# omerbt/Splice

Measured on AMD Instinct MI355X. Metric: opt_steps_per_sec, higher is better.
Workload: dtype bf16

## Files before the change

### include/splice_hip.h

```cpp
#ifndef SPLICE_HIP_H
#define SPLICE_HIP_H
#include <stddef.h>
#include <stdint.h>

#ifdef __cplusplus
extern "C" {
#endif

typedef uint16_t splice_bf16;
typedef void* splice_stream_t;

#define SPLICE_OK 0
#define SPLICE_ERR_ARG -1
#define SPLICE_ERR_HIP -2
#define SPLICE_ERR_STATE -3
#define SPLICE_ERR_NOMEM -4

int splice_version(void);
int splice_dev_switches(void);
const char* splice_last_error(void);

typedef struct splice_gemm_epilogue {
    const float* bias;
    const float* resid;
    int ldr, resid_mod;
    float* out_f32;
    int ldo;
    splice_bf16* out_bf;
    int ldbf;
    splice_bf16* out_bf_t;
    int ldt;
    splice_bf16* out_pre;
    int ldp, pre_row_lo;
    const splice_bf16* aux;
    int ldaux;
    float* out_f32_cols;
    int ld_cols, col_lo, col_hi;
    float alpha;
    int ksplit;
    long long slab_stride;
    const splice_bf16* rd_other;
    int ld_rd, rd_rows;
    float* rowdot;
    const float* row_scale;
    const float* col_scale;
    uint8_t* out_f8;
    int ld8;
    uint8_t* out_f8_t;
    int ldt8;
} splice_gemm_epilogue;

enum {
    SPLICE_EPI_BIAS = 1, SPLICE_EPI_RESID = 2, SPLICE_EPI_OUT_F32 = 4, SPLICE_EPI_OUT_BF = 8,
    SPLICE_EPI_OUT_T = 16, SPLICE_EPI_GELU = 32, SPLICE_EPI_GELU_GRAD = 64,
    SPLICE_EPI_COLS_F32 = 128, SPLICE_EPI_ALPHA = 256, SPLICE_EPI_ROWDOT = 512, SPLICE_EPI_SCALE_RC = 1024, SPLICE_EPI_OUT_F8 = 2048,
    SPLICE_EPI_OUT_F8T = 4096
};

int splice_gemm_nt_bf16(unsigned flags, const splice_bf16* A, int lda, const splice_bf16* B, int ldb,
                        int M, int N, int K, const splice_gemm_epilogue* epi, splice_stream_t stream);

int splice_gemm_nt_fp8(unsigned flags, const uint8_t* A, int lda, const uint8_t* B, int ldb, int M, int N, int K,
                       const splice_gemm_epilogue* epi, splice_stream_t stream);
int splice_quantize_rows_fp8(const float* x, int ldx, uint8_t* q, int ldq, float* scale, int rows, int cols, splice_stream_t stream);
int splice_gemm_splitk_slabs(int M, int ksplit);
int splice_gemm_force_tile(int tile);
int splice_attention_variant(int variant);
int splice_attention_qfold(int on);
int splice_attention_bwd_variant(int variant);

int splice_layernorm_fwd(const float* x, const float* gamma, const float* beta, splice_bf16* y,
                         float* mean, float* rstd, int rows, int D, float eps, splice_stream_t stream);
int splice_layernorm_bwd(const float* dy, const float* x, const float* gamma, const float* mean,
                         const float* rstd, const float* g_in, float* g_out, splice_bf16* g_out_bf,
                         int rows, int D, splice_stream_t stream);

int splice_attention_fwd(const splice_bf16* qkv, const splice_bf16* qkvT, int ldt, int B, int T, int Tld,
                         int D, int H, float scale, splice_bf16* out, float* lse, splice_stream_t stream);
int splice_attention_fwd_fp8(const uint8_t* qkv8, const uint8_t* qkvT8, int ldt8, int B, int T, int Tld, int D, int H, float scale,
                             splice_bf16* out, float* lse, splice_stream_t stream);
int splice_attention_bwd(const splice_bf16* qkv, const splice_bf16* qkvT, int ldt, int B, int T, int Tld,
                         int D, int H, float scale, const splice_bf16* out, const float* lse,
                         const splice_bf16* dout, const splice_bf16* doutT, float* delta,
                         splice_bf16* dqkv, splice_stream_t stream);
int splice_attention_probs(const splice_bf16* qkv, int B, int T, int Tld, int D, int H, float scale,
                           const float* lse, float* probs, splice_stream_t stream);

int splice_augment_structure(const float* img, float* out, float* scratch, int H, int W, int flip, int n_ops, const int* order,
                             const float* factors, float blur_sigma, splice_stream_t stream);

size_t splice_keys_selfsim_ws_bytes(int T, int D);
int splice_keys_selfsim_fwd(const float* K, int ldk, int T, int D, float eps, float* S, void* ws,
                            splice_stream_t stream);
int splice_keys_selfsim_bwd(const float* dS, const float* S, int T, int D, float eps, float* dK, int lddk,
                            int accumulate, void* ws, splice_stream_t stream);

int splice_mse(const float* a, int lda, const float* b, int ldb, int rows, int cols, float weight,
               float* loss_accum, float* grad, int ldg, splice_stream_t stream);

int splice_patchify(const float* img, splice_bf16* patches, int B, int H, int W, int p, int Tld,
                    int normalize, splice_stream_t stream);
int splice_unpatchify(const float* dpatches, float* dimg, int B, int H, int W, int p, int Tld,
                      int normalize, splice_stream_t stream);
int splice_cast_f32_bf16(const float* x, splice_bf16* y, size_t n, splice_stream_t stream);
int splice_cast_bf16_f32(const splice_bf16* x, float* y, size_t n, splice_stream_t stream);
int splice_transpose_f32_bf16(const float* x, splice_bf16* y, int rows, int cols, int ldy, splice_stream_t stream);
int splice_resize_bilinear_fwd(const float* in, float* out, int planes, int h, int w, int oh, int ow, splice_stream_t stream);
int splice_resize_bilinear_bwd(const float* dout, float* din, int planes, int h, int w, int oh, int ow, splice_stream_t stream);

int splice_vit_create(int patch, int dim, int depth, int heads, void** out_handle);
void splice_vit_destroy(void* vit);
int splice_vit_set_param(void* vit, const char* name, const float* data, long long numel, splice_stream_t stream);
float splice_vit_qscale(void* vit);
int splice_vit_params_complete(void* vit);
int splice_vit_enable_fp8(void* vit, splice_stream_t stream);
int splice_vit_ctx_create(void* vit, int B, int H, int W, const float* pos_TD, int need_grad,
                          splice_stream_t stream, void** out_ctx);
void splice_vit_ctx_destroy(void* ctx);
int splice_vit_ctx_info(void* ctx, int* T, int* Tld, int* rows);
int splice_vit_ctx_set_top_cls_only(void* ctx, int on);
int splice_vit_ctx_set_fp8(void* ctx, int mode);
int splice_vit_forward(void* ctx, const float* img, int normalize, splice_stream_t stream);
int splice_vit_forward_ex(void* ctx, const float* img, int normalize, int grad_pass_begin, splice_stream_t stream);
int splice_vit_forward_passes(void* ctx, const float* img, int normalize, int grad_pass_begin, int pass_begin, int pass_end,
                              splice_stream_t stream);
int splice_vit_get_tensor(void* ctx, int kind, int layer, void** out_ptr);
int splice_vit_read_tensor(void* ctx, int kind, int layer, void* dst, size_t bytes, splice_stream_t stream);
int splice_vit_backward(void* ctx, int pass_begin, int pass_end, const float* const* d_block,
                        const float* const* d_qkv, const float* const* d_keys, float* d_img,
                        int normalize, splice_stream_t stream);

int splice_gen_create(void** out_handle);
#define SPLICE_GEN_MAX_SCALES 6
typedef struct splice_gen_arch {
    int n_scales, in_channels, out_channels;
    int down[SPLICE_GEN_MAX_SCALES], up[SPLICE_GEN_MAX_SCALES], skip[SPLICE_GEN_MAX_SCALES];
    int filter_down[SPLICE_GEN_MAX_SCALES], filter_up[SPLICE_GEN_MAX_SCALES];
    int filter_skip;
    int reflect;
} splice_gen_arch;
int splice_gen_create_arch(const splice_gen_arch* arch, void** out_handle);
void splice_gen_destroy(void* gen);
long long splice_gen_param_count(void* gen);
int splice_gen_num_tensors(void* gen);
int splice_gen_tensor_info(void* gen, int i, const char** name, long long* offset, long long* numel);
int splice_gen_plan_create(void* gen, int N, int H, int W, int need_grad, void** out_plan);
void splice_gen_plan_destroy(void* plan);
int splice_gen_forward(void* plan, const float* params, const float* x, float* y, splice_stream_t stream);
int splice_gen_forward_borrowed(void* plan, const float* params, const float* x, float* y, splice_stream_t stream);
int splice_gen_backward(void* plan, const float* params, const float* dy, float* grads, int accumulate,
                        splice_stream_t stream);
long long splice_gen_buffer_count(void* gen);
int splice_gen_num_buffers(void* gen);
int splice_gen_buffer_info(void* gen, int i, const char** name, long long* offset, long long* numel);
int splice_gen_running_stats_update(void* const* plans, int n_plans, float* running, long long running_stride, float momentum,
                                    splice_stream_t stream);
int splice_adam_step(float* params, float* grads, float* m, float* v, long long n, float lr, float beta1,
                     float beta2, float eps, int step, int zero_grad, splice_stream_t stream);
int splice_optim_step(int kind, float* params, float* grads, float* m, float* v, long long n, float lr, float hp0, float hp1,
                      float eps, int step, int zero_grad, splice_stream_t stream);
int splice_optim_step_ex(int kind, float* params, float* grads, const float* g2, float* m, float* v, long long n, float lr,
                         const float* lr_dev, float hp0, float hp1, float eps, int step, int zero_grad, splice_stream_t stream);
int splice_optim_step_pairs(int kind, float* params, float* grads, const float* g2, float* m, float* v, int n_pairs, long long stride,
                            long long n, const float* lr_dev, float hp0, float hp1, float eps, int step, int zero_grad,
                            splice_stream_t stream);

int splice_prof_begin(int which);
int splice_prof_end(float* total_ms, int* launches);
int splice_prof_end_ex(float* total_ms, int* calls, int* kernels);
int splice_prof_end_detail(float* total_ms, int* calls, int* kernels, char* detail, int detail_len);
int splice_prof_active(void);
int splice_vit_ctx_dims(void* ctx, int* B, int* H, int* W, int* D, int* depth, int* heads, int* patch);
int splice_gen_plan_dims(void* plan, int* N, int* H, int* W, long long* nparams);
int splice_gen_plan_set_arena_stride(void* plan, long long stride);
int splice_gen_plan_set_batch_stats(void* plan, int on);
int splice_gen_plan_set_groups(void* plan, int images_per_group);
int splice_gen_plan_resize(void* plan, int H, int W);

typedef struct splice_step_config {
    int crop_h, crop_w;
    int vit_h, vit_w;
    int ent_h, ent_w;
    int ent_vit_h, ent_vit_w;
    float lambda_global_cls, lambda_global_ssim, lambda_global_identity, lambda_entire_cls, lambda_entire_ssim;
    int entire_every, cls_warmup;
    float lr, beta1, beta2, eps;
    int pairs;
    long long arena_stride;
    int fp8_selfsim;
    int top_cls_only;
    int n_crops;
    int n_crops_b;
} splice_step_config;
#define SPLICE_STEP_MAX_PAIR_CFGS 32
#define SPLICE_STEP_MAX_GROUP_IMAGES 32
int splice_step_create(const splice_step_config* cfg, void* vit_ctx_global, void* vit_ctx_entire, void* gen_plan_a, void* gen_plan_b,
                       void* gen_plan_entire, void** out_handle);
void splice_step_destroy(void* step);
int splice_step_run(void* step, float* params, float* grads, float* m, float* v, const float* A_crop, const float* B_crop,
                    const float* A_entire, int step_idx, float* losses_out, splice_stream_t stream);
int splice_step_output(void* step, int which, float** out_ptr);
int splice_step_graph_stats(void* step, long long* out);
int splice_step_use_graph(void* step, int on);
int splice_step_use_overlap(void* step, int on);
int splice_step_set_crops(void* step, int a_h, int a_w, int b_h, int b_w);
int splice_step_set_mode(void* step, int skip_adam, int accumulate);
int splice_step_set_optimizer(void* step, int kind, float hp0, float hp1, float eps);
int splice_step_set_lr(void* step, float lr);
int splice_step_set_pair_weights(void* step, const float* lambdas);
int splice_step_set_pair_lr(void* step, const float* lr);
int splice_step_set_phases(void* step, int phases, void* leader);
int splice_step_set_running_stats(void* step, float* running, long long stride);

#ifdef __cplusplus
}
#endif
#endif
```

### splice_amd/_lib.py

```python
import ctypes as C
import os

_HERE = os.path.dirname(os.path.abspath(__file__))
LIB_PATH = os.path.join(_HERE, "libsplice_hip.so")

_lib = None


class GemmEpilogue(C.Structure):
    _fields_ = [
        ("bias", C.c_void_p), ("resid", C.c_void_p), ("ldr", C.c_int), ("resid_mod", C.c_int),
        ("out_f32", C.c_void_p), ("ldo", C.c_int),
        ("out_bf", C.c_void_p), ("ldbf", C.c_int),
        ("out_bf_t", C.c_void_p), ("ldt", C.c_int),
        ("out_pre", C.c_void_p), ("ldp", C.c_int), ("pre_row_lo", C.c_int),
        ("aux", C.c_void_p), ("ldaux", C.c_int),
        ("out_f32_cols", C.c_void_p), ("ld_cols", C.c_int), ("col_lo", C.c_int), ("col_hi", C.c_int),
        ("alpha", C.c_float), ("ksplit", C.c_int), ("slab_stride", C.c_longlong),
        ("rd_other", C.c_void_p), ("ld_rd", C.c_int), ("rd_rows", C.c_int), ("rowdot", C.c_void_p),
        ("row_scale", C.c_void_p), ("col_scale", C.c_void_p),
        ("out_f8", C.c_void_p), ("ld8", C.c_int),
        ("out_f8_t", C.c_void_p), ("ldt8", C.c_int),
    ]


class GenArch(C.Structure):
    _fields_ = [("n_scales", C.c_int), ("in_channels", C.c_int), ("out_channels", C.c_int),
                ("down", C.c_int * 6), ("up", C.c_int * 6), ("skip", C.c_int * 6),
                ("filter_down", C.c_int * 6), ("filter_up", C.c_int * 6), ("filter_skip", C.c_int), ("reflect", C.c_int)]


class StepConfig(C.Structure):
    _fields_ = [
        ("crop_h", C.c_int), ("crop_w", C.c_int), ("vit_h", C.c_int), ("vit_w", C.c_int),
        ("ent_h", C.c_int), ("ent_w", C.c_int), ("ent_vit_h", C.c_int), ("ent_vit_w", C.c_int),
        ("lambda_global_cls", C.c_float), ("lambda_global_ssim", C.c_float), ("lambda_global_identity", C.c_float),
        ("lambda_entire_cls", C.c_float), ("lambda_entire_ssim", C.c_float),
        ("entire_every", C.c_int), ("cls_warmup", C.c_int),
        ("lr", C.c_float), ("beta1", C.c_float), ("beta2", C.c_float), ("eps", C.c_float),
        ("pairs", C.c_int), ("arena_stride", C.c_longlong), ("fp8_selfsim", C.c_int), ("top_cls_only", C.c_int), ("n_crops", C.c_int), ("n_crops_b", C.c_int),
    ]


EPI_BIAS, EPI_RESID, EPI_OUT_F32, EPI_OUT_BF, EPI_OUT_T = 1, 2, 4, 8, 16
EPI_GELU, EPI_GELU_GRAD, EPI_COLS_F32, EPI_ALPHA, EPI_ROWDOT, EPI_SCALE_RC, EPI_OUT_F8, EPI_OUT_F8T = 32, 64, 128, 256, 512, 1024, 2048, 4096

_vp, _i, _f, _sz, _u = C.c_void_p, C.c_int, C.c_float, C.c_size_t, C.c_uint

_SIGNATURES = {
    "splice_version": ([], C.c_int),
    "splice_dev_switches": ([], C.c_int),
    "splice_last_error": ([], C.c_char_p),
    "splice_gemm_nt_bf16": ([_u, _vp, _i, _vp, _i, _i, _i, _i, C.POINTER(GemmEpilogue), _vp], _i),
    "splice_gemm_nt_fp8": ([_u, _vp, _i, _vp, _i, _i, _i, _i, C.POINTER(GemmEpilogue), _vp], _i),
    "splice_quantize_rows_fp8": ([_vp, _i, _vp, _i, _vp, _i, _i, _vp], _i),
    "splice_gemm_splitk_slabs": ([_i, _i], _i),
    "splice_gemm_force_tile": ([_i], _i),
    "splice_attention_variant": ([_i], _i),
    "splice_attention_qfold": ([_i], _i),
    "splice_attention_bwd_variant": ([_i], _i),
    "splice_layernorm_fwd": ([_vp, _vp, _vp, _vp, _vp, _vp, _i, _i, _f, _vp], _i),
    "splice_layernorm_bwd": ([_vp, _vp, _vp, _vp, _vp, _vp, _vp, _vp, _i, _i, _vp], _i),
    "splice_attention_fwd": ([_vp, _vp, _i, _i, _i, _i, _i, _i, _f, _vp, _vp, _vp], _i),
    "splice_attention_fwd_fp8": ([_vp, _vp, _i, _i, _i, _i, _i, _i, _f, _vp, _vp, _vp], _i),
    "splice_attention_bwd": ([_vp, _vp, _i, _i, _i, _i, _i, _i, _f, _vp, _vp, _vp, _vp, _vp, _vp, _vp], _i),
    "splice_attention_probs": ([_vp, _i, _i, _i, _i, _i, _f, _vp, _vp, _vp], _i),
    "splice_augment_structure": ([_vp, _vp, _vp, _i, _i, _i, _i, C.POINTER(C.c_int), C.POINTER(C.c_float), _f, _vp], _i),
    "splice_keys_selfsim_ws_bytes": ([_i, _i], _sz),
    "splice_keys_selfsim_fwd": ([_vp, _i, _i, _i, _f, _vp, _vp, _vp], _i),
    "splice_keys_selfsim_bwd": ([_vp, _vp, _i, _i, _f, _vp, _i, _i, _vp, _vp], _i),
    "splice_mse": ([_vp, _i, _vp, _i, _i, _i, _f, _vp, _vp, _i, _vp], _i),
    "splice_patchify": ([_vp, _vp, _i, _i, _i, _i, _i, _i, _vp], _i),
    "splice_unpatchify": ([_vp, _vp, _i, _i, _i, _i, _i, _i, _vp], _i),
    "splice_cast_f32_bf16": ([_vp, _vp, _sz, _vp], _i),
    "splice_cast_bf16_f32": ([_vp, _vp, _sz, _vp], _i),
    "splice_transpose_f32_bf16": ([_vp, _vp, _i, _i, _i, _vp], _i),
    "splice_resize_bilinear_fwd": ([_vp, _vp, _i, _i, _i, _i, _i, _vp], _i),
    "splice_resize_bilinear_bwd": ([_vp, _vp, _i, _i, _i, _i, _i, _vp], _i),
    "splice_vit_create": ([_i, _i, _i, _i, C.POINTER(_vp)], _i),
    "splice_vit_destroy": ([_vp], None),
    "splice_vit_set_param": ([_vp, C.c_char_p, _vp, C.c_longlong, _vp], _i),
    "splice_vit_params_complete": ([_vp], _i),
    "splice_vit_enable_fp8": ([_vp, _vp], _i),
    "splice_vit_ctx_create": ([_vp, _i, _i, _i, _vp, _i, _vp, C.POINTER(_vp)], _i),
    "splice_vit_ctx_destroy": ([_vp], None),
    "splice_vit_ctx_info": ([_vp, C.POINTER(_i), C.POINTER(_i), C.POINTER(_i)], _i),
    "splice_vit_ctx_set_top_cls_only": ([_vp, _i], _i),
    "splice_vit_ctx_set_fp8": ([_vp, _i], _i),
    "splice_vit_forward": ([_vp, _vp, _i, _vp], _i),
    "splice_vit_forward_ex": ([_vp, _vp, _i, _i, _vp], _i),
    "splice_vit_forward_passes": ([_vp, _vp, _i, _i, _i, _i, _vp], _i),
    "splice_vit_get_tensor": ([_vp, _i, _i, C.POINTER(_vp)], _i),
    "splice_vit_qscale": ([_vp], C.c_float),
    "splice_vit_read_tensor": ([_vp, _i, _i, _vp, _sz, _vp], _i),
    "splice_vit_backward": ([_vp, _i, _i, C.POINTER(_vp), C.POINTER(_vp), C.POINTER(_vp), _vp, _i, _vp], _i),
    "splice_gen_create": ([C.POINTER(_vp)], _i),
    "splice_gen_create_arch": ([C.POINTER(GenArch), C.POINTER(_vp)], _i),
    "splice_gen_destroy": ([_vp], None),
    "splice_gen_param_count": ([_vp], C.c_longlong),
    "splice_gen_num_tensors": ([_vp], _i),
    "splice_gen_tensor_info": ([_vp, _i, C.POINTER(C.c_char_p), C.POINTER(C.c_longlong), C.POINTER(C.c_longlong)], _i),
    "splice_gen_plan_create": ([_vp, _i, _i, _i, _i, C.POINTER(_vp)], _i),
    "splice_gen_plan_destroy": ([_vp], None),
    "splice_gen_forward": ([_vp, _vp, _vp, _vp, _vp], _i),
    "splice_gen_forward_borrowed": ([_vp, _vp, _vp, _vp, _vp], _i),
    "splice_gen_backward": ([_vp, _vp, _vp, _vp, _i, _vp], _i),
    "splice_adam_step": ([_vp, _vp, _vp, _vp, C.c_longlong, _f, _f, _f, _f, _i, _i, _vp], _i),
    "splice_optim_step": ([_i, _vp, _vp, _vp, _vp, C.c_longlong, _f, _f, _f, _f, _i, _i, _vp], _i),
    "splice_optim_step_ex": ([_i, _vp, _vp, _vp, _vp, _vp, C.c_longlong, _f, _vp, _f, _f, _f, _i, _i, _vp], _i),
    "splice_optim_step_pairs": ([_i, _vp, _vp, _vp, _vp, _vp, _i, C.c_longlong, C.c_longlong, _vp, _f, _f, _f, _i, _i, _vp], _i),
    "splice_prof_begin": ([_i], _i),
    "splice_prof_end": ([C.POINTER(_f), C.POINTER(_i)], _i),
    "splice_prof_end_ex": ([C.POINTER(_f), C.POINTER(_i), C.POINTER(_i)], _i),
    "splice_prof_end_detail": ([C.POINTER(_f), C.POINTER(_i), C.POINTER(_i), C.c_char_p, _i], _i),
    "splice_prof_active": ([], _i),
    "splice_step_use_graph": ([_vp, _i], _i),
    "splice_step_graph_stats": ([_vp, C.POINTER(C.c_longlong)], _i),
    "splice_step_use_overlap": ([_vp, _i], _i),
    "splice_vit_ctx_dims": ([_vp] + [C.POINTER(_i)] * 7, _i),
    "splice_gen_plan_dims": ([_vp, C.POINTER(_i), C.POINTER(_i), C.POINTER(_i), C.POINTER(C.c_longlong)], _i),
    "splice_step_create": ([C.POINTER(StepConfig), _vp, _vp, _vp, _vp, _vp, C.POINTER(_vp)], _i),
    "splice_step_destroy": ([_vp], None),
    "splice_step_run": ([_vp, _vp, _vp, _vp, _vp, _vp, _vp, _vp, _i, _vp, _vp], _i),
    "splice_step_output": ([_vp, _i, C.POINTER(_vp)], _i),
    "splice_step_set_crops": ([_vp, _i, _i, _i, _i], _i),
    "splice_step_set_running_stats": ([_vp, _vp, C.c_longlong], _i),
    "splice_step_set_mode": ([_vp, _i, _i], _i),
    "splice_step_set_optimizer": ([_vp, _i, _f, _f, _f], _i),
    "splice_step_set_lr": ([_vp, _f], _i),
    "splice_step_set_pair_weights": ([_vp, _vp], _i),
    "splice_step_set_pair_lr": ([_vp, _vp], _i),
    "splice_step_set_phases": ([_vp, _i, _vp], _i),
    "splice_gen_buffer_count": ([_vp], C.c_longlong),
    "splice_gen_num_buffers": ([_vp], _i),
    "splice_gen_buffer_info": ([_vp, _i, C.POINTER(C.c_char_p), C.POINTER(C.c_longlong), C.POINTER(C.c_longlong)], _i),
    "splice_gen_running_stats_update": ([C.POINTER(_vp), _i, _vp, C.c_longlong, _f, _vp], _i),
    "splice_gen_plan_resize": ([_vp, _i, _i], _i),
    "splice_gen_plan_set_arena_stride": ([_vp, C.c_longlong], _i),
    "splice_gen_plan_set_batch_stats": ([_vp, _i], _i),
    "splice_gen_plan_set_groups": ([_vp, _i], _i),
}


def exported_symbols():
    return sorted(_SIGNATURES)


def register(name, argtypes, restype):
    _SIGNATURES[name] = (argtypes, restype)


def lib():
    global _lib
    if _lib is None:
        if not os.path.exists(LIB_PATH):
            raise RuntimeError(
                f"{LIB_PATH} not found: the HIP extension is not built "
                "(run __graft_entry__.build() or `make -C splice_amd/csrc`). There is no CPU fallback.")
        _lib = C.CDLL(LIB_PATH)
        for name, (argtypes, restype) in _SIGNATURES.items():
            fn = getattr(_lib, name)
            fn.argtypes = argtypes
            fn.restype = restype
    return _lib


def check(rc, what=""):
    if rc != 0:
        msg = lib().splice_last_error().decode(errors="replace")
        raise RuntimeError(f"libsplice_hip {what} failed (rc={rc}): {msg}")


def ptr(t):
    return None if t is None else C.c_void_p(t.data_ptr())


def current_stream():
    import torch
    return C.c_void_p(torch.cuda.current_stream().cuda_stream)
```

### splice_amd/csrc/capi.hip

```cpp
#include <stdarg.h>
#include <stdio.h>

#include "kernels.h"

static thread_local char g_err[512] = "";

void splice_set_error(const char* fmt, ...) {
    va_list ap;
    va_start(ap, fmt);
    vsnprintf(g_err, sizeof(g_err), fmt, ap);
    va_end(ap);
}

static int finish(int rc, const char* what) {
    if (rc != SPLICE_OK) {
        splice_set_error("%s: invalid argument", what);
        return rc;
    }
    const hipError_t e = hipGetLastError();
    if (e != hipSuccess) {
        splice_set_error("%s: HIP error %d (%s)", what, (int)e, hipGetErrorString(e));
        return SPLICE_ERR_HIP;
    }
    return SPLICE_OK;
}

#define ST(s) ((hipStream_t)(s))

extern "C" {

int splice_version(void) { return 100; }
int splice_dev_switches(void) {
#ifdef SPLICE_DEV_SWITCHES
    return 1;
#else
    return 0;
#endif
}
const char* splice_last_error(void) { return g_err; }

int splice_gemm_nt_bf16(unsigned flags, const splice_bf16* A, int lda, const splice_bf16* B, int ldb, int M, int N, int K,
                        const splice_gemm_epilogue* epi, splice_stream_t stream) {
    if (!A || !B || !epi) return finish(SPLICE_ERR_ARG, "splice_gemm_nt_bf16");
    return finish(gemm_nt_launch(flags, A, lda, B, ldb, M, N, K, *epi, ST(stream)), "splice_gemm_nt_bf16");
}

int splice_gemm_nt_fp8(unsigned flags, const uint8_t* A, int lda, const uint8_t* B, int ldb, int M, int N, int K,
                       const splice_gemm_epilogue* epi, splice_stream_t stream) {
    if (!A || !B || !epi) return finish(SPLICE_ERR_ARG, "splice_gemm_nt_fp8");
    return finish(gemm_nt_fp8_launch(flags, A, lda, B, ldb, M, N, K, *epi, ST(stream)), "splice_gemm_nt_fp8");
}
int splice_quantize_rows_fp8(const float* x, int ldx, uint8_t* q, int ldq, float* scale, int rows, int cols, splice_stream_t stream) {
    if (!x || !q || !scale) return finish(SPLICE_ERR_ARG, "splice_quantize_rows_fp8");
    return finish(quantize_rows_fp8_launch(x, ldx, q, ldq, scale, rows, cols, ST(stream)), "splice_quantize_rows_fp8");
}

int splice_gemm_splitk_slabs(int M, int ksplit) { return gemm_splitk_slabs(M, ksplit); }

int splice_gemm_force_tile(int tile) { gemm_force_tile(tile); return SPLICE_OK; }
int splice_attention_variant(int variant) { attn_set_variant(variant); return SPLICE_OK; }
int splice_attention_qfold(int on) { attn_set_qfold(on); return SPLICE_OK; }
int splice_attention_bwd_variant(int variant) { attn_set_bwd_variant(variant); return SPLICE_OK; }

int splice_layernorm_fwd(const float* x, const float* gamma, const float* beta, splice_bf16* y, float* mean, float* rstd,
                         int rows, int D, float eps, splice_stream_t stream) {
    return finish(layernorm_fwd_launch(x, gamma, beta, y, mean, rstd, rows, D, eps, ST(stream)), "splice_layernorm_fwd");
}
int splice_layernorm_bwd(const float* dy, const float* x, const float* gamma, const float* mean, const float* rstd,
                         const float* g_in, float* g_out, splice_bf16* g_out_bf, int rows, int D, splice_stream_t stream) {
    return finish(layernorm_bwd_launch(dy, x, gamma, mean, rstd, g_in, g_out, g_out_bf, rows, D, ST(stream)), "splice_layernorm_bwd");
}

int splice_attention_fwd(const splice_bf16* qkv, const splice_bf16* qkvT, int ldt, int B, int T, int Tld, int D, int H,
                         float scale, splice_bf16* out, float* lse, splice_stream_t stream) {
    AttnArgs a = {};
    a.qkv = qkv; a.qkvT = qkvT; a.ldt = ldt; a.B = B; a.T = T; a.Tld = Tld; a.D = D; a.H = H; a.scale = scale;
    a.out = out; a.lse = lse; a.qfold = attn_qfold_hook();
    return finish(attn_fwd_launch(&a, ST(stream)), "splice_attention_fwd");
}
int splice_attention_fwd_fp8(const uint8_t* qkv8, const uint8_t* qkvT8, int ldt8, int B, int T, int Tld, int D, int H, float scale,
                             splice_bf16* out, float* lse, splice_stream_t stream) {
    if (!qkv8 || !qkvT8 || !out || !lse) return finish(SPLICE_ERR_ARG, "splice_attention_fwd_fp8");
    AttnArgs a = {};
    a.qkv8 = qkv8; a.qkvT8 = qkvT8; a.ldt8 = ldt8; a.ldt = 4; a.B = B; a.T = T; a.Tld = Tld; a.D = D; a.H = H; a.scale = scale;
    a.out = out; a.lse = lse;
    return finish(attn_fwd_launch(&a, ST(stream)), "splice_attention_fwd_fp8");
}
int splice_attention_bwd(const splice_bf16* qkv, const splice_bf16* qkvT, int ldt, int B, int T, int Tld, int D, int H,
                         float scale, const splice_bf16* out, const float* lse, const splice_bf16* dout,
                         const splice_bf16* doutT, float* delta, splice_bf16* dqkv, splice_stream_t stream) {
    AttnArgs a = {};
    a.qkv = qkv; a.qkvT = qkvT; a.ldt = ldt; a.B = B; a.T = T; a.Tld = Tld; a.D = D; a.H = H; a.scale = scale;
    a.out = const_cast<splice_bf16*>(out); a.lse = const_cast<float*>(lse);
    a.dout = dout; a.doutT = doutT; a.delta = delta; a.dqkv = dqkv; a.qfold = attn_qfold_hook();
    return finish(attn_bwd_launch(&a, ST(stream)), "splice_attention_bwd");
}
int splice_attention_probs(const splice_bf16* qkv, int B, int T, int Tld, int D, int H, float scale, const float* lse,
                           float* probs, splice_stream_t stream) {
    AttnArgs a = {};
    a.qkv = qkv; a.B = B; a.T = T; a.Tld = Tld; a.D = D; a.H = H; a.scale = scale; a.lse = const_cast<float*>(lse);
    return finish(attn_probs_launch(&a, probs, ST(stream)), "splice_attention_probs");
}

int splice_augment_structure(const float* img, float* out, float* scratch, int H, int W, int flip, int n_ops, const int* order,
                             const float* factors, float blur_sigma, splice_stream_t stream) {
    return finish(augment_structure_launch(img, out, scratch, H, W, flip, n_ops, order, factors, blur_sigma, ST(stream)), "splice_augment_structure");
}

size_t splice_keys_selfsim_ws_bytes(int T, int D) { return selfsim_ws_bytes(T, D); }
int splice_keys_selfsim_fwd(const float* K, int ldk, int T, int D, float eps, float* S, void* ws, splice_stream_t stream) {
    SelfSimWs w;
    selfsim_ws_carve(ws, T, D, &w);
    return finish(selfsim_fwd_launch(K, ldk, T, D, eps, S, w, ST(stream)), "splice_keys_selfsim_fwd");
}
int splice_keys_selfsim_bwd(const float* dS, const float* S, int T, int D, float eps, float* dK, int lddk, int accumulate,
                            void* ws, splice_stream_t stream) {
    SelfSimWs w;
    selfsim_ws_carve(ws, T, D, &w);
    return finish(selfsim_bwd_launch(dS, S, T, D, eps, dK, lddk, accumulate, w, ST(stream)), "splice_keys_selfsim_bwd");
}
int splice_mse(const float* a, int lda, const float* b, int ldb, int rows, int cols, float weight, float* loss_accum,
               float* grad, int ldg, splice_stream_t stream) {
    return finish(mse_launch(a, lda, b, ldb, rows, cols, weight, loss_accum, grad, ldg, ST(stream)), "splice_mse");
}

int splice_patchify(const float* img, splice_bf16* patches, int B, int H, int W, int p, int Tld, int normalize,
                    splice_stream_t stream) {
    return finish(patchify_launch(img, patches, B, H, W, p, Tld, normalize, ST(stream)), "splice_patchify");
}
int splice_unpatchify(const float* dpatches, float* dimg, int B, int H, int W, int p, int Tld, int normalize,
                      splice_stream_t stream) {
    return finish(unpatchify_launch(dpatches, dimg, B, H, W, p, Tld, normalize, ST(stream)), "splice_unpatchify");
}
int splice_cast_f32_bf16(const float* x, splice_bf16* y, size_t n, splice_stream_t stream) {
    return finish(cast_f32_bf16_launch(x, y, n, ST(stream)), "splice_cast_f32_bf16");
}
int splice_cast_bf16_f32(const splice_bf16* x, float* y, size_t n, splice_stream_t stream) {
    return finish(cast_bf16_f32_launch(x, y, n, ST(stream)), "splice_cast_bf16_f32");
}
int splice_resize_bilinear_fwd(const float* in, float* out, int planes, int h, int w, int oh, int ow, splice_stream_t stream) {
    return finish(resize_bilinear_fwd_launch(in, out, planes, h, w, oh, ow, ST(stream)), "splice_resize_bilinear_fwd");
}
int splice_resize_bilinear_bwd(const float* dout, float* din, int planes, int h, int w, int oh, int ow, splice_stream_t stream) {
    return finish(resize_bilinear_bwd_launch(dout, din, planes, h, w, oh, ow, ST(stream)), "splice_resize_bilinear_bwd");
}
int splice_transpose_f32_bf16(const float* x, splice_bf16* y, int rows, int cols, int ldy, splice_stream_t stream) {
    return finish(transpose_f32_to_bf16_launch(x, y, rows, cols, ldy, ST(stream)), "splice_transpose_f32_bf16");
}
}
```

### splice_amd/csrc/gemm.h

```cpp
#pragma once
#include <atomic>
#include "common.h"

constexpr int GEMM_BK = 64;

typedef int mx8_t __attribute__((ext_vector_type(8)));
__device__ __forceinline__ f32x4 mfma16_fp8_mx(const u32x4& a0, const u32x4& a1, const u32x4& b0, const u32x4& b1, f32x4 c) {
    const mx8_t av = {(int)a0[0], (int)a0[1], (int)a0[2], (int)a0[3], (int)a1[0], (int)a1[1], (int)a1[2], (int)a1[3]};
    const mx8_t bv = {(int)b0[0], (int)b0[1], (int)b0[2], (int)b0[3], (int)b1[0], (int)b1[1], (int)b1[2], (int)b1[3]};
    return __builtin_amdgcn_mfma_scale_f32_16x16x128_f8f6f4(av, bv, c, 0 , 0 , 0, 0x7F7F7F7F, 0, 0x7F7F7F7F);
}

template <int BM, int BN, bool SWAP = false, bool FP8 = false, int WGM = 2>
struct GemmTile {
    static constexpr int NW = 2 * WGM;
    static constexpr int WROWS = BM / WGM;
    static constexpr int FM = WROWS / 16;
    static constexpr int FN = BN / 32;
    static constexpr int A_LOADS = BM * 8 / (64 * NW);
    static constexpr int B_LOADS = BN * 8 / (64 * NW);
    static constexpr int LDS_ELEMS = (BM + BN) * GEMM_BK;
    f32x4 acc[FM][FN];

    __device__ __forceinline__ void slice_mfma(const bf16_t* As, const bf16_t* Bs, int wm, int wn, int frow, int fchunk) {
// ... 125 lines not shown
        auto issue = [&](int sl, int stage) {
            const uint32_t st = lds0 + (uint32_t)stage * (LDS_ELEMS * 2);
            const bf16_t* ab = A + kbeg + sl * GEMM_BK;
            const bf16_t* bb = B + kbeg + sl * GEMM_BK;
#pragma unroll
            for (int i = 0; i < A_LOADS; ++i) dma16(st + i * (8 * NW * GEMM_BK * 2), ao[i], ab);
#pragma unroll
            for (int i = 0; i < B_LOADS; ++i) dma16(st + (BM + 8 * NW * i) * (GEMM_BK * 2), bo[i], bb);
        };
        const int nsl = K / GEMM_BK;
#pragma unroll
        for (int p = 0; p < NS - 1; ++p)
            if (p < nsl) issue(p, p);
        const int frow = lane & 15, fchunk = lane >> 4;
        int stage = 0, nstage = NS - 1;
        for (int t = 0; t < nsl; ++t) {
            if (t + NS - 2 < nsl) wait_dma<(NS - 2) * NL>(); else wait_dma<0>();
            __builtin_amdgcn_s_barrier();
            if (t + NS - 1 < nsl) issue(t + NS - 1, nstage);
            const bf16_t* As = smem + stage * LDS_ELEMS;
            const bf16_t* Bs = As + BM * GEMM_BK;
            slice_mfma(As, Bs, wm, wn, frow, fchunk);
            stage = stage + 1 == NS ? 0 : stage + 1;
            nstage = nstage + 1 == NS ? 0 : nstage + 1;
        }
    }

    static __device__ __forceinline__ float sumsq8(const u32x4& v, float acc) {
#pragma unroll
        for (int q = 0; q < 4; ++q) {
            const float lo = __uint_as_float(v[q] << 16), hi = __uint_as_float(v[q] & 0xFFFF0000u);
            acc = __builtin_fmaf(lo, lo, acc);
            acc = __builtin_fmaf(hi, hi, acc);
        }
        return acc;
    }
    template <int NS>
    __device__ __forceinline__ void run_ring_norms(const bf16_t* __restrict__ A, int lda, const bf16_t* __restrict__ B, int ldb, int M, int N, int K,
                                                   int m0, int n0, bf16_t* smem, float (&ssa)[FM], float (&ssb)[FN]) {
        static_assert(NS >= 3 && !FP8 && !SWAP, "bf16, unswapped, ring form");
        constexpr int NL = A_LOADS + B_LOADS;
        const int tid = threadIdx.x, lane = tid & 63;
        const int wave = __builtin_amdgcn_readfirstlane(tid >> 6);
        const int wm = wave >> 1, wn = wave & 1;
#pragma unroll
        for (int i = 0; i < FM; ++i) {
            ssa[i] = 0.f;
#pragma unroll
            for (int j = 0; j < FN; ++j) acc[i][j] = f32x4{0.f, 0.f, 0.f, 0.f};
        }
#pragma unroll
        for (int j = 0; j < FN; ++j) ssb[j] = 0.f;
        const int lrow = lane >> 3, gchunk = (lane & 7) ^ lrow;
        uint32_t ao[A_LOADS], bo[B_LOADS];
#pragma unroll
        for (int i = 0; i < A_LOADS; ++i) {
            int gr = m0 + wave * 8 + 8 * NW * i + lrow;
            gr = gr < M ? gr : M - 1;
            ao[i] = ((uint32_t)gr * (uint32_t)lda + gchunk * 8) * 2u;
        }
#pragma unroll
        for (int i = 0; i < B_LOADS; ++i) {
            int gr = n0 + wave * 8 + 8 * NW * i + lrow;
            gr = gr < N ? gr : N - 1;
            bo[i] = ((uint32_t)gr * (uint32_t)ldb + gchunk * 8) * 2u;
        }
        const uint32_t lds0 = (uint32_t)(size_t)(__attribute__((address_space(3))) bf16_t*)smem + (uint32_t)wave * (8 * GEMM_BK * 2);
        auto issue = [&](int sl, int stage) {
            const uint32_t st = lds0 + (uint32_t)stage * (LDS_ELEMS * 2);
            const bf16_t* ab = A + sl * GEMM_BK;
            const bf16_t* bb = B + sl * GEMM_BK;
#pragma unroll
            for (int i = 0; i < A_LOADS; ++i) dma16(st + i * (8 * NW * GEMM_BK * 2), ao[i], ab);
#pragma unroll
            for (int i = 0; i < B_LOADS; ++i) dma16(st + (BM + 8 * NW * i) * (GEMM_BK * 2), bo[i], bb);
        };
        const int nsl = K / GEMM_BK;
#pragma unroll
        for (int p = 0; p < NS - 1; ++p)
            if (p < nsl) issue(p, p);
        const int frow = lane & 15, fchunk = lane >> 4;
        int stage = 0, nstage = NS - 1;
        for (int t = 0; t < nsl; ++t) {
            if (t + NS - 2 < nsl) wait_dma<(NS - 2) * NL>(); else wait_dma<0>();
            __builtin_amdgcn_s_barrier();
            if (t + NS - 1 < nsl) issue(t + NS - 1, nstage);
            const bf16_t* As = smem + stage * LDS_ELEMS;
            const bf16_t* Bs = As + BM * GEMM_BK;
#pragma unroll
            for (int kk = 0; kk < 2; ++kk) {
                u32x4 af[FM], bf[FN];
                const int chunk = kk * 4 + fchunk;
#pragma unroll
                for (int i = 0; i < FM; ++i) {
                    const int row = wm * WROWS + i * 16 + frow;
                    af[i] = *reinterpret_cast<const u32x4*>(As + row * GEMM_BK + ((chunk ^ (row & 7)) << 3));
                }
#pragma unroll
                for (int j = 0; j < FN; ++j) {
                    const int row = wn * (BN / 2) + j * 16 + frow;
                    bf[j] = *reinterpret_cast<const u32x4*>(Bs + row * GEMM_BK + ((chunk ^ (row & 7)) << 3));
                }
#pragma unroll
                for (int i = 0; i < FM; ++i)
#pragma unroll
                    for (int j = 0; j < FN; ++j) acc[i][j] = mfma16(af[i], bf[j], acc[i][j]);
#pragma unroll
                for (int i = 0; i < FM; ++i) ssa[i] = sumsq8(af[i], ssa[i]);
#pragma unroll
                for (int j = 0; j < FN; ++j) ssb[j] = sumsq8(bf[j], ssb[j]);
            }
            stage = stage + 1 == NS ? 0 : stage + 1;
            nstage = nstage + 1 == NS ? 0 : nstage + 1;
        }
#pragma unroll
        for (int i = 0; i < FM; ++i) { ssa[i] += __shfl_xor(ssa[i], 16, 64); ssa[i] += __shfl_xor(ssa[i], 32, 64); }
#pragma unroll
        for (int j = 0; j < FN; ++j) { ssb[j] += __shfl_xor(ssb[j], 16, 64); ssb[j] += __shfl_xor(ssb[j], 32, 64); }
    }

    template <class F>
    __device__ __forceinline__ void for_each_cols(int m0, int n0, F&& f) {
        static_assert(SWAP, "for_each_cols needs the swapped fragment layout");
        const int lane = threadIdx.x & 63, wave = threadIdx.x >> 6;
        const int wm = wave >> 1, wn = wave & 1;
#pragma unroll
        for (int i = 0; i < FM; ++i)
#pragma unroll
            for (int j = 0; j < FN; ++j)
                f(m0 + wm * WROWS + i * 16 + (lane & 15), n0 + wn * (BN / 2) + j * 16 + (lane >> 4) * 4, acc[i][j]);
    }

    template <class F>
    __device__ __forceinline__ void for_each(int m0, int n0, F&& f) {
        const int lane = threadIdx.x & 63, wave = threadIdx.x >> 6;
        const int wm = wave >> 1, wn = wave & 1;
#pragma unroll
        for (int i = 0; i < FM; ++i)
#pragma unroll
            for (int j = 0; j < FN; ++j)
                f(m0 + wm * WROWS + i * 16 + (lane >> 4) * 4, n0 + wn * (BN / 2) + j * 16 + (lane & 15), acc[i][j]);
    }
};

constexpr int GEMM_VSPLIT_ROWS = 2401;
static inline int gemm_splitk_slabs(int M, int ks) { return (ks > 1 && M >= GEMM_VSPLIT_ROWS) ? 1 : ks; }

typedef splice_gemm_epilogue GemmEpi;
enum : unsigned {
    EPI_BIAS = SPLICE_EPI_BIAS, EPI_RESID = SPLICE_EPI_RESID, EPI_OUT_F32 = SPLICE_EPI_OUT_F32,
    EPI_OUT_BF = SPLICE_EPI_OUT_BF, EPI_OUT_T = SPLICE_EPI_OUT_T, EPI_GELU = SPLICE_EPI_GELU,
    EPI_GELU_GRAD = SPLICE_EPI_GELU_GRAD, EPI_COLS_F32 = SPLICE_EPI_COLS_F32, EPI_ALPHA = SPLICE_EPI_ALPHA,
    EPI_ROWDOT = SPLICE_EPI_ROWDOT, EPI_SCALE_RC = SPLICE_EPI_SCALE_RC, EPI_OUT_F8 = SPLICE_EPI_OUT_F8,
    EPI_OUT_F8T = SPLICE_EPI_OUT_F8T
};

template <unsigned FLAGS>
__device__ __forceinline__ void gemm_epilogue(const GemmEpi& e, int M, int N, int row0, int col, f32x4 v) {
    if (col >= N || row0 >= M) return;
    float b = 0.f;
    if (FLAGS & EPI_BIAS) b = e.bias[col];
    float x[4];
#pragma unroll
    for (int r = 0; r < 4; ++r) {
        x[r] = v[r];
        if (FLAGS & EPI_ALPHA) x[r] *= e.alpha;
        x[r] += b;
    }
    if (FLAGS & EPI_RESID) {
#pragma unroll
        for (int r = 0; r < 4; ++r)
            if (row0 + r < M) {
                const int rr = e.resid_mod ? (row0 + r) % e.resid_mod : (row0 + r);
                x[r] += e.resid[(size_t)rr * e.ldr + col];
            }
    }
    if (FLAGS & EPI_GELU_GRAD) {
#pragma unroll
        for (int r = 0; r < 4; ++r)
            if (row0 + r < M) x[r] *= gelu_grad_f(bf2f(e.aux[(size_t)(row0 + r) * e.ldaux + col]));
    }
    if (FLAGS & EPI_GELU) {
        if (e.out_pre) {
#pragma unroll
            for (int r = 0; r < 4; ++r)
                if (row0 + r < M) e.out_pre[(size_t)(row0 + r) * e.ldp + col] = f2bf(x[r]);
        }
#pragma unroll
        for (int r = 0; r < 4; ++r) x[r] = gelu_f(x[r]);
    }
    if (FLAGS & EPI_OUT_F32) {
#pragma unroll
        for (int r = 0; r < 4; ++r)
            if (row0 + r < M) e.out_f32[(size_t)(row0 + r) * e.ldo + col] = x[r];
    }
    if (FLAGS & EPI_OUT_BF) {
#pragma unroll
        for (int r = 0; r < 4; ++r)
            if (row0 + r < M) e.out_bf[(size_t)(row0 + r) * e.ldbf + col] = f2bf(x[r]);
    }
    if (FLAGS & EPI_OUT_T) {
        bf16_t* p = e.out_bf_t + (size_t)col * e.ldt + row0;
        if (row0 + 3 < M) {
            uint2 pk = {pack2bf(x[0], x[1]), pack2bf(x[2], x[3])};
            *reinterpret_cast<uint2*>(p) = pk;
        } else {
#pragma unroll
            for (int r = 0; r < 4; ++r)
                if (row0 + r < M) p[r] = f2bf(x[r]);
        }
    }
    if (FLAGS & EPI_COLS_F32) {
        if (col >= e.col_lo && col < e.col_hi) {
#pragma unroll
            for (int r = 0; r < 4; ++r)
                if (row0 + r < M) e.out_f32_cols[(size_t)(row0 + r) * e.ld_cols + (col - e.col_lo)] = x[r];
        }
    }
}

template <unsigned FLAGS, bool PRE = false>
__device__ __forceinline__ void gemm_epilogue_cols(const GemmEpi& e, int M, int N, int row, int col0, f32x4 v, float4 pre_bias = float4{},
                                                   float4 pre_resid = float4{}, uint2 pre_aux = uint2{}) {
    if (row >= M || col0 >= N) return;
    const bool full = PRE || col0 + 3 < N;
    float x[4] = {v[0], v[1], v[2], v[3]};
    if (FLAGS & EPI_ALPHA) {
#pragma unroll
        for (int r = 0; r < 4; ++r) x[r] *= e.alpha;
    }
    if (FLAGS & EPI_SCALE_RC) {
        const float rs = e.row_scale ? e.row_scale[row] : 1.0f;
#pragma unroll
        for (int r = 0; r < 4; ++r) x[r] *= rs * e.col_scale[min(col0 + r, N - 1)];
    }
    if (FLAGS & EPI_BIAS) {
        if (full) {
            const float4 b = PRE ? pre_bias : *reinterpret_cast<const float4*>(e.bias + col0);
            x[0] += b.x; x[1] += b.y; x[2] += b.z; x[3] += b.w;
        } else {
#pragma unroll
            for (int r = 0; r < 4; ++r) if (col0 + r < N) x[r] += e.bias[col0 + r];
        }
    }
    if (FLAGS & EPI_RESID) {
        const int rr = PRE ? 0 : (e.resid_mod ? row % e.resid_mod : row);
        const float* p = e.resid + (size_t)rr * e.ldr + col0;
        if (PRE || (full && !(e.ldr & 3))) {
            const float4 b = PRE ? pre_resid : *reinterpret_cast<const float4*>(p);
            x[0] += b.x; x[1] += b.y; x[2] += b.z; x[3] += b.w;
        } else {
#pragma unroll
            for (int r = 0; r < 4; ++r) if (col0 + r < N) x[r] += p[r];
        }
    }
    if (FLAGS & EPI_GELU_GRAD) {
        const bf16_t* p = e.aux + (size_t)row * e.ldaux + col0;
        if (PRE || (full && !(e.ldaux & 3))) {
            const uint2 u = PRE ? pre_aux : *reinterpret_cast<const uint2*>(p);
            x[0] *= gelu_grad_f(bf2f((bf16_t)(u.x & 0xFFFF))); x[1] *= gelu_grad_f(bf2f((bf16_t)(u.x >> 16)));
            x[2] *= gelu_grad_f(bf2f((bf16_t)(u.y & 0xFFFF))); x[3] *= gelu_grad_f(bf2f((bf16_t)(u.y >> 16)));
        } else {
#pragma unroll
            for (int r = 0; r < 4; ++r) if (col0 + r < N) x[r] *= gelu_grad_f(bf2f(p[r]));
        }
    }
    auto store_bf = [&](bf16_t* base, int ld) {
        bf16_t* p = base + (size_t)row * ld + col0;
        if (full && !(ld & 3)) *reinterpret_cast<uint2*>(p) = uint2{pack2bf(x[0], x[1]), pack2bf(x[2], x[3])};
        else {
#pragma unroll
            for (int r = 0; r < 4; ++r) if (col0 + r < N) p[r] = f2bf(x[r]);
        }
    };
    if (FLAGS & EPI_GELU) {
        if (e.out_pre && row >= e.pre_row_lo) store_bf(e.out_pre, e.ldp);
#pragma unroll
        for (int r = 0; r < 4; ++r) x[r] = gelu_f(x[r]);
    }
    if (FLAGS & EPI_OUT_F32) {
        float* p = e.out_f32 + (size_t)row * e.ldo + col0;
        if (full && !(e.ldo & 3)) *reinterpret_cast<float4*>(p) = float4{x[0], x[1], x[2], x[3]};
        else {
#pragma unroll
            for (int r = 0; r < 4; ++r) if (col0 + r < N) p[r] = x[r];
        }
    }
    if (FLAGS & EPI_OUT_BF) store_bf(e.out_bf, e.ldbf);
    if (FLAGS & EPI_OUT_T) {
#pragma unroll
        for (int r = 0; r < 4; ++r)
            if (col0 + r < N) e.out_bf_t[(size_t)(col0 + r) * e.ldt + row] = f2bf(x[r]);
    }
    if (FLAGS & EPI_COLS_F32) {
#pragma unroll
        for (int r = 0; r < 4; ++r) {
            const int c = col0 + r;
            if (c < N && c >= e.col_lo && c < e.col_hi) e.out_f32_cols[(size_t)row * e.ld_cols + (c - e.col_lo)] = x[r];
        }
    }
}

template <unsigned FLAGS, bool PRE, bool STORE_F32 = true>
__device__ __forceinline__ f32x4 gemm_frag_value(const GemmEpi& e, int M, int N, int row, int col0, f32x4 v, float4 pre_bias, float4 pre_resid,
                                                 uint2 pre_aux) {
    const bool inb = row < M && col0 < N;
    const int rowc = min(row, M - 1), colc = min(col0, N - 4);
    float x[4] = {v[0], v[1], v[2], v[3]};
    if (FLAGS & EPI_ALPHA) {
#pragma unroll
        for (int r = 0; r < 4; ++r) x[r] *= e.alpha;
    }
    if (FLAGS & EPI_SCALE_RC) {
        const float rs = e.row_scale ? e.row_scale[rowc] : 1.0f;
        const float4 cs = *reinterpret_cast<const float4*>(e.col_scale + colc);
        x[0] *= rs * cs.x; x[1] *= rs * cs.y; x[2] *= rs * cs.z; x[3] *= rs * cs.w;
    }
    if (FLAGS & EPI_BIAS) {
        const float4 b = PRE ? pre_bias : *reinterpret_cast<const float4*>(e.bias + colc);
        x[0] += b.x; x[1] += b.y; x[2] += b.z; x[3] += b.w;
    }
    if (FLAGS & EPI_RESID) {
        const int rr = e.resid_mod ? rowc % e.resid_mod : rowc;
        const float4 b = PRE ? pre_resid : *reinterpret_cast<const float4*>(e.resid + (size_t)rr * e.ldr + colc);
        x[0] += b.x; x[1] += b.y; x[2] += b.z; x[3] += b.w;
    }
    if (FLAGS & EPI_GELU_GRAD) {
        const uint2 u = PRE ? pre_aux : *reinterpret_cast<const uint2*>(e.aux + (size_t)rowc * e.ldaux + colc);
        x[0] *= gelu_grad_f(bf2f((bf16_t)(u.x & 0xFFFF))); x[1] *= gelu_grad_f(bf2f((bf16_t)(u.x >> 16)));
        x[2] *= gelu_grad_f(bf2f((bf16_t)(u.y & 0xFFFF))); x[3] *= gelu_grad_f(bf2f((bf16_t)(u.y >> 16)));
    }
    if (inb) {
        if ((FLAGS & EPI_OUT_F32) && STORE_F32) *reinterpret_cast<float4*>(e.out_f32 + (size_t)row * e.ldo + col0) = float4{x[0], x[1], x[2], x[3]};
        if (FLAGS & EPI_COLS_F32) {
#pragma unroll
            for (int r = 0; r < 4; ++r) {
                const int c = col0 + r;
                if (c >= e.col_lo && c < e.col_hi) e.out_f32_cols[(size_t)row * e.ld_cols + (c - e.col_lo)] = x[r];
            }
        }
    }
    return f32x4{x[0], x[1], x[2], x[3]};
}
template <int BM, int BN, bool TRANSPOSED>
__device__ __forceinline__ void gemm_stage_store(const f32x4 (&acc)[BM / 32][BN / 32], bf16_t* cs, bf16_t* out, int ld, int M, int N, int m0, int n0,
                                                 int row_lo) {
    constexpr int FMt = BM / 32, FNt = BN / 32;
    constexpr int R = TRANSPOSED ? BN : BM, Cc = TRANSPOSED ? BM : BN, PITCH = Cc + 8;
    const int lane = threadIdx.x & 63, wave = threadIdx.x >> 6, wm = wave >> 1, wn = wave & 1;
    __syncthreads();
#pragma unroll
    for (int i = 0; i < FMt; ++i)
#pragma unroll
        for (int j = 0; j < FNt; ++j) {
            const int lr = wm * (BM / 2) + i * 16 + (lane & 15), lc = wn * (BN / 2) + j * 16 + (lane >> 4) * 4;
            const f32x4 v = acc[i][j];
            if (!TRANSPOSED) {
                *reinterpret_cast<uint2*>(cs + lr * PITCH + lc) = uint2{pack2bf(v[0], v[1]), pack2bf(v[2], v[3])};
            } else {
#pragma unroll
                for (int r = 0; r < 4; ++r) cs[(lc + r) * PITCH + lr] = f2bf(v[r]);
            }
        }
    __syncthreads();
    const int r0 = TRANSPOSED ? n0 : m0, c0 = TRANSPOSED ? m0 : n0, Rm = TRANSPOSED ? N : M, Cm = TRANSPOSED ? M : N;
    constexpr int CH = Cc / 8;
    for (int c = threadIdx.x; c < R * CH; c += 256) {
        const int r = c / CH, k = (c % CH) * 8;
        const int gr = r0 + r, gc = c0 + k;
        if (gr >= Rm || gc >= Cm) continue;
        if (!TRANSPOSED && gr < row_lo) continue;
        const u32x4 v = *reinterpret_cast<const u32x4*>(cs + r * PITCH + k);
        bf16_t* q = out + (size_t)gr * ld + gc;
        if (gc + 7 < Cm && !(ld & 7)) st_out(reinterpret_cast<u32x4*>(q), v);
        else {
            const bf16_t* h = reinterpret_cast<const bf16_t*>(&v);
#pragma unroll
            for (int t = 0; t < 8; ++t)
                if (gc + t < Cm) q[t] = h[t];
        }
    }
}

__device__ __forceinline__ uint32_t pack4_e4m3_sat(const f32x4& v) {
    int w = 0;
    w = __builtin_amdgcn_cvt_pk_fp8_f32(fminf(fmaxf(v[0], -448.f), 448.f), fminf(fmaxf(v[1], -448.f), 448.f), w, false);
    w = __builtin_amdgcn_cvt_pk_fp8_f32(fminf(fmaxf(v[2], -448.f), 448.f), fminf(fmaxf(v[3], -448.f), 448.f), w, true);
    return (uint32_t)w;
}
template <int BM, int BN>
__device__ __forceinline__ void gemm_stage_store_f8(const f32x4 (&acc)[BM / 32][BN / 32], uint8_t* cs, uint8_t* out, int ld, int M, int N, int m0, int n0) {
    constexpr int FMt = BM / 32, FNt = BN / 32, PITCH = BN + 16, CH = BN / 16;
    const int lane = threadIdx.x & 63, wave = threadIdx.x >> 6, wm = wave >> 1, wn = wave & 1;
    __syncthreads();
#pragma unroll
    for (int i = 0; i < FMt; ++i)
#pragma unroll
        for (int j = 0; j < FNt; ++j) {
            const int lr = wm * (BM / 2) + i * 16 + (lane & 15), lc = wn * (BN / 2) + j * 16 + (lane >> 4) * 4;
            *reinterpret_cast<uint32_t*>(cs + lr * PITCH + lc) = pack4_e4m3_sat(acc[i][j]);
        }
    __syncthreads();
    for (int c = threadIdx.x; c < BM * CH; c += 256) {
        const int r = c / CH, k = (c % CH) * 16;
        const int gr = m0 + r, gc = n0 + k;
        if (gr >= M || gc >= N) continue;
        st_out(reinterpret_cast<u32x4*>(out + (size_t)gr * ld + gc), *reinterpret_cast<const u32x4*>(cs + r * PITCH + k));
    }
}

template <int BM, int BN>
__device__ __forceinline__ void gemm_stage_store_f8t(const f32x4 (&acc)[BM / 32][BN / 32], uint8_t* cs, uint8_t* out, int ld, int M, int N, int m0, int n0) {
    constexpr int FMt = BM / 32, FNt = BN / 32, PITCH = BM + 16, CH = BM / 16;
    const int lane = threadIdx.x & 63, wave = threadIdx.x >> 6, wm = wave >> 1, wn = wave & 1;
    __syncthreads();
#pragma unroll
    for (int i = 0; i < FMt; ++i)
#pragma unroll
        for (int j = 0; j < FNt; ++j) {
            const int lr = wm * (BM / 2) + i * 16 + (lane & 15), lc = wn * (BN / 2) + j * 16 + (lane >> 4) * 4;
            const uint32_t w = pack4_e4m3_sat(acc[i][j]);
#pragma unroll
            for (int r = 0; r < 4; ++r) cs[(lc + r) * PITCH + lr] = (uint8_t)(w >> (8 * r));
        }
    __syncthreads();
    for (int c = threadIdx.x; c < BN * CH; c += 256) {
        const int r = c / CH, k = (c % CH) * 16;
        const int gr = n0 + r, gc = m0 + k;
        if (gr >= N || gc >= M) continue;
        uint8_t* q = out + (size_t)gr * ld + gc;
        if (gc + 15 < M) st_out(reinterpret_cast<u32x4*>(q), *reinterpret_cast<const u32x4*>(cs + r * PITCH + k));
        else
            for (int t = 0; t < 16 && gc + t < M; ++t) q[t] = cs[r * PITCH + k + t];
    }
}

template <int BM, int BN>
__device__ __forceinline__ void gemm_stage_store_f32(const f32x4 (&acc)[BM / 32][BN / 32], float* cs, float* out, int ld, int M, int N, int m0, int n0) {
    constexpr int FMt = BM / 32, FNt = BN / 32, PITCH = BN + 4, CH = BN / 4;
    const int lane = threadIdx.x & 63, wave = threadIdx.x >> 6, wm = wave >> 1, wn = wave & 1;
    __syncthreads();
#pragma unroll
    for (int i = 0; i < FMt; ++i)
#pragma unroll
        for (int j = 0; j < FNt; ++j) {
            const int lr = wm * (BM / 2) + i * 16 + (lane & 15), lc = wn * (BN / 2) + j * 16 + (lane >> 4) * 4;
            *reinterpret_cast<f32x4*>(cs + lr * PITCH + lc) = acc[i][j];
        }
    __syncthreads();
    for (int c = threadIdx.x; c < BM * CH; c += 256) {
        const int r = c / CH, k = (c % CH) * 4;
        const int gr = m0 + r, gc = n0 + k;
        if (gr >= M || gc >= N) continue;
        st_out(reinterpret_cast<f32x4*>(out + (size_t)gr * ld + gc), *reinterpret_cast<const f32x4*>(cs + r * PITCH + k));
    }
}

template <int BM, int BN, unsigned FLAGS, int NS, bool FP8 = false>
__global__ __launch_bounds__(256) void gemm_nt_kernel(const bf16_t* __restrict__ A, int lda, const bf16_t* __restrict__ B,
                                                      int ldb, int M, int N, int K, int gm, int ksplit, GemmEpi e) {
    extern __shared__ __attribute__((aligned(16))) bf16_t gemm_smem[];
    const int tiles_n = (N + BN - 1) / BN, tiles_m = (M + BM - 1) / BM;
    const int nwg = gridDim.x;
    int t = xcd_remap(blockIdx.x, nwg);
    int kbeg = 0;
    if (ksplit > 1) {
        const int slice = t % ksplit;
        t /= ksplit;
        K /= ksplit;
        kbeg = slice * K;
        e.out_f32 += (size_t)slice * e.slab_stride;
    }
    int tm, tn;
    grouped_tile(t, tiles_m, tiles_n, gm, tm, tn);
    const int m0 = tm * BM, n0 = tn * BN;
    GemmTile<BM, BN, true, FP8> tile;
    bool walked = false;
    if constexpr (FLAGS == EPI_OUT_F32 && NS == 2) {
        if (ksplit < -1) {
            const int vs = -ksplit, Kp = K / vs;
            f32x4 tot[GemmTile<BM, BN>::FM][GemmTile<BM, BN>::FN];
            for (int sl = 0; sl < vs; ++sl) {
                if (sl) __syncthreads();
                tile.run_glds(A, lda, B, ldb, M, N, Kp, m0, n0, gemm_smem, sl * Kp);
#pragma unroll
                for (int i = 0; i < GemmTile<BM, BN>::FM; ++i)
#pragma unroll
                    for (int j = 0; j < GemmTile<BM, BN>::FN; ++j) tot[i][j] = sl ? tot[i][j] + tile.acc[i][j] : tile.acc[i][j];
            }
#pragma unroll
            for (int i = 0; i < GemmTile<BM, BN>::FM; ++i)
#pragma unroll
                for (int j = 0; j < GemmTile<BM, BN>::FN; ++j) tile.acc[i][j] = tot[i][j];
            walked = true;
        }
    }
    if (walked) {
    } else if (NS == 2) tile.run_glds(A, lda, B, ldb, M, N, K, m0, n0, gemm_smem, kbeg);
    else tile.template run_ring<(NS < 3 ? 3 : NS)>(A, lda, B, ldb, M, N, K, m0, n0, gemm_smem, kbeg);
    constexpr bool HAS_OPERANDS = (FLAGS & (EPI_BIAS | EPI_RESID | EPI_GELU_GRAD)) != 0;
    constexpr bool STAGE_F32_FITS = (size_t)NS * GemmTile<BM, BN>::LDS_ELEMS * 2 >= (size_t)BM * (BN + 4) * 4;
    const bool pre_ok = HAS_OPERANDS && !(N & 3) && (!(FLAGS & EPI_RESID) || !(e.ldr & 3)) && (!(FLAGS & EPI_GELU_GRAD) || !(e.ldaux & 3));
    const bool stage_ok = (FLAGS & EPI_OUT_BF) && !(N & 3) && (!(FLAGS & EPI_RESID) || !(e.ldr & 3)) && (!(FLAGS & EPI_GELU_GRAD) || !(e.ldaux & 3)) &&
                          (!(FLAGS & EPI_OUT_F32) || !(e.ldo & 3)) && (!(FLAGS & EPI_OUT_T) || !(e.ldt & 7));
    if constexpr ((FLAGS & EPI_OUT_F8) != 0 && (FLAGS & EPI_OUT_BF) == 0) {
        constexpr int FMt = GemmTile<BM, BN>::FM, FNt = GemmTile<BM, BN>::FN;
        static_assert((size_t)NS * GemmTile<BM, BN>::LDS_ELEMS >= (size_t)BM * (BN + 8), "the ring must hold one staged output tile");
        const int lane = threadIdx.x & 63, wave = threadIdx.x >> 6, wm = wave >> 1, wn = wave & 1;
        float4 pb[FNt];
#pragma unroll
        for (int j = 0; j < FNt; ++j)
            if (FLAGS & EPI_BIAS) pb[j] = *reinterpret_cast<const float4*>(e.bias + min(n0 + wn * (BN / 2) + j * 16 + (lane >> 4) * 4, N - 4));
#pragma unroll
        for (int i = 0; i < FMt; ++i)
#pragma unroll
            for (int j = 0; j < FNt; ++j)
                tile.acc[i][j] = gemm_frag_value<FLAGS, true>(e, M, N, m0 + wm * (BM / 2) + i * 16 + (lane & 15), n0 + wn * (BN / 2) + j * 16 + (lane >> 4) * 4,
                                                              tile.acc[i][j], pb[j], float4{}, uint2{});
        if (FLAGS & EPI_GELU) {
            if (e.out_pre) gemm_stage_store<BM, BN, false>(tile.acc, gemm_smem, e.out_pre, e.ldp, M, N, m0, n0, e.pre_row_lo);
#pragma unroll
            for (int i = 0; i < FMt; ++i)
#pragma unroll
                for (int j = 0; j < FNt; ++j)
#pragma unroll
                    for (int r = 0; r < 4; ++r) tile.acc[i][j][r] = gelu_f(tile.acc[i][j][r]);
        }
        gemm_stage_store_f8<BM, BN>(tile.acc, reinterpret_cast<uint8_t*>(gemm_smem), e.out_f8, e.ld8, M, N, m0, n0);
    } else if ((FLAGS & EPI_OUT_BF) && stage_ok) {
        constexpr int FMt = GemmTile<BM, BN>::FM, FNt = GemmTile<BM, BN>::FN;
        static_assert((size_t)NS * GemmTile<BM, BN>::LDS_ELEMS >= (size_t)BM * (BN + 8) && (size_t)NS * GemmTile<BM, BN>::LDS_ELEMS >= (size_t)BN * (BM + 8),
                      "the ring must hold one staged output tile");
        const int lane = threadIdx.x & 63, wave = threadIdx.x >> 6, wm = wave >> 1, wn = wave & 1;
        float4 pb[FNt], pr[FMt][FNt];
        uint2 pa[FMt][FNt];
        if (HAS_OPERANDS) {
#pragma unroll
            for (int j = 0; j < FNt; ++j) {
                const int colc = min(n0 + wn * (BN / 2) + j * 16 + (lane >> 4) * 4, N - 4);
                if (FLAGS & EPI_BIAS) pb[j] = *reinterpret_cast<const float4*>(e.bias + colc);
#pragma unroll
                for (int i = 0; i < FMt; ++i) {
                    const int rowc = min(m0 + wm * (BM / 2) + i * 16 + (lane & 15), M - 1);
                    const int rr = e.resid_mod ? rowc % e.resid_mod : rowc;
                    if (FLAGS & EPI_RESID) pr[i][j] = *reinterpret_cast<const float4*>(e.resid + (size_t)rr * e.ldr + colc);
                    if (FLAGS & EPI_GELU_GRAD) pa[i][j] = *reinterpret_cast<const uint2*>(e.aux + (size_t)rowc * e.ldaux + colc);
                }
            }
        }
#pragma unroll
        for (int i = 0; i < FMt; ++i)
#pragma unroll
            for (int j = 0; j < FNt; ++j)
                tile.acc[i][j] = gemm_frag_value<FLAGS, HAS_OPERANDS>(e, M, N, m0 + wm * (BM / 2) + i * 16 + (lane & 15), n0 + wn * (BN / 2) + j * 16 + (lane >> 4) * 4,
                                                                      tile.acc[i][j], pb[j], pr[i][j], pa[i][j]);
        if (FLAGS & EPI_GELU) {
            if (e.out_pre) gemm_stage_store<BM, BN, false>(tile.acc, gemm_smem, e.out_pre, e.ldp, M, N, m0, n0, e.pre_row_lo);
#pragma unroll
            for (int i = 0; i < FMt; ++i)
#pragma unroll
                for (int j = 0; j < FNt; ++j)
#pragma unroll
                    for (int r = 0; r < 4; ++r) tile.acc[i][j][r] = gelu_f(tile.acc[i][j][r]);
        }
        gemm_stage_store<BM, BN, false>(tile.acc, gemm_smem, e.out_bf, e.ldbf, M, N, m0, n0, 0);
        if (FLAGS & EPI_OUT_T) gemm_stage_store<BM, BN, true>(tile.acc, gemm_smem, e.out_bf_t, e.ldt, M, N, m0, n0, 0);
        if constexpr ((FLAGS & EPI_OUT_F8) != 0) gemm_stage_store_f8<BM, BN>(tile.acc, reinterpret_cast<uint8_t*>(gemm_smem), e.out_f8, e.ld8, M, N, m0, n0);
        if constexpr ((FLAGS & EPI_OUT_F8T) != 0) gemm_stage_store_f8t<BM, BN>(tile.acc, reinterpret_cast<uint8_t*>(gemm_smem), e.out_f8_t, e.ldt8, M, N, m0, n0);
        if (FLAGS & EPI_ROWDOT) {
#pragma unroll
            for (int i = 0; i < FMt; ++i)
#pragma unroll
                for (int j = 0; j < FNt; ++j)
#pragma unroll
                    for (int r = 0; r < 4; ++r) tile.acc[i][j][r] = bf2f(f2bf(tile.acc[i][j][r]));
        }
    } else if (STAGE_F32_FITS && (FLAGS & EPI_OUT_F32) && !(FLAGS & (EPI_OUT_BF | EPI_COLS_F32)) && !(N & 3) && !(e.ldo & 3) && (!(FLAGS & EPI_RESID) || !(e.ldr & 3))) {
        constexpr int FMt = GemmTile<BM, BN>::FM, FNt = GemmTile<BM, BN>::FN;
        const int lane = threadIdx.x & 63, wave = threadIdx.x >> 6, wm = wave >> 1, wn = wave & 1;
        float4 pb[FNt], pr[FMt][FNt];
        if (HAS_OPERANDS) {
#pragma unroll
            for (int j = 0; j < FNt; ++j) {
                const int colc = min(n0 + wn * (BN / 2) + j * 16 + (lane >> 4) * 4, N - 4);
                if (FLAGS & EPI_BIAS) pb[j] = *reinterpret_cast<const float4*>(e.bias + colc);
#pragma unroll
                for (int i = 0; i < FMt; ++i) {
                    const int rowc = min(m0 + wm * (BM / 2) + i * 16 + (lane & 15), M - 1);
                    const int rr = e.resid_mod ? rowc % e.resid_mod : rowc;
                    if (FLAGS & EPI_RESID) pr[i][j] = *reinterpret_cast<const float4*>(e.resid + (size_t)rr * e.ldr + colc);
                }
            }
        }
#pragma unroll
        for (int i = 0; i < FMt; ++i)
#pragma unroll
            for (int j = 0; j < FNt; ++j)
                tile.acc[i][j] = gemm_frag_value<FLAGS, HAS_OPERANDS, false>(e, M, N, m0 + wm * (BM / 2) + i * 16 + (lane & 15),
                                                                             n0 + wn * (BN / 2) + j * 16 + (lane >> 4) * 4, tile.acc[i][j], pb[j], pr[i][j], uint2{});
        if constexpr (STAGE_F32_FITS) gemm_stage_store_f32<BM, BN>(tile.acc, reinterpret_cast<float*>(gemm_smem), e.out_f32, e.ldo, M, N, m0, n0);
    } else if (pre_ok) {
        constexpr int FMt = GemmTile<BM, BN>::FM, FNt = GemmTile<BM, BN>::FN;
        const int lane = threadIdx.x & 63, wave = threadIdx.x >> 6, wm = wave >> 1, wn = wave & 1;
        float4 pb[FNt], pr[FMt][FNt];
        uint2 pa[FMt][FNt];
        int colc[FNt];
#pragma unroll
        for (int j = 0; j < FNt; ++j) {
            colc[j] = min(n0 + wn * (BN / 2) + j * 16 + (lane >> 4) * 4, N - 4);
            if (FLAGS & EPI_BIAS) pb[j] = *reinterpret_cast<const float4*>(e.bias + colc[j]);
        }
#pragma unroll
        for (int i = 0; i < FMt; ++i) {
            const int rowc = min(m0 + wm * (BM / 2) + i * 16 + (lane & 15), M - 1);
            const int rr = e.resid_mod ? rowc % e.resid_mod : rowc;
#pragma unroll
            for (int j = 0; j < FNt; ++j) {
                if (FLAGS & EPI_RESID) pr[i][j] = *reinterpret_cast<const float4*>(e.resid + (size_t)rr * e.ldr + colc[j]);
                if (FLAGS & EPI_GELU_GRAD) pa[i][j] = *reinterpret_cast<const uint2*>(e.aux + (size_t)rowc * e.ldaux + colc[j]);
            }
        }
#pragma unroll
        for (int i = 0; i < FMt; ++i)
#pragma unroll
            for (int j = 0; j < FNt; ++j)
                gemm_epilogue_cols<FLAGS, true>(e, M, N, m0 + wm * (BM / 2) + i * 16 + (lane & 15), n0 + wn * (BN / 2) + j * 16 + (lane >> 4) * 4,
                                                tile.acc[i][j], pb[j], pr[i][j], pa[i][j]);
    } else {
        tile.for_each_cols(m0, n0, [&](int row, int col0, f32x4 v) { gemm_epilogue_cols<FLAGS>(e, M, N, row, col0, v); });
    }
    if (FLAGS & EPI_ROWDOT) {
        static_assert(!(FLAGS & EPI_ROWDOT) || BN == 64, "EPI_ROWDOT needs the 64-column tile");
        constexpr int FMt = GemmTile<BM, BN>::FM, FNt = GemmTile<BM, BN>::FN;
        const int lane = threadIdx.x & 63, wave = threadIdx.x >> 6, wm = wave >> 1, wn = wave & 1;
        float* red = reinterpret_cast<float*>(gemm_smem);
        __syncthreads();
        uint2 ov[FMt][FNt];
#pragma unroll
        for (int i = 0; i < FMt; ++i)
#pragma unroll
            for (int j = 0; j < FNt; ++j)
                ov[i][j] = *reinterpret_cast<const uint2*>(e.rd_other + (size_t)min(m0 + wm * (BM / 2) + i * 16 + (lane & 15), M - 1) * e.ld_rd + n0 +
                                                           wn * (BN / 2) + j * 16 + (lane >> 4) * 4);
#pragma unroll
        for (int i = 0; i < FMt; ++i) {
            const int lrow = wm * (BM / 2) + i * 16 + (lane & 15);
            const int row = m0 + lrow;
            float part = 0.f;
            if (row < M) {
#pragma unroll
                for (int j = 0; j < FNt; ++j) {
                    const uint2 o = ov[i][j];
                    const f32x4 v = tile.acc[i][j];
                    part += bf2f(f2bf(v[0])) * bf2f((bf16_t)(o.x & 0xFFFF)) + bf2f(f2bf(v[1])) * bf2f((bf16_t)(o.x >> 16)) +
                            bf2f(f2bf(v[2])) * bf2f((bf16_t)(o.y & 0xFFFF)) + bf2f(f2bf(v[3])) * bf2f((bf16_t)(o.y >> 16));
                }
            }
            part += __shfl_xor(part, 16, 64);
            part += __shfl_xor(part, 32, 64);
            if (lane < 16) red[wn * BM + lrow] = part;
        }
        __syncthreads();
        if (threadIdx.x < BM) {
            const int row = m0 + threadIdx.x;
            if (row < M)
                e.rowdot[((size_t)(row / e.rd_rows) * (N / 64) + n0 / 64) * e.rd_rows + row % e.rd_rows] = red[threadIdx.x] + red[BM + threadIdx.x];
        }
    }
}

template <int BM, int BN, unsigned FLAGS, int NS, bool FP8 = false>
static inline void launch_gemm_nt(hipStream_t s, const bf16_t* A, int lda, const bf16_t* B, int ldb, int M, int N, int K,
                                  const GemmEpi& e) {
    const int tm = cdiv(M, BM), tn = cdiv(N, BN);
    int ksplit = (FLAGS == EPI_OUT_F32 && e.ksplit > 1 && K % (e.ksplit * GEMM_BK) == 0) ? e.ksplit : 1;
    if (NS == 2 && ksplit > 1 && gemm_splitk_slabs(M, ksplit) == 1) ksplit = -ksplit;
    const int grid = tm * tn * (ksplit > 1 ? ksplit : 1);
    int gm = 1;
    while ((gm + 1) * (gm + 1) * BM <= (tm * tn / 8 + 1) * BN && gm + 1 <= tm) ++gm;
    constexpr size_t lds = (size_t)NS * GemmTile<BM, BN>::LDS_ELEMS * sizeof(bf16_t);
    if (lds > 65536) {
        int dev = 0;
        (void)hipGetDevice(&dev);
        static std::atomic<unsigned long long> done_mask{0};
        const unsigned long long bit = 1ull << (dev & 63);
        if (!(done_mask.load(std::memory_order_relaxed) & bit)) {
            (void)hipFuncSetAttribute((const void*)gemm_nt_kernel<BM, BN, FLAGS, NS, FP8>, hipFuncAttributeMaxDynamicSharedMemorySize, (int)lds);
            done_mask.fetch_or(bit, std::memory_order_relaxed);
        }
    }
    SPLICE_LAUNCH((gemm_nt_kernel<BM, BN, FLAGS, NS, FP8>), dim3(grid), dim3(256), lds, s, A, lda, B, ldb, M, N, K, gm, ksplit, e);
}
```

### splice_amd/csrc/gemm.hip

```cpp
#include "kernels.h"
#include "gemm8p.h"

static int g_force_tile = 0;
void gemm_force_tile(int t) { g_force_tile = t; }

template <unsigned FLAGS>
static int dispatch_tile(const bf16_t* A, int lda, const bf16_t* B, int ldb, int M, int N, int K, const GemmEpi& e,
                         hipStream_t s) {
    const long t128 = (long)cdiv(M, 128) * cdiv(N, 128);
    const long t12864 = (long)cdiv(M, 128) * cdiv(N, 64);
    if constexpr (FLAGS == (EPI_BIAS | EPI_OUT_BF) || FLAGS == (EPI_BIAS | EPI_GELU | EPI_OUT_BF) || FLAGS == (EPI_BIAS | EPI_RESID | EPI_OUT_F32)) {
        constexpr int on8p = 7;
        const int bit = (FLAGS & EPI_OUT_F32) ? 4 : (FLAGS & EPI_GELU) ? 2 : 1;
        const bool want = g_force_tile == 5 ? gemm8p_operands_ok(N, K, e, FLAGS) : (!g_force_tile && (on8p & bit) && gemm8p_shape_ok(M, N, K, lda, ldb, e, FLAGS));
        if (want) {
            launch_gemm8p<FLAGS>(s, A, lda, B, ldb, M, N, K, e);
            return SPLICE_OK;
        }
    }
    int tile, ring;
    if (g_force_tile && g_force_tile != 5 && !(FLAGS & EPI_ROWDOT)) { tile = g_force_tile % 10; ring = g_force_tile / 10; }
    else {
        constexpr int t2min = 300;
        constexpr int t2ring = 3;
#ifndef SPLICE_T1MIN
#define SPLICE_T1MIN 230
#endif
#ifndef SPLICE_T96
#define SPLICE_T96 6
#endif
        constexpr int t1min = SPLICE_T1MIN;
        constexpr int bigm = 2401;
        tile = (FLAGS & EPI_ROWDOT) ? 3 : N <= 768 ? (M >= bigm ? 2 : 3) : t128 >= t1min ? 1 : t12864 >= t2min ? 2 : 3;
        const int ks = (FLAGS == EPI_OUT_F32 && e.ksplit > 1 && K % (e.ksplit * GEMM_BK) == 0) ? e.ksplit : 1;
        constexpr int ringk = 768;
        constexpr int ringwg = 640;
        ring = (tile == 3 && M <= 2400 && K / ks >= (ks > 1 ? 768 : ringk) && (long)cdiv(M, 64) * cdiv(N, 64) * ks <= ringwg) ? 1 : 0;
        if (tile == 2 && t2ring && M <= 2400) ring = t2ring == 3 ? 2 : 1;
        constexpr int shortns = 3;
        if (ring && tile == 3 && ks == 1 && K < 1536 && shortns == 3) ring = 2;
    }
    if constexpr ((FLAGS & EPI_ROWDOT) != 0) {
        if (ring == 2) launch_gemm_nt<64, 64, FLAGS, 3>(s, A, lda, B, ldb, M, N, K, e);
        else if (ring) launch_gemm_nt<64, 64, FLAGS, 4>(s, A, lda, B, ldb, M, N, K, e);
        else launch_gemm_nt<64, 64, FLAGS, 2>(s, A, lda, B, ldb, M, N, K, e);
    } else {
        if constexpr (FLAGS == (EPI_BIAS | EPI_RESID | EPI_OUT_F32)) {
            constexpr int t96 = SPLICE_T96;
            const long wg64 = (long)cdiv(M, 64) * cdiv(N, 64), wg96 = (long)cdiv(M, 64) * (N / 96);
            if (t96 && !(t96 == 5 && K < 1536) && !(t96 == 6 && K >= 1536) && tile == 3 && N % 96 == 0 && wg64 > 256 && wg96 <= 256) {
                if (K >= 1536 && t96 != 3) launch_gemm_nt<64, 96, FLAGS, 4>(s, A, lda, B, ldb, M, N, K, e);
                else launch_gemm_nt<64, 96, FLAGS, 3>(s, A, lda, B, ldb, M, N, K, e);
                return SPLICE_OK;
            }
        }
        if (tile == 3 && ring == 2) { launch_gemm_nt<64, 64, FLAGS, 3>(s, A, lda, B, ldb, M, N, K, e); return SPLICE_OK; }
        if (tile == 2 && ring == 2) { launch_gemm_nt<128, 64, FLAGS, 3>(s, A, lda, B, ldb, M, N, K, e); return SPLICE_OK; }
        switch (tile * 2 + (ring ? 1 : 0)) {
            case 2: launch_gemm_nt<128, 128, FLAGS, 2>(s, A, lda, B, ldb, M, N, K, e); break;
            case 3: launch_gemm_nt<128, 128, FLAGS, 4>(s, A, lda, B, ldb, M, N, K, e); break;
            case 4: launch_gemm_nt<128, 64, FLAGS, 2>(s, A, lda, B, ldb, M, N, K, e); break;
            case 5: launch_gemm_nt<128, 64, FLAGS, 4>(s, A, lda, B, ldb, M, N, K, e); break;
            case 6: launch_gemm_nt<64, 64, FLAGS, 2>(s, A, lda, B, ldb, M, N, K, e); break;
            default: launch_gemm_nt<64, 64, FLAGS, 4>(s, A, lda, B, ldb, M, N, K, e); break;
        }
    }
    return SPLICE_OK;
}

int gemm_nt_launch(unsigned flags, const bf16_t* A, int lda, const bf16_t* B, int ldb, int M, int N, int K,
                   const GemmEpi& e, hipStream_t s) {
    if (M < 1 || N < 1 || K < GEMM_BK || K % GEMM_BK || lda % 8 || ldb % 8) return SPLICE_ERR_ARG;
    if ((size_t)M * lda * sizeof(bf16_t) >= (1ull << 32) || (size_t)N * ldb * sizeof(bf16_t) >= (1ull << 32)) return SPLICE_ERR_ARG;
    if ((flags & EPI_OUT_T) && (e.ldt % 4)) return SPLICE_ERR_ARG;
    if ((flags & EPI_ROWDOT) && (N % 64 || !e.rd_other || !e.rowdot || e.rd_rows < 1 || e.ld_rd % 4)) return SPLICE_ERR_ARG;
#define CASE(F) case (F): return dispatch_tile<(F)>(A, lda, B, ldb, M, N, K, e, s)
    switch (flags) {
        CASE(EPI_BIAS | EPI_OUT_BF | EPI_OUT_T);
        CASE(EPI_BIAS | EPI_OUT_BF | EPI_OUT_T | EPI_COLS_F32);
        CASE(EPI_BIAS | EPI_OUT_F32);
        CASE(EPI_BIAS | EPI_OUT_BF);
        CASE(EPI_BIAS | EPI_RESID | EPI_OUT_F32);
        CASE(EPI_BIAS | EPI_GELU | EPI_OUT_BF);
        CASE(EPI_OUT_F32);
        CASE(EPI_OUT_F32 | EPI_ALPHA);
        CASE(EPI_OUT_BF);
        CASE(EPI_OUT_BF | EPI_OUT_T);
        CASE(EPI_OUT_BF | EPI_OUT_T | EPI_ROWDOT);
        CASE(EPI_OUT_BF | EPI_ROWDOT);
        CASE(EPI_GELU_GRAD | EPI_OUT_BF);
        default: return SPLICE_ERR_ARG;
    }
#undef CASE
}

template <unsigned FLAGS>
static int dispatch_fp8(const uint8_t* A, int lda, const uint8_t* B, int ldb, int M, int N, int K, const GemmEpi& e, hipStream_t s) {
    const bf16_t* a = reinterpret_cast<const bf16_t*>(A);
    const bf16_t* b = reinterpret_cast<const bf16_t*>(B);
    const long t128 = (long)cdiv(M, 128) * cdiv(N, 128), t12864 = (long)cdiv(M, 128) * cdiv(N, 64);
    constexpr int t1min8 = 230;
    constexpr int t2min8 = 300;
    if (N <= 768) {
        if (M >= 2401) launch_gemm_nt<128, 64, FLAGS, 2, true>(s, a, lda / 2, b, ldb / 2, M, N, K / 2, e);
        else launch_gemm_nt<64, 64, FLAGS, 4, true>(s, a, lda / 2, b, ldb / 2, M, N, K / 2, e);
    } else if (t128 >= t1min8) launch_gemm_nt<128, 128, FLAGS, 2, true>(s, a, lda / 2, b, ldb / 2, M, N, K / 2, e);
    else if (t12864 >= t2min8) launch_gemm_nt<128, 64, FLAGS, 3, true>(s, a, lda / 2, b, ldb / 2, M, N, K / 2, e);
    else launch_gemm_nt<64, 64, FLAGS, 3, true>(s, a, lda / 2, b, ldb / 2, M, N, K / 2, e);
    return SPLICE_OK;
}
int gemm_nt_fp8_launch(unsigned flags, const uint8_t* A, int lda, const uint8_t* B, int ldb, int M, int N, int K, const GemmEpi& e, hipStream_t s) {
    if (M < 1 || N < 1 || K < 128 || K % 128 || lda % 16 || ldb % 16) return SPLICE_ERR_ARG;
    if ((size_t)M * lda >= (1ull << 32) || (size_t)N * ldb >= (1ull << 32)) return SPLICE_ERR_ARG;
    if (!(flags & EPI_SCALE_RC) || !e.col_scale) return SPLICE_ERR_ARG;
    if ((flags & EPI_OUT_T) && (e.ldt % 4)) return SPLICE_ERR_ARG;
    if ((flags & EPI_OUT_F8) && (!e.out_f8 || N % 16 || e.ld8 % 16 || (e.out_pre && e.ldp % 8))) return SPLICE_ERR_ARG;
    if ((flags & EPI_OUT_F8T) && (!e.out_f8_t || e.ldt8 % 16)) return SPLICE_ERR_ARG;
    if ((flags & (EPI_OUT_F8 | EPI_OUT_F8T)) && (flags & EPI_OUT_BF) && (N % 16 || e.ldbf % 8 || ((flags & EPI_OUT_T) && e.ldt % 8))) return SPLICE_ERR_ARG;
#define CASE8(F) case (F): return dispatch_fp8<(F)>(A, lda, B, ldb, M, N, K, e, s)
    switch (flags) {
        CASE8(EPI_SCALE_RC | EPI_BIAS | EPI_OUT_BF);
        CASE8(EPI_SCALE_RC | EPI_BIAS | EPI_OUT_BF | EPI_OUT_F8 | EPI_OUT_F8T);
        CASE8(EPI_SCALE_RC | EPI_BIAS | EPI_OUT_BF | EPI_OUT_T);
        CASE8(EPI_SCALE_RC | EPI_BIAS | EPI_OUT_BF | EPI_OUT_T | EPI_COLS_F32);
        CASE8(EPI_SCALE_RC | EPI_BIAS | EPI_OUT_BF | EPI_OUT_T | EPI_OUT_F8 | EPI_OUT_F8T);
        CASE8(EPI_SCALE_RC | EPI_BIAS | EPI_OUT_BF | EPI_OUT_T | EPI_COLS_F32 | EPI_OUT_F8 | EPI_OUT_F8T);
        CASE8(EPI_SCALE_RC | EPI_OUT_F32);
        CASE8(EPI_SCALE_RC | EPI_BIAS | EPI_GELU | EPI_OUT_F8);
        CASE8(EPI_SCALE_RC | EPI_BIAS | EPI_RESID | EPI_OUT_F32);
        default: return SPLICE_ERR_ARG;
    }
#undef CASE8
}
```

### splice_amd/csrc/gemm8p.h

```cpp
#pragma once
#include <type_traits>
#include "gemm.h"

struct Gemm8p {
    static constexpr int BM = 256, BN = 256, NTHREADS = 512;
    static constexpr int SLOT_ELEMS = 128 * GEMM_BK;
    static constexpr int LDS_BYTES = 8 * SLOT_ELEMS * 2;
    f32x4 acc[8][4];
    u32x4 af[4][2];
    u32x4 bfr[2][2][2];

    template <int N>
    static __device__ __forceinline__ void wait_vm() { asm volatile("s_waitcnt vmcnt(%0)" ::"n"(N) : "memory"); }
    template <int N>
    static __device__ __forceinline__ void wait_lgkm() { asm volatile("s_waitcnt lgkmcnt(%0)" ::"n"(N) : "memory"); }
    static __device__ __forceinline__ void dma16(uint32_t lds_byte, uint32_t voff, const void* sbase) {
        asm volatile("s_mov_b32 m0, %0\n\ts_nop 0\n\tglobal_load_lds_dwordx4 %1, %2" ::"s"(lds_byte), "v"(voff), "s"(sbase) : "memory");
    }

    struct Src { int m0, n0; };
    template <class Coords, class Epi>
    __device__ __forceinline__ void run_tiles(const bf16_t* __restrict__ A, int lda, const bf16_t* __restrict__ B, int ldb, int M, int N, int K, int count,
                                              Coords&& coords, Epi&& epi, bf16_t* smem) {
        const int tid = threadIdx.x, lane = tid & 63;
        const int wave = __builtin_amdgcn_readfirstlane(tid >> 6);
        const int wr = wave >> 2, wc = wave & 3;
        const uint32_t lds0 = (uint32_t)(size_t)(__attribute__((address_space(3))) bf16_t*)smem + (uint32_t)wave * 1024u;
        const int nt = K / GEMM_BK;
        const int prow = wave * 8 + (lane >> 3);
        const uint32_t pcol = (uint32_t)(((lane & 7) ^ (lane >> 3)) * 16);
        auto issue = [&](const Src& sc, int tile, auto qc, auto slotc) {
            constexpr int q = decltype(qc)::value, slot = decltype(slotc)::value;
            constexpr bool isA = q == 1 || q == 3;
            constexpr int h = q >> 1;
            const bf16_t* src = (isA ? A : B) + (size_t)tile * GEMM_BK;
            const uint32_t d = lds0 + (uint32_t)slot * (SLOT_ELEMS * 2);
            const int r0 = (isA ? sc.m0 : sc.n0) + h * 128 + prow, lim = (isA ? M : N) - 1;
            const uint32_t ld2 = (uint32_t)(isA ? lda : ldb) * 2u;
            dma16(d, (uint32_t)min(r0, lim) * ld2 + pcol, src);
            dma16(d + 8192u, (uint32_t)min(r0 + 64, lim) * ld2 + pcol, src);
        };
        const int frow = lane & 15, fchunk = lane >> 4;
        const bf16_t* arow = smem + (wr * 64 + frow) * GEMM_BK;
        const bf16_t* brow = smem + (wc * 32 + frow) * GEMM_BK;
        const int ck0 = ((0 * 4 + fchunk) ^ (frow & 7)) << 3, ck1 = ((1 * 4 + fchunk) ^ (frow & 7)) << 3;
        auto read_a = [&](auto slotc) {
            constexpr int slot = decltype(slotc)::value;
#pragma unroll
            for (int i = 0; i < 4; ++i) {
                af[i][0] = *reinterpret_cast<const u32x4*>(arow + slot * SLOT_ELEMS + i * 16 * GEMM_BK + ck0);
                af[i][1] = *reinterpret_cast<const u32x4*>(arow + slot * SLOT_ELEMS + i * 16 * GEMM_BK + ck1);
            }
        };
        auto read_b = [&](auto slotc, auto nhc) {
            constexpr int slot = decltype(slotc)::value, nh = decltype(nhc)::value;
#pragma unroll
            for (int j = 0; j < 2; ++j) {
                bfr[nh][j][0] = *reinterpret_cast<const u32x4*>(brow + slot * SLOT_ELEMS + j * 16 * GEMM_BK + ck0);
                bfr[nh][j][1] = *reinterpret_cast<const u32x4*>(brow + slot * SLOT_ELEMS + j * 16 * GEMM_BK + ck1);
            }
        };
        auto quadrant = [&](auto mhc, auto nhc) {
            constexpr int mh = decltype(mhc)::value, nh = decltype(nhc)::value;
            __builtin_amdgcn_s_setprio(1);
#pragma unroll
            for (int kk = 0; kk < 2; ++kk)
#pragma unroll
                for (int i = 0; i < 4; ++i)
#pragma unroll
                    for (int j = 0; j < 2; ++j) acc[mh * 4 + i][nh * 2 + j] = mfma16(bfr[nh][j][kk], af[i][kk], acc[mh * 4 + i][nh * 2 + j]);
            __builtin_amdgcn_s_setprio(0);
        };
        using I0 = std::integral_constant<int, 0>; using I1 = std::integral_constant<int, 1>; using I2 = std::integral_constant<int, 2>;
        using I3 = std::integral_constant<int, 3>;
        auto ktile = [&](auto parc, const Src& s0, int t0, bool on0, const Src& s1, int t1, bool on1, int waitn) {
            constexpr int PAR = decltype(parc)::value;
            using S0 = std::integral_constant<int, PAR * 4 + 0>; using S1 = std::integral_constant<int, PAR * 4 + 1>;
            using S2 = std::integral_constant<int, PAR * 4 + 2>; using S3 = std::integral_constant<int, PAR * 4 + 3>;
            using O3 = std::integral_constant<int, (1 - PAR) * 4 + 3>;
            read_b(S0{}, I0{});
            __builtin_amdgcn_sched_barrier(0);
            read_a(S1{});
            __builtin_amdgcn_sched_barrier(0);
            if (on0) issue(s0, t0, I3{}, O3{});
            wait_lgkm<8>();
            __builtin_amdgcn_s_barrier();
            wait_lgkm<0>();
            __builtin_amdgcn_sched_barrier(0);
            quadrant(I0{}, I0{});
            __builtin_amdgcn_sched_barrier(0);
            __builtin_amdgcn_s_barrier();
            read_b(S2{}, I1{});
            __builtin_amdgcn_sched_barrier(0);
            if (on1) issue(s1, t1, I0{}, S0{});
            __builtin_amdgcn_s_barrier();
            wait_lgkm<0>();
            __builtin_amdgcn_sched_barrier(0);
            quadrant(I0{}, I1{});
            __builtin_amdgcn_sched_barrier(0);
            __builtin_amdgcn_s_barrier();
            read_a(S3{});
            __builtin_amdgcn_sched_barrier(0);
            if (on1) issue(s1, t1, I1{}, S1{});
            __builtin_amdgcn_s_barrier();
            wait_lgkm<0>();
            __builtin_amdgcn_sched_barrier(0);
            quadrant(I1{}, I1{});
            __builtin_amdgcn_sched_barrier(0);
            __builtin_amdgcn_s_barrier();
            if (on1) issue(s1, t1, I2{}, S2{});
            if (waitn == 6) wait_vm<6>();
            else if (waitn == 0) wait_vm<0>();
            __builtin_amdgcn_s_barrier();
            __builtin_amdgcn_sched_barrier(0);
            quadrant(I1{}, I0{});
            __builtin_amdgcn_sched_barrier(0);
            __builtin_amdgcn_s_barrier();
        };
        if (count < 1) return;
        Src cur, nxt;
        coords(0, cur.m0, cur.n0);
        nxt = cur;
        if (count > 1) coords(1, nxt.m0, nxt.n0);
        issue(cur, 0, I0{}, I0{}); issue(cur, 0, I1{}, I1{}); issue(cur, 0, I2{}, I2{}); issue(cur, 0, I3{}, I3{});
        issue(cur, 1, I0{}, std::integral_constant<int, 4>{}); issue(cur, 1, I1{}, std::integral_constant<int, 5>{}); issue(cur, 1, I2{}, std::integral_constant<int, 6>{});
        wait_vm<6>();
        __builtin_amdgcn_s_barrier();
        if (wr == 1) __builtin_amdgcn_s_barrier();
#pragma unroll
        for (int i = 0; i < 8; ++i)
#pragma unroll
            for (int j = 0; j < 4; ++j) acc[i][j] = f32x4{0.f, 0.f, 0.f, 0.f};
        int r = 0, t = 0;
        const int pairs = count * (nt >> 1);
#pragma unroll 1
        for (int it = 0; it < pairs; ++it) {
            const bool more = r + 1 < count;
            const bool in2 = t + 2 < nt, in3 = t + 3 < nt;
            const Src s2 = in2 ? cur : nxt, s3 = in3 ? cur : nxt;
            const int k2 = in2 ? t + 2 : 0, k3 = in3 ? t + 3 : 1;
            const bool on2 = in2 || more, on3 = in3 || more;
            ktile(I0{}, cur, t + 1, true, s2, k2, on2, on2 ? 6 : 0);
            ktile(I1{}, s2, k2, on2, s3, k3, on3, on3 ? 6 : -1);
            t += 2;
            if (t == nt) {
                epi(cur.m0, cur.n0);
#pragma unroll
                for (int i = 0; i < 8; ++i)
#pragma unroll
                    for (int j = 0; j < 4; ++j) acc[i][j] = f32x4{0.f, 0.f, 0.f, 0.f};
                cur = nxt;
                ++r;
                t = 0;
                if (r + 1 < count) coords(r + 1, nxt.m0, nxt.n0);
            }
        }
        if (wr == 0) __builtin_amdgcn_s_barrier();
    }
};

template <unsigned FLAGS>
__global__ __launch_bounds__(512) void gemm8p_kernel(const bf16_t* __restrict__ A, int lda, const bf16_t* __restrict__ B, int ldb, int M, int N, int K, int gm,
                                                     GemmEpi e) {
    static_assert(FLAGS == (EPI_BIAS | EPI_OUT_BF) || FLAGS == (EPI_BIAS | EPI_GELU | EPI_OUT_BF) || FLAGS == (EPI_BIAS | EPI_RESID | EPI_OUT_F32),
                  "epilogues of the 8-phase tile");
    extern __shared__ __attribute__((aligned(16))) bf16_t gemm8p_smem[];
    const int tiles_n = N / 256, tiles_m = (M + 255) / 256, ntiles = tiles_m * tiles_n;
    const int G = gridDim.x;
    const int count = (ntiles - (int)blockIdx.x + G - 1) / G;
    Gemm8p g;
    const int lane = threadIdx.x & 63, wave = threadIdx.x >> 6, wr = wave >> 2, wc = wave & 3;
    const int grp = lane >> 4;
    const int c8 = ((grp & 1) << 4) | ((grp >> 1) << 3);
    g.run_tiles(A, lda, B, ldb, M, N, K, count,
                [&](int r, int& m0, int& n0) {
                    const int t = xcd_remap(blockIdx.x + r * G, ntiles);
                    int tm, tn;
                    grouped_tile(t, tiles_m, tiles_n, gm, tm, tn);
                    m0 = tm * 256; n0 = tn * 256;
                },
                [&](int m0, int n0) {
                    if constexpr ((FLAGS & EPI_OUT_F32) != 0) {
#pragma unroll
                        for (int nh = 0; nh < 2; ++nh) {
                            const int colf = n0 + nh * 128 + wc * 32 + grp * 4;
                            const float4 b0 = *reinterpret_cast<const float4*>(e.bias + colf), b1 = *reinterpret_cast<const float4*>(e.bias + colf + 16);
#pragma unroll
                            for (int mh = 0; mh < 2; ++mh) {
                                float4 r0[4], r1[4];
#pragma unroll
                                for (int i = 0; i < 4; ++i) {
                                    const int row = min(m0 + mh * 128 + wr * 64 + i * 16 + (lane & 15), M - 1);
                                    r0[i] = *reinterpret_cast<const float4*>(e.resid + (size_t)row * e.ldr + colf);
                                    r1[i] = *reinterpret_cast<const float4*>(e.resid + (size_t)row * e.ldr + colf + 16);
                                }
#pragma unroll
                                for (int i = 0; i < 4; ++i) {
                                    const int row = m0 + mh * 128 + wr * 64 + i * 16 + (lane & 15);
                                    const f32x4 v0 = g.acc[mh * 4 + i][nh * 2 + 0], v1 = g.acc[mh * 4 + i][nh * 2 + 1];
                                    if (row < M) {
                                        float* q = e.out_f32 + (size_t)row * e.ldo + colf;
                                        *reinterpret_cast<float4*>(q) = float4{v0[0] + b0.x + r0[i].x, v0[1] + b0.y + r0[i].y, v0[2] + b0.z + r0[i].z, v0[3] + b0.w + r0[i].w};
                                        *reinterpret_cast<float4*>(q + 16) = float4{v1[0] + b1.x + r1[i].x, v1[1] + b1.y + r1[i].y, v1[2] + b1.z + r1[i].z, v1[3] + b1.w + r1[i].w};
                                    }
                                }
                            }
                        }
                        return;
                    }
#pragma unroll
                    for (int nh = 0; nh < 2; ++nh) {
                        const int colf = n0 + nh * 128 + wc * 32 + grp * 4;
                        const float4 b0 = *reinterpret_cast<const float4*>(e.bias + colf), b1 = *reinterpret_cast<const float4*>(e.bias + colf + 16);
                        const int col = n0 + nh * 128 + wc * 32 + c8;
#pragma unroll
                        for (int mh = 0; mh < 2; ++mh)
#pragma unroll
                            for (int i = 0; i < 4; ++i) {
                                f32x4 v0 = g.acc[mh * 4 + i][nh * 2 + 0], v1 = g.acc[mh * 4 + i][nh * 2 + 1];
                                v0[0] += b0.x; v0[1] += b0.y; v0[2] += b0.z; v0[3] += b0.w;
                                v1[0] += b1.x; v1[1] += b1.y; v1[2] += b1.z; v1[3] += b1.w;
                                const int row = m0 + mh * 128 + wr * 64 + i * 16 + (lane & 15);
                                auto store8 = [&](bf16_t* base, int ld, const f32x4& x0, const f32x4& x1, bool on) {
                                    const uint2 a = uint2{pack2bf(x0[0], x0[1]), pack2bf(x0[2], x0[3])}, b = uint2{pack2bf(x1[0], x1[1]), pack2bf(x1[2], x1[3])};
                                    const auto rx = __builtin_amdgcn_permlane16_swap(a.x, b.x, false, false);
                                    const auto ry = __builtin_amdgcn_permlane16_swap(a.y, b.y, false, false);
                                    if (on) *reinterpret_cast<uint4*>(base + (size_t)row * ld + col) = uint4{rx[0], ry[0], rx[1], ry[1]};
                                };
                                if constexpr ((FLAGS & EPI_GELU) != 0) {
                                    if (e.out_pre) store8(e.out_pre, e.ldp, v0, v1, row < M && row >= e.pre_row_lo);
#pragma unroll
                                    for (int r = 0; r < 4; ++r) { v0[r] = gelu_f(v0[r]); v1[r] = gelu_f(v1[r]); }
                                }
                                store8(e.out_bf, e.ldbf, v0, v1, row < M);
                            }
                    }
                },
                gemm8p_smem);
}

static inline bool gemm8p_operands_ok(int N, int K, const GemmEpi& e, unsigned flags) {
    if (N % 256 || K % 128 || K < 128 || (reinterpret_cast<size_t>(e.bias) & 15)) return false;
    if (flags & EPI_OUT_F32)
        return !e.resid_mod && e.ldr % 4 == 0 && e.ldo % 4 == 0 && !(reinterpret_cast<size_t>(e.resid) & 15) && !(reinterpret_cast<size_t>(e.out_f32) & 15);
    if (e.ldbf % 8 || (reinterpret_cast<size_t>(e.out_bf) & 15)) return false;
    if ((flags & EPI_GELU) && e.out_pre && (e.ldp % 8 || (reinterpret_cast<size_t>(e.out_pre) & 15))) return false;
    return true;
}
static inline bool gemm8p_shape_ok(int M, int N, int K, int lda, int ldb, const GemmEpi& e, unsigned flags) {
    if (!gemm8p_operands_ok(N, K, e, flags) || M < 256) return false;
    const long tiles = (long)((M + 255) / 256) * (N / 256);
    if ((flags & EPI_OUT_F32) && tiles >= 128 && tiles <= 256) return true;
    if ((flags & EPI_OUT_F32) && tiles > 256 && tiles * 100 >= ((tiles + 255) / 256) * 256 * 55) return true;
    if (tiles < 200) return false;
    const long rounds = (tiles + 255) / 256;
    return tiles * 100 >= rounds * 256 * 75;
}
template <unsigned FLAGS>
static inline void launch_gemm8p(hipStream_t s, const bf16_t* A, int lda, const bf16_t* B, int ldb, int M, int N, int K, const GemmEpi& e) {
    const int tm = (M + 255) / 256, tn = N / 256, tiles = tm * tn;
    int gm = 1;
    while ((gm + 1) * (gm + 1) <= (tiles / 8 + 1) && gm + 1 <= tm) ++gm;
    int dev = 0;
    (void)hipGetDevice(&dev);
    static std::atomic<unsigned long long> done_mask{0};
    const unsigned long long bit = 1ull << (dev & 63);
    if (!(done_mask.load(std::memory_order_relaxed) & bit)) {
        (void)hipFuncSetAttribute((const void*)gemm8p_kernel<FLAGS>, hipFuncAttributeMaxDynamicSharedMemorySize, Gemm8p::LDS_BYTES);
        done_mask.fetch_or(bit, std::memory_order_relaxed);
    }
    SPLICE_LAUNCH((gemm8p_kernel<FLAGS>), dim3(tiles < 256 ? tiles : 256), dim3(512), Gemm8p::LDS_BYTES, s, A, lda, B, ldb, M, N, K, gm, e);
}
```

### splice_amd/csrc/kernels.h

```cpp
#pragma once
#include "common.h"
#include "gemm.h"

struct AttnArgs {
    const bf16_t* qkv;
    const bf16_t* qkvT;
    int ldt;
    int B, T, Tld, D, H;
    float scale;
    bf16_t* out;
    float* lse;
    const bf16_t* dout;
    const bf16_t* doutT;
    float* delta;
    int delta_ready;
    bf16_t* dqkv;
    const uint8_t* qkv8;
    const uint8_t* qkvT8;
    int ldt8;
    int qfold;
};
int attn_fwd_launch(const AttnArgs* a, hipStream_t s);
int attn_bwd_launch(const AttnArgs* a, hipStream_t s);
int attn_probs_launch(const AttnArgs* a, float* probs, hipStream_t s);
void attn_set_variant(int v);
void attn_set_bwd_variant(int v);
int attn_qfold_hook();
void attn_set_qfold(int on);

int attn_cls_fwd_launch(const bf16_t* qkv, const bf16_t* qkvT, int ldt, int B, int T, int Tld, int D, int H, float scale, bf16_t* out, float* probs,
                        hipStream_t s);
int attn_cls_bwd_launch(const bf16_t* qkv, const bf16_t* qkvT, int ldt, int B, int T, int Tld, int D, int H, float scale, const float* probs,
                        const float* dout_slabs, int n_slabs, size_t slab_stride, bf16_t* dqkv, hipStream_t s);
int ln_rows_fwd_launch(float* x, size_t xs, const float* gamma, const float* beta, bf16_t* y, size_t ys, float* mean, float* rstd, size_t ss, int rows,
                       int D, float eps, const float* slabs, int n_slabs, size_t slab_stride, const float* bias, const float* resid, size_t rs, hipStream_t s);
int ln_rows_bwd_launch(float* dy, size_t dys, const float* x, size_t xs, const float* gamma, const float* mean, const float* rstd, size_t ss, float* g,
                       bf16_t* g_bf, int rows, int D, int n_slabs, size_t slab_stride, hipStream_t s);
int rows_finish_launch(int mode, const float* slabs, int n_slabs, size_t slab_stride, int rows, int N, const float* bias, const float* resid, size_t rs,
                       float* out_f32, size_t os, bf16_t* out_bf, bf16_t* pre_bf, const bf16_t* aux, size_t ps, int pre_lo, hipStream_t s);

int gemm_nt_launch(unsigned flags, const bf16_t* A, int lda, const bf16_t* B, int ldb, int M, int N, int K,
                   const GemmEpi& e, hipStream_t s);

void gemm_force_tile(int t);
int gemm_nt_fp8_launch(unsigned flags, const uint8_t* A, int lda, const uint8_t* B, int ldb, int M, int N, int K, const GemmEpi& e, hipStream_t s);

int layernorm_fwd_launch(const float* x, const float* gamma, const float* beta, bf16_t* y, float* mean, float* rstd,
                         int rows, int D, float eps, hipStream_t s);
int layernorm_fwd_fp8_launch(const float* x, const float* gamma, const float* beta, uint8_t* y, float* yscale, float* mean, float* rstd,
                             int rows, int D, float eps, hipStream_t s);
int quantize_rows_fp8_launch(const float* x, int ldx, uint8_t* q, int ldq, float* scale, int rows, int cols, hipStream_t s);
int quantize_rows_bf16_fp8_launch(const bf16_t* x, int ldx, uint8_t* q, int ldq, float* scale, int rows, int cols, hipStream_t s);
int quantize_keys_fp8_launch(const bf16_t* k, int ldk, size_t k_pstride, uint8_t* q, int ldq, size_t q_pstride, float* qnorm, int T, int Tp, int D,
                             int pairs, hipStream_t s);
int layernorm_bwd_launch(const float* dy, const float* x, const float* gamma, const float* mean, const float* rstd,
                         const float* g_in, float* g_out, bf16_t* g_out_bf, int rows, int D, hipStream_t s);
int layernorm_bwd_slabs_launch(const float* dy, int n_slabs, size_t slab_stride, const float* x, const float* gamma, const float* mean,
                               const float* rstd, const float* g_in, float* g_out, bf16_t* g_out_bf, int rows, int D, hipStream_t s);
int patchify_launch(const float* img, bf16_t* patches, int B, int H, int W, int p, int Tld, int normalize, hipStream_t s);
int unpatchify_launch(const float* dpatches, float* dimg, int B, int H, int W, int p, int Tld, int normalize, hipStream_t s);
int cast_f32_bf16_launch(const float* x, bf16_t* y, size_t n, hipStream_t s);
int cast_bf16_f32_launch(const bf16_t* x, float* y, size_t n, hipStream_t s);
int transpose_f32_to_bf16_launch(const float* x, bf16_t* y, int rows, int cols, int ldy, hipStream_t s);
int fill_f32_launch(float* x, float v, size_t n, hipStream_t s);
int dev_copy_launch(void* dst, const void* src, size_t bytes, hipStream_t s);
int dev_zero_launch(void* dst, size_t bytes, hipStream_t s);
int resize_bilinear_fwd_launch(const float* in, float* out, int planes, int h, int w, int oh, int ow, hipStream_t s);
int resize_bilinear_bwd_launch(const float* dout, float* din, int planes, int h, int w, int oh, int ow, hipStream_t s);
int add_f32_launch(float* y, const float* x, size_t n, hipStream_t s);

int augment_structure_launch(const float* img, float* out, float* scratch, int H, int W, int flip, int n_ops, const int* order,
                             const float* factors, float blur_sigma, hipStream_t s);

struct SelfSimWs {
    bf16_t* kbf;
    bf16_t* kbfT;
    float* norm;
    bf16_t* wmat;
    float* rowdot;
    int Tp;
};
size_t selfsim_ws_bytes(int T, int D);
void selfsim_ws_carve(void* base, int T, int D, SelfSimWs* ws);
int selfsim_fwd_launch(const float* K, int ldk, int T, int D, float eps, float* S, const SelfSimWs& ws, hipStream_t s);
int selfsim_bwd_launch(const float* dS, const float* S, int T, int D, float eps, float* dK, int lddk, int accumulate,
                       const SelfSimWs& ws, hipStream_t s);
struct SelfSimBatch {
    int T, Tp, D, pairs;
    int ldk, ldt;
    size_t k_pstride, kT_pstride;
    const bf16_t* k_tgt;
    const bf16_t* k_x;
    const bf16_t* kT_x;
    float* S_tgt;
    bf16_t* wmat;
    float *norm_tgt, *norm_x;
    float* rpart;
    float* loss_part;
    size_t part_pstride;
    float* dk;
    size_t dk_pstride; int lddk;
    float eps, e_scale, loss_scale;
    const float* e_scale_tab;
    int fp8;
    uint8_t *k8_tgt, *k8_x;
    float *qnorm_tgt, *qnorm_x;
};
size_t selfsim_batch_ws_bytes(int T, int D, int pairs);
void selfsim_batch_carve(void* base, int T, int D, int pairs, SelfSimBatch* b);
int selfsim_target_launch(const SelfSimBatch& b, hipStream_t s);
int selfsim_loss_launch(const SelfSimBatch& b, hipStream_t s);
int mse_batched_launch(const float* a, int lda, size_t a_ps, const float* b, int ldb, size_t b_ps, int rows, int cols, float loss_weight,
                       float grad_weight, float* part, size_t part_ps, float* grad, int ldg, size_t g_ps, int pairs, hipStream_t s,
                       const float* grad_tab = nullptr);
int mse_launch(const float* a, int lda, const float* b, int ldb, int rows, int cols, float weight, float* loss_accum,
               float* grad, int ldg, hipStream_t s);
#define SPLICE_MSE_PARTIALS 1024
int mse_partials_launch(const float* a, int lda, const float* b, int ldb, int rows, int cols, float loss_weight, float grad_weight,
                        float* part, float* grad, int ldg, hipStream_t s);
int mse2_launch(const float* a, int lda, const float* b, int ldb, int rows, int cols, float loss_weight, float grad_weight,
                float* loss_accum, float* grad, int ldg, hipStream_t s);
```

### splice_amd/csrc/vit_engine.hip

```cpp
#include <string.h>

#include <string>
#include <vector>

#include "kernels.h"


struct Linear {
    bf16_t* w = nullptr;
    bf16_t* wT = nullptr;
    float* b = nullptr;
    int out = 0, in = 0;
    uint8_t* w8 = nullptr;
    float* w8_scale = nullptr;
};
struct LayerW {
    float *ln1_g = nullptr, *ln1_b = nullptr, *ln2_g = nullptr, *ln2_b = nullptr;
    Linear qkv, proj, fc1, fc2;
};

struct SpliceVit {
    int patch = 0, dim = 0, depth = 0, heads = 0, hidden = 0;
    int device = 0;
    std::vector<LayerW> layers;
    Linear pe;
    float* cls = nullptr;
    float* pos = nullptr;
    int pos_tokens = 0;
    float *norm_g = nullptr, *norm_b = nullptr;
    std::vector<void*> allocs;
    int n_set = 0;
    int fp8 = 0;
    int qfold = 1;
    float qscale = 1.0f;
};
static const float kLn2 = 0.6931471805599453f, kLog2e = 1.4426950408889634f;

struct SpliceVitCtx {
    SpliceVit* vit = nullptr;
    int B = 0, H = 0, W = 0, T = 0, Tld = 0, rows = 0, need_grad = 0;
    int grad_pass_begin = 0;
    float* pos_eff = nullptr;
    bf16_t* patches = nullptr;
    std::vector<float*> xs;
    std::vector<float*> xmid;
    std::vector<float*> mean1, rstd1, mean2, rstd2;
    std::vector<bf16_t*> qkv, attn_out, hpre;
    bf16_t* qkvT_last = nullptr;
    std::vector<float*> lse;
    float* qkv_last_f32 = nullptr;
    bf16_t* ln_out = nullptr;
    int fp8 = 0;
    uint8_t* ln_out8 = nullptr;
    float* ln_scale = nullptr;
    uint8_t* hact8 = nullptr;
    uint8_t *qkv8 = nullptr, *qkvT8 = nullptr;
    bf16_t* hact = nullptr;
    float* g = nullptr;
    bf16_t* g_bf = nullptr;
    bf16_t* dh = nullptr;
    float* dln = nullptr;
    bf16_t *dout = nullptr, *dqkv = nullptr;
    float* delta = nullptr;
    float* dpatches = nullptr;
    std::vector<void*> allocs;
    int forward_done = 0;
    int top_cls_only = 0;
    bf16_t *cls_attn = nullptr, *cls_ln = nullptr, *cls_h = nullptr, *cls_dh = nullptr, *cls_dout = nullptr;
    float *cls_probs = nullptr, *cls_dln = nullptr;
    float* cls_slabs = nullptr;
};

template <class T>
static int dev_alloc(std::vector<void*>& list, T** p, size_t n) {
    void* q = nullptr;
    if (hipMalloc(&q, n * sizeof(T) + 256) != hipSuccess) {
        splice_set_error("hipMalloc of %zu bytes failed", n * sizeof(T));
        return SPLICE_ERR_NOMEM;
    }
    list.push_back(q);
    *p = (T*)q;
    return SPLICE_OK;
}

static int pack_linear(SpliceVit* v, Linear& L, const float* w, int out, int in, hipStream_t s) {
    L.out = out; L.in = in;
    RC(dev_alloc(v->allocs, &L.w, (size_t)out * in));
    RC(dev_alloc(v->allocs, &L.wT, (size_t)out * in));
    RC(cast_f32_bf16_launch(w, L.w, (size_t)out * in, s));
    RC(transpose_f32_to_bf16_launch(w, L.wT, out, in, out, s));
    return SPLICE_OK;
}
__global__ void scale_f32_kernel(float* dst, const float* src, size_t n, size_t n_scaled, float f) {
    for (size_t i = (size_t)blockIdx.x * blockDim.x + threadIdx.x; i < n; i += (size_t)gridDim.x * blockDim.x) dst[i] = i < n_scaled ? src[i] * f : src[i];
}
static int pack_qkv(SpliceVit* v, Linear& L, const float* w, int D, hipStream_t s) {
    if (!v->qfold) return pack_linear(v, L, w, 3 * D, D, s);
    float* tmp = nullptr;
    const size_t n = (size_t)3 * D * D;
    HIPCHK(hipMalloc((void**)&tmp, n * sizeof(float)));
    hipLaunchKernelGGL(scale_f32_kernel, dim3(1024), dim3(256), 0, s, tmp, w, n, (size_t)D * D, v->qscale);
    const int rc = pack_linear(v, L, tmp, 3 * D, D, s);
    (void)hipStreamSynchronize(s);
    (void)hipFree(tmp);
    return rc;
}
static int copy_vec(SpliceVit* v, float** dst, const float* src, size_t n, hipStream_t s) {
    RC(dev_alloc(v->allocs, dst, n));
    HIPCHK(hipMemcpyAsync(*dst, src, n * sizeof(float), hipMemcpyDeviceToDevice, s));
    return SPLICE_OK;
}

__global__ void add_f32_into_bf16_kernel(bf16_t* dst, int ldd, int col0, const float* src, int lds, int rows, int cols, int qcols, float qf) {
    const size_t n = (size_t)rows * cols;
    for (size_t i = (size_t)blockIdx.x * blockDim.x + threadIdx.x; i < n; i += (size_t)gridDim.x * blockDim.x) {
        const int r = i / cols, c = i % cols;
        bf16_t* p = dst + (size_t)r * ldd + col0 + c;
        const float v = src[(size_t)r * lds + c];
        *p = f2bf(bf2f(*p) + (c < qcols ? v * qf : v));
    }
}
__global__ void grad_stream_kernel(float* g, bf16_t* g_bf, const float* add, size_t n, int init) {
    for (size_t i = (size_t)blockIdx.x * blockDim.x + threadIdx.x; i < n; i += (size_t)gridDim.x * blockDim.x) {
        float v = init ? 0.f : g[i];
        if (add) v += add[i];
        g[i] = v;
        g_bf[i] = f2bf(v);
    }
}
__global__ void scale_cols_bf16_kernel(bf16_t* x, int ld, int rows, int cols, float f) {
    const size_t n = (size_t)rows * cols;
    for (size_t i = (size_t)blockIdx.x * blockDim.x + threadIdx.x; i < n; i += (size_t)gridDim.x * blockDim.x) {
        bf16_t* p = x + (i / cols) * ld + i % cols;
        *p = f2bf(bf2f(*p) * f);
    }
}
__global__ void scale_cols_f32_kernel(float* x, int ld, int rows, int cols, float f) {
    const size_t n = (size_t)rows * cols;
    for (size_t i = (size_t)blockIdx.x * blockDim.x + threadIdx.x; i < n; i += (size_t)gridDim.x * blockDim.x) x[(i / cols) * ld + i % cols] *= f;
}
static inline unsigned grid_n(size_t n) { size_t b = (n + 255) / 256; return (unsigned)(b > 2048 ? 2048 : (b ? b : 1)); }

extern "C" {

int splice_vit_create(int patch, int dim, int depth, int heads, void** out) {
    if (!out || (patch != 8 && patch != 16) || dim % 64 || dim / 64 != heads || depth < 1 || dim > 1024) {
        splice_set_error("splice_vit_create: unsupported config patch=%d dim=%d depth=%d heads=%d (head dim must be 64)", patch, dim, depth, heads);
        return SPLICE_ERR_ARG;
    }
    SpliceVit* v = new SpliceVit();
    v->patch = patch; v->dim = dim; v->depth = depth; v->heads = heads; v->hidden = 4 * dim;
    v->qfold = 1;
    v->qscale = v->qfold ? 0.125f * kLog2e : 1.0f;
    (void)hipGetDevice(&v->device);
    v->layers.resize(depth);
    *out = v;
    return SPLICE_OK;
}

void splice_vit_destroy(void* h) {
    SpliceVit* v = (SpliceVit*)h;
    if (!v) return;
    for (void* p : v->allocs) (void)hipFree(p);
    delete v;
}

int splice_vit_set_param(void* h, const char* name, const float* data, long long numel, splice_stream_t stream) {
    SpliceVit* v = (SpliceVit*)h;
    hipStream_t s = (hipStream_t)stream;
    if (!v || !name || !data) return SPLICE_ERR_ARG;
    const int D = v->dim, Hd = v->hidden, pp3 = 3 * v->patch * v->patch;
    std::string n(name);
    auto expect = [&](long long want) {
        if (numel != want) { splice_set_error("splice_vit_set_param(%s): numel %lld, expected %lld", name, numel, want); return false; }
        return true;
    };
    if (n == "cls_token") { if (!expect(D)) return SPLICE_ERR_ARG; RC(copy_vec(v, &v->cls, data, D, s)); }
    else if (n == "pos_embed") {
        if (numel % D) return SPLICE_ERR_ARG;
        v->pos_tokens = (int)(numel / D);
        RC(copy_vec(v, &v->pos, data, numel, s));
    }
    else if (n == "patch_embed.proj.weight") { if (!expect((long long)D * pp3)) return SPLICE_ERR_ARG; RC(pack_linear(v, v->pe, data, D, pp3, s)); }
    else if (n == "patch_embed.proj.bias") { if (!expect(D)) return SPLICE_ERR_ARG; RC(copy_vec(v, &v->pe.b, data, D, s)); }
    else if (n == "norm.weight") { if (!expect(D)) return SPLICE_ERR_ARG; RC(copy_vec(v, &v->norm_g, data, D, s)); }
    else if (n == "norm.bias") { if (!expect(D)) return SPLICE_ERR_ARG; RC(copy_vec(v, &v->norm_b, data, D, s)); }
    else if (n.rfind("blocks.", 0) == 0) {
        const size_t dot = n.find('.', 7);
        if (dot == std::string::npos) return SPLICE_ERR_ARG;
        const int li = atoi(n.substr(7, dot - 7).c_str());
        if (li < 0 || li >= v->depth) { splice_set_error("splice_vit_set_param: layer %d out of range", li); return SPLICE_ERR_ARG; }
        LayerW& L = v->layers[li];
        const std::string r = n.substr(dot + 1);
        if (r == "norm1.weight") { if (!expect(D)) return SPLICE_ERR_ARG; RC(copy_vec(v, &L.ln1_g, data, D, s)); }
        else if (r == "norm1.bias") { if (!expect(D)) return SPLICE_ERR_ARG; RC(copy_vec(v, &L.ln1_b, data, D, s)); }
        else if (r == "norm2.weight") { if (!expect(D)) return SPLICE_ERR_ARG; RC(copy_vec(v, &L.ln2_g, data, D, s)); }
        else if (r == "norm2.bias") { if (!expect(D)) return SPLICE_ERR_ARG; RC(copy_vec(v, &L.ln2_b, data, D, s)); }
        else if (r == "attn.qkv.weight") { if (!expect(3LL * D * D)) return SPLICE_ERR_ARG; RC(pack_qkv(v, L.qkv, data, D, s)); }
        else if (r == "attn.qkv.bias") { if (!expect(3 * D)) return SPLICE_ERR_ARG; RC(copy_vec(v, &L.qkv.b, data, 3 * D, s)); if (v->qfold) hipLaunchKernelGGL(scale_f32_kernel, dim3(8), dim3(256), 0, s, L.qkv.b, L.qkv.b, (size_t)3 * D, (size_t)D, v->qscale); }
        else if (r == "attn.proj.weight") { if (!expect((long long)D * D)) return SPLICE_ERR_ARG; RC(pack_linear(v, L.proj, data, D, D, s)); }
        else if (r == "attn.proj.bias") { if (!expect(D)) return SPLICE_ERR_ARG; RC(copy_vec(v, &L.proj.b, data, D, s)); }
        else if (r == "mlp.fc1.weight") { if (!expect((long long)Hd * D)) return SPLICE_ERR_ARG; RC(pack_linear(v, L.fc1, data, Hd, D, s)); }
        else if (r == "mlp.fc1.bias") { if (!expect(Hd)) return SPLICE_ERR_ARG; RC(copy_vec(v, &L.fc1.b, data, Hd, s)); }
        else if (r == "mlp.fc2.weight") { if (!expect((long long)Hd * D)) return SPLICE_ERR_ARG; RC(pack_linear(v, L.fc2, data, D, Hd, s)); }
        else if (r == "mlp.fc2.bias") { if (!expect(D)) return SPLICE_ERR_ARG; RC(copy_vec(v, &L.fc2.b, data, D, s)); }
        else { splice_set_error("splice_vit_set_param: unknown key %s", name); return SPLICE_ERR_ARG; }
    } else { splice_set_error("splice_vit_set_param: unknown key %s", name); return SPLICE_ERR_ARG; }
    v->n_set++;
    return SPLICE_OK;
}

int splice_vit_enable_fp8(void* h, splice_stream_t stream) {
    SpliceVit* v = (SpliceVit*)h;
    if (!v || !splice_vit_params_complete(h) || v->dim % 128) { splice_set_error("splice_vit_enable_fp8: incomplete weights or dim %% 128 != 0"); return SPLICE_ERR_STATE; }
    hipStream_t s = (hipStream_t)stream;
    for (auto& L : v->layers) {
        for (Linear* lin : {&L.qkv, &L.fc1, &L.fc2}) {
            if (lin->w8) continue;
            RC(dev_alloc(v->allocs, &lin->w8, (size_t)lin->out * lin->in));
            RC(dev_alloc(v->allocs, &lin->w8_scale, (size_t)lin->out));
            RC(quantize_rows_bf16_fp8_launch(lin->w, lin->in, lin->w8, lin->in, lin->w8_scale, lin->out, lin->in, s));
        }
    }
    v->fp8 = 1;
    return SPLICE_OK;
}

float splice_vit_qscale(void* h) { return h ? ((SpliceVit*)h)->qscale : 1.0f; }

int splice_vit_params_complete(void* h) {
    SpliceVit* v = (SpliceVit*)h;
    if (!v) return 0;
    bool ok = v->cls && v->pos && v->pe.w && v->pe.b;
    for (auto& L : v->layers)
        ok = ok && L.ln1_g && L.ln1_b && L.ln2_g && L.ln2_b && L.qkv.w && L.qkv.b && L.proj.w && L.proj.b && L.fc1.w &&
             L.fc1.b && L.fc2.w && L.fc2.b;
    return ok ? 1 : 0;
}

int splice_vit_ctx_create(void* h, int B, int H, int W, const float* pos_TD, int need_grad, splice_stream_t stream, void** out);
}

__global__ void pos_eff_kernel(float* pos_eff, const float* pos, const float* cls, const float* pe_bias, int T, int Tld, int D) {
    const size_t n = (size_t)Tld * D;
    for (size_t i = (size_t)blockIdx.x * blockDim.x + threadIdx.x; i < n; i += (size_t)gridDim.x * blockDim.x) {
        const int t = i / D, d = i % D;
        float v;
        if (t == 0) v = cls[d] + pos[d] - pe_bias[d];
        else if (t < T) v = pos[(size_t)t * D + d];
        else v = -pe_bias[d];
        pos_eff[i] = v;
    }
}

extern "C" {

int splice_vit_ctx_create(void* h, int B, int H, int W, const float* pos_TD, int need_grad, splice_stream_t stream, void** out) {
    SpliceVit* v = (SpliceVit*)h;
    hipStream_t s = (hipStream_t)stream;
    if (!v || !out || B < 1 || !splice_vit_params_complete(h)) {
        splice_set_error("splice_vit_ctx_create: bad handle / incomplete weights / B<1");
        return SPLICE_ERR_STATE;
    }
    const int p = v->patch, D = v->dim, Hd = v->hidden, pp3 = 3 * p * p;
    if (H < p || W < p) return SPLICE_ERR_ARG;
    SpliceVitCtx* c = new SpliceVitCtx();
    c->vit = v; c->B = B; c->H = H; c->W = W; c->need_grad = need_grad;
    c->T = 1 + (H / p) * (W / p);
    c->Tld = (c->T + 31) / 32 * 32;
    c->rows = B * c->Tld;
    const size_t rows = c->rows;
    const int L = v->depth;
    int rc = SPLICE_OK;
#define A(ptr, n) if (rc == SPLICE_OK) rc = dev_alloc(c->allocs, &(ptr), (size_t)(n))
    A(c->pos_eff, (size_t)c->Tld * D);
    A(c->patches, rows * pp3);
    c->xs.resize(L + 1); c->xmid.resize(L); c->mean1.resize(L); c->rstd1.resize(L); c->mean2.resize(L); c->rstd2.resize(L);
    c->qkv.resize(L); c->attn_out.resize(L); c->hpre.resize(L); c->lse.resize(L);
    for (int l = 0; l <= L; ++l) A(c->xs[l], rows * D);
    for (int l = 0; l < L; ++l) {
        A(c->xmid[l], rows * D);
        A(c->mean1[l], rows); A(c->rstd1[l], rows); A(c->mean2[l], rows); A(c->rstd2[l], rows);
        A(c->qkv[l], rows * 3 * D); A(c->attn_out[l], rows * D);
        A(c->hpre[l], rows * Hd);
        A(c->lse[l], (size_t)B * v->heads * c->Tld);
    }
    A(c->qkv_last_f32, rows * 3 * D);
    A(c->qkvT_last, rows * 3 * D);
    A(c->ln_out, rows * D);
    A(c->cls_attn, (size_t)B * D); A(c->cls_ln, (size_t)B * D); A(c->cls_h, (size_t)B * Hd); A(c->cls_probs, (size_t)B * v->heads * c->Tld);
    A(c->cls_slabs, (size_t)16 * B * Hd);
    if (need_grad) { A(c->cls_dh, (size_t)B * Hd); A(c->cls_dout, (size_t)B * D); A(c->cls_dln, (size_t)B * D); }
    A(c->hact, rows * Hd);
    if (need_grad) {
        A(c->g, rows * D); A(c->g_bf, rows * D); A(c->dh, rows * Hd); A(c->dln, rows * D * 4);
        A(c->dout, rows * D); A(c->dqkv, rows * 3 * D);
        A(c->delta, (size_t)B * v->heads * c->Tld);
        A(c->dpatches, rows * pp3);
    }
#undef A
    if (rc != SPLICE_OK) {
        for (void* q : c->allocs) (void)hipFree(q);
        delete c;
        return rc;
    }
    SPLICE_LAUNCH(pos_eff_kernel, dim3(grid_n((size_t)c->Tld * D)), dim3(256), 0, s, c->pos_eff, pos_TD, v->cls, v->pe.b, c->T, c->Tld, D);
    *out = c;
    return SPLICE_OK;
}

void splice_vit_ctx_destroy(void* ctx) {
    SpliceVitCtx* c = (SpliceVitCtx*)ctx;
    if (!c) return;
    for (void* p : c->allocs) (void)hipFree(p);
    delete c;
}

int splice_vit_ctx_info(void* ctx, int* T, int* Tld, int* rows) {
    SpliceVitCtx* c = (SpliceVitCtx*)ctx;
    if (!c) return SPLICE_ERR_ARG;
    if (T) *T = c->T;
    if (Tld) *Tld = c->Tld;
    if (rows) *rows = c->rows;
    return SPLICE_OK;
}

int splice_vit_ctx_set_top_cls_only(void* ctx, int on) {
    SpliceVitCtx* c = (SpliceVitCtx*)ctx;
    if (!c) return SPLICE_ERR_ARG;
    c->top_cls_only = on ? 1 : 0;
    return SPLICE_OK;
}

int splice_vit_ctx_set_fp8(void* ctx, int mode) {
    SpliceVitCtx* c = (SpliceVitCtx*)ctx;
    if (!c || mode < 0 || mode > 3 || mode == 2) return SPLICE_ERR_ARG;
    if (mode && !c->vit->fp8) { splice_set_error("splice_vit_ctx_set_fp8: the engine has no e4m3 weights (splice_vit_enable_fp8 first)"); return SPLICE_ERR_STATE; }
    const size_t rows = c->rows;
    if (mode && !c->ln_out8) {
        RC(dev_alloc(c->allocs, &c->ln_out8, rows * c->vit->dim));
        RC(dev_alloc(c->allocs, &c->ln_scale, rows));
        RC(dev_alloc(c->allocs, &c->hact8, rows * c->vit->hidden));
    }
    if ((mode & 2) && !c->qkv8) {
        RC(dev_alloc(c->allocs, &c->qkv8, rows * 3 * c->vit->dim));
        RC(dev_alloc(c->allocs, &c->qkvT8, rows * 3 * c->vit->dim));
    }
    c->fp8 = mode;
    return SPLICE_OK;
}

int splice_vit_ctx_dims(void* ctx, int* B, int* H, int* W, int* D, int* depth, int* heads, int* patch) {
    SpliceVitCtx* c = (SpliceVitCtx*)ctx;
    if (!c) return SPLICE_ERR_ARG;
    if (B) *B = c->B;
    if (H) *H = c->H;
    if (W) *W = c->W;
    if (D) *D = c->vit->dim;
    if (depth) *depth = c->vit->depth;
    if (heads) *heads = c->vit->heads;
    if (patch) *patch = c->vit->patch;
    return SPLICE_OK;
}

int splice_vit_forward_ex(void* ctx, const float* img, int normalize, int grad_pass_begin, splice_stream_t stream) {
    SpliceVitCtx* c = (SpliceVitCtx*)ctx;
    if (!c) return SPLICE_ERR_ARG;
    return splice_vit_forward_passes(ctx, img, normalize, grad_pass_begin, 0, c->B, stream);
}
int splice_vit_forward(void* ctx, const float* img, int normalize, splice_stream_t stream) {
    return splice_vit_forward_ex(ctx, img, normalize, 0, stream);
}
int splice_vit_forward_passes(void* ctx, const float* img, int normalize, int grad_pass_begin, int pass_begin, int pass_end,
                              splice_stream_t stream) {
    SpliceVitCtx* c = (SpliceVitCtx*)ctx;
    if (!c || !img || grad_pass_begin < 0 || grad_pass_begin > c->B || pass_begin < 0 || pass_end > c->B || pass_begin >= pass_end)
        return SPLICE_ERR_ARG;
    c->grad_pass_begin = grad_pass_begin;
    SpliceVit* v = c->vit;
    hipStream_t s = (hipStream_t)stream;
    const int D = v->dim, Hd = v->hidden, pp3 = 3 * v->patch * v->patch, L = v->depth;
    const int Bp = pass_end - pass_begin, R = Bp * c->Tld;
    const size_t r0 = (size_t)pass_begin * c->Tld;
    bf16_t* patches = c->patches + r0 * pp3;
    bf16_t* ln_out = c->ln_out + r0 * D;
    bf16_t* hact = c->hact + r0 * Hd;
    RC(patchify_launch(img + (size_t)pass_begin * 3 * c->H * c->W, patches, Bp, c->H, c->W, v->patch, c->Tld, normalize, s));
    {
        GemmEpi e = {};
        e.bias = v->pe.b; e.resid = c->pos_eff; e.ldr = D; e.resid_mod = c->Tld; e.out_f32 = c->xs[0] + r0 * D; e.ldo = D;
        RC(gemm_nt_launch(EPI_BIAS | EPI_RESID | EPI_OUT_F32, patches, pp3, v->pe.w, pp3, R, D, pp3, e, s));
    }
    for (int l = 0; l < L; ++l) {
        const LayerW& W = v->layers[l];
        float* x_in = c->xs[l] + r0 * D;
        float* x_mid = c->xmid[l] + r0 * D;
        const bool fp8 = (c->fp8 & 1) && c->ln_out8 && W.qkv.w8;
        const bool fp8_attn = fp8 && (c->fp8 & 2) && c->qkv8;
        {
            SpliceProfScope ps(10); SPLICE_DEV_REGION(1);
            if (fp8) RC(layernorm_fwd_fp8_launch(x_in, W.ln1_g, W.ln1_b, c->ln_out8 + r0 * D, c->ln_scale + r0, c->mean1[l] + r0, c->rstd1[l] + r0, R, D, 1e-6f, s));
            else RC(layernorm_fwd_launch(x_in, W.ln1_g, W.ln1_b, ln_out, c->mean1[l] + r0, c->rstd1[l] + r0, R, D, 1e-6f, s));
        }
        {
            GemmEpi e = {};
            e.bias = W.qkv.b; e.out_bf = c->qkv[l] + r0 * 3 * D; e.ldbf = 3 * D;
            unsigned fl = EPI_BIAS | EPI_OUT_BF;
            if (l == L - 1) {
                fl |= EPI_OUT_T | EPI_COLS_F32;
                e.out_bf_t = c->qkvT_last + r0; e.ldt = c->rows;
                e.out_f32_cols = c->qkv_last_f32 + r0 * 3 * D; e.ld_cols = 3 * D; e.col_lo = 0; e.col_hi = 3 * D;
            }
            SpliceProfScope ps(l == L - 1 ? 0 : 2); SPLICE_DEV_REGION(2);
            if (fp8) {
                e.row_scale = c->ln_scale + r0; e.col_scale = W.qkv.w8_scale;
                if (fp8_attn && !(l == L - 1 && c->top_cls_only)) {
                    fl |= EPI_OUT_F8 | EPI_OUT_F8T;
                    e.out_f8 = c->qkv8 + r0 * 3 * D; e.ld8 = 3 * D; e.out_f8_t = c->qkvT8 + r0; e.ldt8 = c->rows;
                }
                RC(gemm_nt_fp8_launch(fl | EPI_SCALE_RC, c->ln_out8 + r0 * D, D, W.qkv.w8, D, R, 3 * D, D, e, s));
            } else {
                RC(gemm_nt_launch(fl, ln_out, D, W.qkv.w, D, R, 3 * D, D, e, s));
            }
        }
        if (l == L - 1 && c->top_cls_only) {
            SPLICE_DEV_REGION(19);
            const int rs = c->Tld * D, hs = c->Tld * Hd;
            bf16_t* cattn = c->cls_attn + (size_t)pass_begin * D;
            bf16_t* cln = c->cls_ln + (size_t)pass_begin * D;
            bf16_t* ch = c->cls_h + (size_t)pass_begin * Hd;
            RC(attn_cls_fwd_launch(c->qkv[l] + r0 * 3 * D, c->qkvT_last + r0, c->rows, Bp, c->T, c->Tld, D, v->heads, v->qfold ? kLn2 : 0.125f, cattn,
                                   c->cls_probs + (size_t)pass_begin * v->heads * c->Tld, s));
            const size_t sstr = (size_t)c->B * Hd;
            float* slabs = c->cls_slabs + (size_t)pass_begin * Hd;
            auto ks_of = [](int K) { int n = K / 64, k = 16; while (k > 1 && n % k) --k; return k; };
            {
                GemmEpi e = {};
                e.out_f32 = slabs; e.ldo = D; e.ksplit = ks_of(D); e.slab_stride = (long long)sstr;
                RC(gemm_nt_launch(EPI_OUT_F32, cattn, D, W.proj.w, D, Bp, D, D, e, s));
                RC(ln_rows_fwd_launch(x_mid, rs, W.ln2_g, W.ln2_b, cln, D, c->mean2[l] + r0, c->rstd2[l] + r0, c->Tld, Bp, D, 1e-6f, slabs, e.ksplit, sstr,
                                      W.proj.b, x_in, rs, s));
            }
            {
                GemmEpi e = {};
                e.out_f32 = slabs; e.ldo = Hd; e.ksplit = ks_of(D); e.slab_stride = (long long)sstr;
                RC(gemm_nt_launch(EPI_OUT_F32, cln, D, W.fc1.w, D, Bp, Hd, D, e, s));
                const int lo = c->grad_pass_begin - pass_begin;
                RC(rows_finish_launch(1, slabs, e.ksplit, sstr, Bp, Hd, W.fc1.b, nullptr, 0, nullptr, 0, ch, c->need_grad ? c->hpre[l] + r0 * Hd : nullptr, nullptr, hs,
                                      lo > 0 ? lo : 0, s));
            }
            {
                GemmEpi e = {};
                e.out_f32 = slabs; e.ldo = D; e.ksplit = ks_of(Hd); e.slab_stride = (long long)sstr;
                RC(gemm_nt_launch(EPI_OUT_F32, ch, Hd, W.fc2.w, Hd, Bp, D, Hd, e, s));
                RC(rows_finish_launch(0, slabs, e.ksplit, sstr, Bp, D, W.fc2.b, x_mid, rs, c->xs[l + 1] + r0 * D, rs, nullptr, nullptr, nullptr, 0, 0, s));
            }
            continue;
        }
        {
            AttnArgs a = {};
            a.qkv = c->qkv[l] + r0 * 3 * D; a.B = Bp; a.T = c->T; a.Tld = c->Tld; a.D = D; a.H = v->heads;
            a.scale = v->qfold ? kLn2 : 0.125f; a.qfold = v->qfold; a.out = c->attn_out[l] + r0 * D; a.lse = c->lse[l] + (size_t)pass_begin * v->heads * c->Tld;
            if (fp8_attn) { a.qkv8 = c->qkv8 + r0 * 3 * D; a.qkvT8 = c->qkvT8 + r0; a.ldt8 = c->rows; }
            SpliceProfScope ps(3); SPLICE_DEV_REGION(3);
            RC(attn_fwd_launch(&a, s));
        }
        {
            GemmEpi e = {};
            e.bias = W.proj.b; e.resid = x_in; e.ldr = D; e.out_f32 = x_mid; e.ldo = D;
            SpliceProfScope ps(9); SPLICE_DEV_REGION(4);
            RC(gemm_nt_launch(EPI_BIAS | EPI_RESID | EPI_OUT_F32, c->attn_out[l] + r0 * D, D, W.proj.w, D, R, D, D, e, s));
        }
        {
            SpliceProfScope ps(10); SPLICE_DEV_REGION(1);
            if (fp8) RC(layernorm_fwd_fp8_launch(x_mid, W.ln2_g, W.ln2_b, c->ln_out8 + r0 * D, c->ln_scale + r0, c->mean2[l] + r0, c->rstd2[l] + r0, R, D, 1e-6f, s));
            else RC(layernorm_fwd_launch(x_mid, W.ln2_g, W.ln2_b, ln_out, c->mean2[l] + r0, c->rstd2[l] + r0, R, D, 1e-6f, s));
        }
        {
            GemmEpi e = {};
            e.bias = W.fc1.b; e.out_bf = hact; e.ldbf = Hd; e.out_pre = c->need_grad ? c->hpre[l] + r0 * Hd : nullptr; e.ldp = Hd;
            const long lo = (long)c->grad_pass_begin * c->Tld - (long)r0;
            e.pre_row_lo = lo > 0 ? (int)lo : 0;
            SpliceProfScope ps(1); SPLICE_DEV_REGION(5);
            if (fp8) {
                e.out_bf = nullptr; e.out_f8 = c->hact8 + r0 * Hd; e.ld8 = Hd;
                e.row_scale = c->ln_scale + r0; e.col_scale = W.fc1.w8_scale;
                RC(gemm_nt_fp8_launch(EPI_SCALE_RC | EPI_BIAS | EPI_GELU | EPI_OUT_F8, c->ln_out8 + r0 * D, D, W.fc1.w8, D, R, Hd, D, e, s));
            } else {
                RC(gemm_nt_launch(EPI_BIAS | EPI_GELU | EPI_OUT_BF, ln_out, D, W.fc1.w, D, R, Hd, D, e, s));
            }
        }
        {
            GemmEpi e = {};
            e.bias = W.fc2.b; e.resid = x_mid; e.ldr = D; e.out_f32 = c->xs[l + 1] + r0 * D; e.ldo = D;
            SpliceProfScope ps(4); SPLICE_DEV_REGION(6);
            if (fp8) {
                e.row_scale = nullptr; e.col_scale = W.fc2.w8_scale;
                RC(gemm_nt_fp8_launch(EPI_SCALE_RC | EPI_BIAS | EPI_RESID | EPI_OUT_F32, c->hact8 + r0 * Hd, Hd, W.fc2.w8, Hd, R, D, Hd, e, s));
            } else {
                RC(gemm_nt_launch(EPI_BIAS | EPI_RESID | EPI_OUT_F32, hact, Hd, W.fc2.w, Hd, R, D, Hd, e, s));
            }
        }
    }
    c->forward_done = 1;
    const hipError_t e = hipGetLastError();
    if (e != hipSuccess) { splice_set_error("splice_vit_forward: %s", hipGetErrorString(e)); return SPLICE_ERR_HIP; }
    return SPLICE_OK;
}

int splice_vit_get_tensor(void* ctx, int kind, int layer, void** out) {
    SpliceVitCtx* c = (SpliceVitCtx*)ctx;
    if (!c || !out || layer < 0 || layer >= c->vit->depth) return SPLICE_ERR_ARG;
    switch (kind) {
        case 0: *out = c->xs[layer + 1]; break;
        case 1: *out = c->qkv[layer]; break;
        case 2: *out = c->attn_out[layer]; break;
        case 3: *out = c->qkv_last_f32; break;
        case 4: *out = c->lse[layer]; break;
        case 5: *out = c->xs[0]; break;
        case 6: if (layer != c->vit->depth - 1) return SPLICE_ERR_ARG; *out = c->qkvT_last; break;
        case 7: *out = c->qkv[layer]; break;
        default: return SPLICE_ERR_ARG;
    }
    return SPLICE_OK;
}

int splice_vit_read_tensor(void* ctx, int kind, int layer, void* dst, size_t bytes, splice_stream_t stream) {
    void* src = nullptr;
    RC(splice_vit_get_tensor(ctx, kind, layer, &src));
    HIPCHK(hipMemcpyAsync(dst, src, bytes, hipMemcpyDeviceToDevice, (hipStream_t)stream));
    SpliceVitCtx* c = (SpliceVitCtx*)ctx;
    if (c->vit->qfold && (kind == 1 || kind == 3)) {
        const int D = c->vit->dim;
        const size_t rows = bytes / ((size_t)3 * D * (kind == 1 ? 2 : 4));
        if (kind == 1) hipLaunchKernelGGL(scale_cols_bf16_kernel, dim3(grid_n(rows * D)), dim3(256), 0, (hipStream_t)stream, (bf16_t*)dst, 3 * D, (int)rows, D, 1.0f / c->vit->qscale);
        else hipLaunchKernelGGL(scale_cols_f32_kernel, dim3(grid_n(rows * D)), dim3(256), 0, (hipStream_t)stream, (float*)dst, 3 * D, (int)rows, D, 1.0f / c->vit->qscale);
    }
    return SPLICE_OK;
}

int splice_vit_backward(void* ctx, int pass_begin, int pass_end, const float* const* d_block, const float* const* d_qkv,
                        const float* const* d_keys, float* d_img, int normalize, splice_stream_t stream) {
    SpliceVitCtx* c = (SpliceVitCtx*)ctx;
    if (!c || !c->need_grad || !c->forward_done || pass_begin < c->grad_pass_begin || pass_end > c->B || pass_begin >= pass_end || !d_img) {
        splice_set_error("splice_vit_backward: bad ctx / range / no forward / ctx created without need_grad");
        return SPLICE_ERR_STATE;
    }
    SpliceVit* v = c->vit;
    hipStream_t s = (hipStream_t)stream;
    const int D = v->dim, Hd = v->hidden, pp3 = 3 * v->patch * v->patch, L = v->depth;
    const size_t r0 = (size_t)pass_begin * c->Tld;
    const int R = (pass_end - pass_begin) * c->Tld;
    const int Bp = pass_end - pass_begin;
    float* g = c->g + r0 * D;
    bf16_t* g_bf = c->g_bf + r0 * D;
    bool g_live = false;
    const size_t slab = (size_t)c->rows * D;
    const int tiles1 = cdiv(c->Tld, 64) * cdiv(D, 64);
    const int ks = (tiles1 * 3 <= 640 && D % 192 == 0) ? 3 : (tiles1 <= 640 && D % 128 == 0) ? 2 : 1;
    for (int l = L - 1; l >= 0; --l) {
        const LayerW& W = v->layers[l];
        const float* db = d_block ? d_block[l] : nullptr;
        const float* dq = d_qkv ? d_qkv[l] : nullptr;
        const float* dk = d_keys ? d_keys[l] : nullptr;
        if (db) {
            SPLICE_LAUNCH(grad_stream_kernel, dim3(grid_n((size_t)R * D)), dim3(256), 0, s, g, g_bf, db + r0 * D, (size_t)R * D, g_live ? 0 : 1);
            g_live = true;
        }
        if (!g_live && !dq && !dk) continue;
        bf16_t* dqkv = c->dqkv + r0 * 3 * D;
        const float* g_after_mlp = nullptr;
        if (g_live && l == L - 1 && c->top_cls_only) {
            SPLICE_DEV_REGION(20);
            const int rs = c->Tld * D, hs = c->Tld * Hd;
            bf16_t* cdh = c->cls_dh + (size_t)pass_begin * Hd;
            const size_t sstr = (size_t)c->B * Hd;
            float* slabs = c->cls_slabs + (size_t)pass_begin * Hd;
            auto ks_of = [](int K) { int n = K / 64, k = 16; while (k > 1 && n % k) --k; return k; };
            {
                GemmEpi e = {};
                e.out_f32 = slabs; e.ldo = Hd; e.ksplit = ks_of(D); e.slab_stride = (long long)sstr;
                RC(gemm_nt_launch(EPI_OUT_F32, g_bf, rs, W.fc2.wT, D, Bp, Hd, D, e, s));
                RC(rows_finish_launch(2, slabs, e.ksplit, sstr, Bp, Hd, nullptr, nullptr, 0, nullptr, 0, cdh, nullptr, c->hpre[l] + r0 * Hd, hs, 0, s));
            }
            {
                GemmEpi e = {};
                e.out_f32 = slabs; e.ldo = D; e.ksplit = ks_of(Hd); e.slab_stride = (long long)sstr;
                RC(gemm_nt_launch(EPI_OUT_F32, cdh, Hd, W.fc1.wT, Hd, Bp, D, Hd, e, s));
                RC(ln_rows_bwd_launch(slabs, D, c->xmid[l] + r0 * D, rs, W.ln2_g, c->mean2[l] + r0, c->rstd2[l] + r0, c->Tld, g, g_bf, Bp, D, e.ksplit, sstr, s));
            }
            {
                GemmEpi e = {};
                e.out_f32 = slabs; e.ldo = D; e.ksplit = ks_of(D); e.slab_stride = (long long)sstr;
                RC(gemm_nt_launch(EPI_OUT_F32, g_bf, rs, W.proj.wT, D, Bp, D, D, e, s));
                RC(attn_cls_bwd_launch(c->qkv[l] + r0 * 3 * D, c->qkvT_last + r0, c->rows, Bp, c->T, c->Tld, D, v->heads, v->qfold ? kLn2 : 0.125f,
                                       c->cls_probs + (size_t)pass_begin * v->heads * c->Tld, slabs, e.ksplit, sstr, dqkv, s));
            }
            g_after_mlp = g;
        } else if (g_live) {
            {
                GemmEpi e = {};
                e.aux = c->hpre[l] + r0 * Hd; e.ldaux = Hd; e.out_bf = c->dh + r0 * Hd; e.ldbf = Hd;
                SpliceProfScope ps(11); SPLICE_DEV_REGION(7);
                RC(gemm_nt_launch(EPI_GELU_GRAD | EPI_OUT_BF, g_bf, D, W.fc2.wT, D, R, Hd, D, e, s));
            }
            {
                GemmEpi e = {};
                e.out_f32 = c->dln + r0 * D; e.ldo = D; e.ksplit = ks; e.slab_stride = (long long)slab;
                SpliceProfScope ps(5); SPLICE_DEV_REGION(8);
                RC(gemm_nt_launch(EPI_OUT_F32, c->dh + r0 * Hd, Hd, W.fc1.wT, Hd, R, D, Hd, e, s));
            }
            {
                SpliceProfScope ps(10); SPLICE_DEV_REGION(9);
                RC(layernorm_bwd_slabs_launch(c->dln + r0 * D, gemm_splitk_slabs(R, ks), slab, c->xmid[l] + r0 * D, W.ln2_g, c->mean2[l] + r0, c->rstd2[l] + r0, g, g, g_bf, R, D, s));
            }
            {
                GemmEpi e = {};
                e.out_bf = c->dout + r0 * D; e.ldbf = D;
                e.rd_other = c->attn_out[l] + r0 * D; e.ld_rd = D; e.rd_rows = c->Tld;
                e.rowdot = c->delta + (size_t)pass_begin * v->heads * c->Tld;
                SpliceProfScope ps(11); SPLICE_DEV_REGION(10);
                RC(gemm_nt_launch(EPI_OUT_BF | EPI_ROWDOT, g_bf, D, W.proj.wT, D, R, D, D, e, s));
            }
            {
                AttnArgs a = {};
                a.qkv = c->qkv[l] + r0 * 3 * D; a.B = Bp; a.T = c->T; a.Tld = c->Tld;
                a.D = D; a.H = v->heads; a.scale = v->qfold ? kLn2 : 0.125f; a.qfold = v->qfold; a.out = c->attn_out[l] + r0 * D;
                a.lse = c->lse[l] + (size_t)pass_begin * v->heads * c->Tld;
                a.dout = c->dout + r0 * D; a.doutT = nullptr; a.delta = c->delta + (size_t)pass_begin * v->heads * c->Tld; a.delta_ready = 1; a.dqkv = dqkv;
                SpliceProfScope ps(6); SPLICE_DEV_REGION(11);
                RC(attn_bwd_launch(&a, s));
            }
            g_after_mlp = g;
        } else {
            RC(dev_zero_launch(dqkv, (size_t)R * 3 * D * sizeof(bf16_t), s));
        }
        if (dq) SPLICE_LAUNCH(add_f32_into_bf16_kernel, dim3(grid_n((size_t)R * 3 * D)), dim3(256), 0, s, dqkv, 3 * D, 0, dq + r0 * 3 * D, 3 * D, R, 3 * D, v->qfold ? D : 0, 1.0f / v->qscale);
        if (dk) SPLICE_LAUNCH(add_f32_into_bf16_kernel, dim3(grid_n((size_t)R * D)), dim3(256), 0, s, dqkv, 3 * D, D, dk + r0 * D, D, R, D, 0, 1.0f);
        {
            GemmEpi e = {};
            e.out_f32 = c->dln + r0 * D; e.ldo = D; e.ksplit = ks; e.slab_stride = (long long)slab;
            SpliceProfScope ps(5); SPLICE_DEV_REGION(12);
            RC(gemm_nt_launch(EPI_OUT_F32, dqkv, 3 * D, W.qkv.wT, 3 * D, R, D, 3 * D, e, s));
        }
        {
            SpliceProfScope ps(10); SPLICE_DEV_REGION(9);
            RC(layernorm_bwd_slabs_launch(c->dln + r0 * D, gemm_splitk_slabs(R, ks), slab, c->xs[l] + r0 * D, W.ln1_g, c->mean1[l] + r0, c->rstd1[l] + r0, g_after_mlp, g, g_bf, R, D, s));
        }
        g_live = true;
    }
    if (!g_live) {
        RC(dev_zero_launch(d_img + (size_t)pass_begin * 3 * c->H * c->W, (size_t)Bp * 3 * c->H * c->W * sizeof(float), s));
        return SPLICE_OK;
// ... 13 lines not shown
```

### splice_amd/csrc/vit_ops.hip

```cpp
#include "kernels.h"

template <int MAXV>
__global__ __launch_bounds__(256) void layernorm_fwd_kernel(const float* __restrict__ x, const float* __restrict__ gamma,
                                                            const float* __restrict__ beta, bf16_t* __restrict__ y,
                                                            float* __restrict__ mean_o, float* __restrict__ rstd_o,
                                                            int rows, int D, float eps) {
    const int lane = threadIdx.x & 63;
    const int row = blockIdx.x * 4 + (threadIdx.x >> 6);
    if (row >= rows) return;
    const int nv = D >> 2;
    const float4* xr = reinterpret_cast<const float4*>(x + (size_t)row * D);
    const float4* g4 = reinterpret_cast<const float4*>(gamma);
    const float4* b4 = reinterpret_cast<const float4*>(beta);
    float4 v[MAXV], gv[MAXV], bv[MAXV];
    float sum = 0.f;
#pragma unroll
    for (int i = 0; i < MAXV; ++i) {
        if (64 * i >= nv) continue;
        const int j = min(lane + 64 * i, nv - 1);
        v[i] = xr[j]; gv[i] = g4[j]; bv[i] = b4[j];
    }
#pragma unroll
    for (int i = 0; i < MAXV; ++i) {
        if (!(64 * i < nv && lane + 64 * i < nv)) v[i] = float4{0.f, 0.f, 0.f, 0.f};
        sum += v[i].x + v[i].y + v[i].z + v[i].w;
    }
    const float mean = wave_sum(sum) / (float)D;
    float sq = 0.f;
#pragma unroll
    for (int i = 0; i < MAXV; ++i) {
        const int idx = lane + 64 * i;
        if (idx < nv) {
            const float a = v[i].x - mean, b = v[i].y - mean, c = v[i].z - mean, d = v[i].w - mean;
            sq += a * a + b * b + c * c + d * d;
        }
    }
    const float rstd = rsqrtf(wave_sum(sq) / (float)D + eps);
    if (lane == 0 && mean_o) { mean_o[row] = mean; rstd_o[row] = rstd; }
    uint2* yr = reinterpret_cast<uint2*>(y + (size_t)row * D);
#pragma unroll
    for (int i = 0; i < MAXV; ++i) {
        const int idx = lane + 64 * i;
        if (idx < nv) {
            const float4 g = gv[i], b = bv[i];
            st_out(yr + idx, uint2{pack2bf((v[i].x - mean) * rstd * g.x + b.x, (v[i].y - mean) * rstd * g.y + b.y),
                                   pack2bf((v[i].z - mean) * rstd * g.z + b.z, (v[i].w - mean) * rstd * g.w + b.w)});
        }
    }
}

int layernorm_fwd_launch(const float* x, const float* gamma, const float* beta, bf16_t* y, float* mean, float* rstd,
                         int rows, int D, float eps, hipStream_t s) {
    if (D % 4 || D > 64 * 4 * 4) return SPLICE_ERR_ARG;
    SPLICE_LAUNCH(layernorm_fwd_kernel<4>, dim3(cdiv(rows, 4)), dim3(256), 0, s, x, gamma, beta, y, mean, rstd, rows, D, eps);
    return SPLICE_OK;
}

__device__ __forceinline__ uint32_t pack4fp8(float a, float b, float c, float d) {
    int v = 0;
    v = __builtin_amdgcn_cvt_pk_fp8_f32(a, b, v, false);
    v = __builtin_amdgcn_cvt_pk_fp8_f32(c, d, v, true);
    return (uint32_t)v;
}
template <int MAXV>
__global__ __launch_bounds__(256) void layernorm_fwd_fp8_kernel(const float* __restrict__ x, const float* __restrict__ gamma,
                                                                const float* __restrict__ beta, uint8_t* __restrict__ y, float* __restrict__ yscale,
                                                                float* __restrict__ mean_o, float* __restrict__ rstd_o, int rows, int D, float eps) {
    const int lane = threadIdx.x & 63;
    const int row = blockIdx.x * 4 + (threadIdx.x >> 6);
    if (row >= rows) return;
    const int nv = D >> 2;
    const float4* xr = reinterpret_cast<const float4*>(x + (size_t)row * D);
    const float4* g4 = reinterpret_cast<const float4*>(gamma);
    const float4* b4 = reinterpret_cast<const float4*>(beta);
    float4 v[MAXV], gv[MAXV], bv[MAXV];
    float sum = 0.f;
#pragma unroll
    for (int i = 0; i < MAXV; ++i) {
        if (64 * i >= nv) continue;
        const int j = min(lane + 64 * i, nv - 1);
        v[i] = xr[j]; gv[i] = g4[j]; bv[i] = b4[j];
    }
#pragma unroll
    for (int i = 0; i < MAXV; ++i) {
        if (!(64 * i < nv && lane + 64 * i < nv)) v[i] = float4{0.f, 0.f, 0.f, 0.f};
        sum += v[i].x + v[i].y + v[i].z + v[i].w;
    }
    const float mean = wave_sum(sum) / (float)D;
    float sq = 0.f;
#pragma unroll
    for (int i = 0; i < MAXV; ++i) {
        if (lane + 64 * i < nv) {
            const float a = v[i].x - mean, b = v[i].y - mean, c = v[i].z - mean, d = v[i].w - mean;
            sq += a * a + b * b + c * c + d * d;
        }
    }
    const float rstd = rsqrtf(wave_sum(sq) / (float)D + eps);
    if (lane == 0 && mean_o) { mean_o[row] = mean; rstd_o[row] = rstd; }
    float amax = 0.f;
#pragma unroll
    for (int i = 0; i < MAXV; ++i) {
        if (lane + 64 * i < nv) {
            const float4 g = gv[i], b = bv[i];
            v[i] = float4{(v[i].x - mean) * rstd * g.x + b.x, (v[i].y - mean) * rstd * g.y + b.y, (v[i].z - mean) * rstd * g.z + b.z,
                          (v[i].w - mean) * rstd * g.w + b.w};
            amax = fmaxf(amax, fmaxf(fmaxf(fabsf(v[i].x), fabsf(v[i].y)), fmaxf(fabsf(v[i].z), fabsf(v[i].w))));
        }
    }
    amax = fmaxf(wave_max(amax), 1e-20f);
    const float q = 448.0f / amax;
    if (lane == 0) yscale[row] = amax / 448.0f;
    uint32_t* yr = reinterpret_cast<uint32_t*>(y + (size_t)row * D);
#pragma unroll
    for (int i = 0; i < MAXV; ++i)
        if (lane + 64 * i < nv) yr[lane + 64 * i] = pack4fp8(v[i].x * q, v[i].y * q, v[i].z * q, v[i].w * q);
}
int layernorm_fwd_fp8_launch(const float* x, const float* gamma, const float* beta, uint8_t* y, float* yscale, float* mean, float* rstd,
                             int rows, int D, float eps, hipStream_t s) {
    if (D % 4 || D > 64 * 4 * 4) return SPLICE_ERR_ARG;
    SPLICE_LAUNCH(layernorm_fwd_fp8_kernel<4>, dim3(cdiv(rows, 4)), dim3(256), 0, s, x, gamma, beta, y, yscale, mean, rstd, rows, D, eps);
    return SPLICE_OK;
}
template <class T>
__global__ __launch_bounds__(256) void quantize_rows_fp8_kernel(const T* __restrict__ x, int ldx, uint8_t* __restrict__ q, int ldq, float* __restrict__ scale,
                                                                float* __restrict__ qnorm, int rows, int cols, size_t x_pstride, size_t q_pstride, int rows_alloc) {
    const int lane = threadIdx.x & 63;
    const int row = blockIdx.x * 4 + (threadIdx.x >> 6);
    if (row >= rows_alloc) return;
    const T* xr = x + (size_t)blockIdx.y * x_pstride + (size_t)row * ldx;
    auto ld = [&](int c) -> float {
        if constexpr (sizeof(T) == 2) return bf2f(xr[c]);
        else return xr[c];
    };
    float amax = 0.f;
    if (row < rows)
        for (int c = lane; c < cols; c += 64) amax = fmaxf(amax, fabsf(ld(c)));
    amax = fmaxf(wave_max(amax), 1e-20f);
    const float sc = 448.0f / amax;
    uint32_t* qr = reinterpret_cast<uint32_t*>(q + (size_t)blockIdx.y * q_pstride + (size_t)row * ldq);
    float sq = 0.f;
    for (int c4 = lane; c4 < cols / 4; c4 += 64) {
        uint32_t pk = 0;
        if (row < rows) {
            pk = pack4fp8(ld(4 * c4) * sc, ld(4 * c4 + 1) * sc, ld(4 * c4 + 2) * sc, ld(4 * c4 + 3) * sc);
            const float f0 = __builtin_amdgcn_cvt_f32_fp8((int)pk, 0), f1 = __builtin_amdgcn_cvt_f32_fp8((int)pk, 1),
                        f2 = __builtin_amdgcn_cvt_f32_fp8((int)pk, 2), f3 = __builtin_amdgcn_cvt_f32_fp8((int)pk, 3);
            sq += (f0 * f0 + f1 * f1) + (f2 * f2 + f3 * f3);
        }
        qr[c4] = pk;
    }
    sq = wave_sum(sq);
    if (lane == 0) {
        if (scale) scale[(size_t)blockIdx.y * rows_alloc + row] = row < rows ? amax / 448.0f : 0.f;
        if (qnorm) qnorm[(size_t)blockIdx.y * rows_alloc + row] = sqrtf(sq);
    }
}
int quantize_rows_fp8_launch(const float* x, int ldx, uint8_t* q, int ldq, float* scale, int rows, int cols, hipStream_t s) {
    if (cols % 4 || ldq % 4) return SPLICE_ERR_ARG;
    SPLICE_LAUNCH(quantize_rows_fp8_kernel<float>, dim3(cdiv(rows, 4), 1), dim3(256), 0, s, x, ldx, q, ldq, scale, (float*)nullptr, rows, cols, (size_t)0, (size_t)0, rows);
    return SPLICE_OK;
}
int quantize_keys_fp8_launch(const bf16_t* k, int ldk, size_t k_pstride, uint8_t* q, int ldq, size_t q_pstride, float* qnorm, int T, int Tp, int D,
                             int pairs, hipStream_t s) {
    if (D % 4 || ldq % 4) return SPLICE_ERR_ARG;
    SPLICE_LAUNCH(quantize_rows_fp8_kernel<bf16_t>, dim3(cdiv(Tp, 4), pairs), dim3(256), 0, s, k, ldk, q, ldq, (float*)nullptr, qnorm, T, D, k_pstride, q_pstride, Tp);
    return SPLICE_OK;
}
int quantize_rows_bf16_fp8_launch(const bf16_t* x, int ldx, uint8_t* q, int ldq, float* scale, int rows, int cols, hipStream_t s) {
    if (cols % 4 || ldq % 4) return SPLICE_ERR_ARG;
    SPLICE_LAUNCH(quantize_rows_fp8_kernel<bf16_t>, dim3(cdiv(rows, 4), 1), dim3(256), 0, s, x, ldx, q, ldq, scale, (float*)nullptr, rows, cols, (size_t)0, (size_t)0, rows);
    return SPLICE_OK;
}

constexpr int LN_MAX_SLABS = 4;
template <int MAXV>
__global__ __launch_bounds__(256) void layernorm_bwd_kernel(const float* __restrict__ dy, const float* __restrict__ x,
                                                            const float* __restrict__ gamma, const float* __restrict__ mean_i,
                                                            const float* __restrict__ rstd_i, const float* __restrict__ g_in,
                                                            float* __restrict__ g_out, bf16_t* __restrict__ g_out_bf,
                                                            int rows, int D, int n_slabs, size_t slab_stride) {
    const int lane = threadIdx.x & 63;
    const int row = blockIdx.x * 4 + (threadIdx.x >> 6);
    if (row >= rows) return;
    const int nv = D >> 2;
    const float4* xr = reinterpret_cast<const float4*>(x + (size_t)row * D);
    const float4* dr = reinterpret_cast<const float4*>(dy + (size_t)row * D);
    const float4* g4 = reinterpret_cast<const float4*>(gamma);
    const float4* gi = g_in ? reinterpret_cast<const float4*>(g_in + (size_t)row * D) : nullptr;
    const float mean = mean_i[row], rstd = rstd_i[row];
    float4 xv[MAXV], gv[MAXV], dv[MAXV], ev[LN_MAX_SLABS - 1][MAXV], av[MAXV];
#pragma unroll
    for (int i = 0; i < MAXV; ++i) {
        if (64 * i >= nv) continue;
        const int j = min(lane + 64 * i, nv - 1);
        xv[i] = xr[j]; gv[i] = g4[j]; dv[i] = dr[j];
#pragma unroll
        for (int sl = 1; sl < LN_MAX_SLABS; ++sl)
            if (sl < n_slabs) ev[sl - 1][i] = reinterpret_cast<const float4*>(dy + (size_t)sl * slab_stride + (size_t)row * D)[j];
        if (gi) av[i] = gi[j];
    }
    float4 xh[MAXV], dh[MAXV];
// ... 248 lines not shown
```

Measured before the change: 262.5.

## Fold LayerNorm into adjacent GEMMs via partial stats and gamma-folded weights

Drops the standalone LayerNorm forward kernels. The producing GEMMs (patch embed, proj, fc2) now emit per-32-column partial statistics alongside the raw residual output. The consuming QKV and fc1 GEMMs then apply mean/rstd correction in their epilogue, using weights pre-multiplied by gamma plus a beta-folded bias. This saves a full read/write pass over activations per LayerNorm, at the cost of extra epilogue work, register pressure, a separate finalize kernel on some paths, and small numerical differences from bf16 rounding of the unnormalized input.

```diff
diff --git a/include/splice_hip.h b/include/splice_hip.h
--- a/include/splice_hip.h
+++ b/include/splice_hip.h
@@ -48,13 +48,18 @@
     int ld8;
     uint8_t* out_f8_t;
     int ldt8;
+    float* ln_part;
+    const float* ln_c1;
+    float* ln_mean;
+    float* ln_rstd;
+    float ln_eps;
 } splice_gemm_epilogue;
 
 enum {
     SPLICE_EPI_BIAS = 1, SPLICE_EPI_RESID = 2, SPLICE_EPI_OUT_F32 = 4, SPLICE_EPI_OUT_BF = 8,
     SPLICE_EPI_OUT_T = 16, SPLICE_EPI_GELU = 32, SPLICE_EPI_GELU_GRAD = 64,
     SPLICE_EPI_COLS_F32 = 128, SPLICE_EPI_ALPHA = 256, SPLICE_EPI_ROWDOT = 512, SPLICE_EPI_SCALE_RC = 1024, SPLICE_EPI_OUT_F8 = 2048,
-    SPLICE_EPI_OUT_F8T = 4096
+    SPLICE_EPI_OUT_F8T = 4096, SPLICE_EPI_LN_STATS = 8192, SPLICE_EPI_LN_A = 16384
 };
 
 int splice_gemm_nt_bf16(unsigned flags, const splice_bf16* A, int lda, const splice_bf16* B, int ldb,
@@ -71,6 +76,9 @@
 
 int splice_layernorm_fwd(const float* x, const float* gamma, const float* beta, splice_bf16* y,
                          float* mean, float* rstd, int rows, int D, float eps, splice_stream_t stream);
+int splice_ln_fold_pack(const float* w, const float* gamma, const float* beta, const float* bias, splice_bf16* wg, float* c1,
+                        float* bias_f, int N, int K, splice_stream_t stream);
+int splice_ln_fold_finalize(const float* part, float* mean, float* rstd, int rows, int D, float eps, splice_stream_t stream);
 int splice_layernorm_bwd(const float* dy, const float* x, const float* gamma, const float* mean,
                          const float* rstd, const float* g_in, float* g_out, splice_bf16* g_out_bf,
                          int rows, int D, splice_stream_t stream);
diff --git a/splice_amd/_lib.py b/splice_amd/_lib.py
--- a/splice_amd/_lib.py
+++ b/splice_amd/_lib.py
@@ -21,6 +21,7 @@
         ("row_scale", C.c_void_p), ("col_scale", C.c_void_p),
         ("out_f8", C.c_void_p), ("ld8", C.c_int),
         ("out_f8_t", C.c_void_p), ("ldt8", C.c_int),
+        ("ln_part", C.c_void_p), ("ln_c1", C.c_void_p), ("ln_mean", C.c_void_p), ("ln_rstd", C.c_void_p), ("ln_eps", C.c_float),
     ]
 
 
@@ -44,6 +45,7 @@
 
 EPI_BIAS, EPI_RESID, EPI_OUT_F32, EPI_OUT_BF, EPI_OUT_T = 1, 2, 4, 8, 16
 EPI_GELU, EPI_GELU_GRAD, EPI_COLS_F32, EPI_ALPHA, EPI_ROWDOT, EPI_SCALE_RC, EPI_OUT_F8, EPI_OUT_F8T = 32, 64, 128, 256, 512, 1024, 2048, 4096
+EPI_LN_STATS, EPI_LN_A = 8192, 16384
 
 _vp, _i, _f, _sz, _u = C.c_void_p, C.c_int, C.c_float, C.c_size_t, C.c_uint
 
@@ -60,6 +62,8 @@
     "splice_attention_qfold": ([_i], _i),
     "splice_attention_bwd_variant": ([_i], _i),
     "splice_layernorm_fwd": ([_vp, _vp, _vp, _vp, _vp, _vp, _i, _i, _f, _vp], _i),
+    "splice_ln_fold_pack": ([_vp, _vp, _vp, _vp, _vp, _vp, _vp, _i, _i, _vp], _i),
+    "splice_ln_fold_finalize": ([_vp, _vp, _vp, _i, _i, _f, _vp], _i),
     "splice_layernorm_bwd": ([_vp, _vp, _vp, _vp, _vp, _vp, _vp, _vp, _i, _i, _vp], _i),
     "splice_attention_fwd": ([_vp, _vp, _i, _i, _i, _i, _i, _i, _f, _vp, _vp, _vp], _i),
     "splice_attention_fwd_fp8": ([_vp, _vp, _i, _i, _i, _i, _i, _i, _f, _vp, _vp, _vp], _i),
diff --git a/splice_amd/csrc/capi.hip b/splice_amd/csrc/capi.hip
--- a/splice_amd/csrc/capi.hip
+++ b/splice_amd/csrc/capi.hip
@@ -65,6 +65,13 @@
 int splice_layernorm_fwd(const float* x, const float* gamma, const float* beta, splice_bf16* y, float* mean, float* rstd,
                          int rows, int D, float eps, splice_stream_t stream) {
     return finish(layernorm_fwd_launch(x, gamma, beta, y, mean, rstd, rows, D, eps, ST(stream)), "splice_layernorm_fwd");
+}
+int splice_ln_fold_pack(const float* w, const float* gamma, const float* beta, const float* bias, splice_bf16* wg, float* c1, float* bias_f, int N, int K,
+                        splice_stream_t stream) {
+    return finish(ln_fold_pack_launch(w, gamma, beta, bias, wg, c1, bias_f, N, K, ST(stream)), "splice_ln_fold_pack");
+}
+int splice_ln_fold_finalize(const float* part, float* mean, float* rstd, int rows, int D, float eps, splice_stream_t stream) {
+    return finish(ln_fold_finalize_launch(part, mean, rstd, rows, D, eps, ST(stream)), "splice_ln_fold_finalize");
 }
 int splice_layernorm_bwd(const float* dy, const float* x, const float* gamma, const float* mean, const float* rstd,
                          const float* g_in, float* g_out, splice_bf16* g_out_bf, int rows, int D, splice_stream_t stream) {
diff --git a/splice_amd/csrc/gemm.h b/splice_amd/csrc/gemm.h
--- a/splice_amd/csrc/gemm.h
+++ b/splice_amd/csrc/gemm.h
@@ -301,8 +301,55 @@
     EPI_OUT_BF = SPLICE_EPI_OUT_BF, EPI_OUT_T = SPLICE_EPI_OUT_T, EPI_GELU = SPLICE_EPI_GELU,
     EPI_GELU_GRAD = SPLICE_EPI_GELU_GRAD, EPI_COLS_F32 = SPLICE_EPI_COLS_F32, EPI_ALPHA = SPLICE_EPI_ALPHA,
     EPI_ROWDOT = SPLICE_EPI_ROWDOT, EPI_SCALE_RC = SPLICE_EPI_SCALE_RC, EPI_OUT_F8 = SPLICE_EPI_OUT_F8,
-    EPI_OUT_F8T = SPLICE_EPI_OUT_F8T
+    EPI_OUT_F8T = SPLICE_EPI_OUT_F8T, EPI_LN_STATS = SPLICE_EPI_LN_STATS, EPI_LN_A = SPLICE_EPI_LN_A
 };
+
+constexpr int LN_MAX_D = 768;
+constexpr int LN_SLOT = 3;
+__device__ __forceinline__ float ln_sum4(const f32x4& v) {
+#pragma clang fp contract(off)
+    return (v[0] + v[1]) + (v[2] + v[3]);
+}
+__device__ __forceinline__ float ln_sq4(const f32x4& v, float m) {
+#pragma clang fp contract(off)
+    const float a = v[0] - m, b = v[1] - m, c = v[2] - m, d = v[3] - m;
+    return (a * a + b * b) + (c * c + d * d);
+}
+__device__ __forceinline__ float ln_dev4(const f32x4& v, float m) {
+#pragma clang fp contract(off)
+    return ((v[0] - m) + (v[1] - m)) + ((v[2] - m) + (v[3] - m));
+}
+__device__ __forceinline__ float ln_group_mean(float sum) {
+#pragma clang fp contract(off)
+    return sum * (1.0f / 32.0f);
+}
+struct LnPart { float4 v[18]; };
+__device__ __forceinline__ void ln_load_part(LnPart& p, const float* part, int row, int D) {
+    const float4* src = reinterpret_cast<const float4*>(part + (size_t)row * ((D >> 5) * LN_SLOT));
+#pragma unroll
+    for (int v = 0; v < 18; ++v) p.v[v] = v * 128 < 3 * D ? src[v] : float4{0.f, 0.f, 0.f, 0.f};
+}
+__device__ __forceinline__ void ln_row_stats(const LnPart& p, int D, float eps, float& mean, float& rstd) {
+    double A = 0.0, B = 0.0, C = 0.0, E = 0.0, F = 0.0;
+#pragma unroll
+    for (int g = 0; g < 24; ++g)
+        if (g * 32 < D) {
+            const int o = 3 * g;
+            auto at = [&](int k) { const float4& v = p.v[k >> 2]; return (k & 3) == 0 ? v.x : (k & 3) == 1 ? v.y : (k & 3) == 2 ? v.z : v.w; };
+            const double S = (double)at(o), Q = (double)at(o + 1), R = (double)at(o + 2);
+            A += S; B += R; C += Q;
+            E = __builtin_fma(S, S, E);
+            F = __builtin_fma(S, R, F);
+        }
+    const double m = (A + B) / (double)D;
+    const double q = __builtin_fma(-(double)D * m, m, __builtin_fma(E, 1.0 / 32.0, __builtin_fma(F, 1.0 / 16.0, C)));
+    mean = (float)m;
+    rstd = rsqrtf((float)(q / (double)D) + eps);
+}
+__device__ __forceinline__ f32x4 ln_apply(const f32x4& acc, float mean, float rstd, const float4& c1) {
+#pragma clang fp contract(off)
+    return f32x4{rstd * (acc[0] - mean * c1.x), rstd * (acc[1] - mean * c1.y), rstd * (acc[2] - mean * c1.z), rstd * (acc[3] - mean * c1.w)};
+}
 
 template <unsigned FLAGS>
 __device__ __forceinline__ void gemm_epilogue(const GemmEpi& e, int M, int N, int row0, int col, f32x4 v) {
@@ -602,6 +649,42 @@
         const int gr = m0 + r, gc = n0 + k;
         if (gr >= M || gc >= N) continue;
         st_out(reinterpret_cast<f32x4*>(out + (size_t)gr * ld + gc), *reinterpret_cast<const f32x4*>(cs + r * PITCH + k));
+    }
+}
+
+template <int BM, int BN>
+__device__ __forceinline__ void gemm_stage_store_f32_ln(const f32x4 (&acc)[BM / 32][BN / 32], float* cs, const GemmEpi& e, int M, int N, int m0, int n0) {
+    constexpr int FMt = BM / 32, FNt = BN / 32, PITCH = BN + 4, CH = BN / 4;
+    static_assert(CH % 8 == 0 && (BM * CH) % 256 == 0, "whole 32-column groups per 8 lanes, whole passes");
+    const int lane = threadIdx.x & 63, wave = threadIdx.x >> 6, wm = wave >> 1, wn = wave & 1;
+    __syncthreads();
+#pragma unroll
+    for (int i = 0; i < FMt; ++i)
+#pragma unroll
+        for (int j = 0; j < FNt; ++j) {
+            const int lr = wm * (BM / 2) + i * 16 + (lane & 15), lc = wn * (BN / 2) + j * 16 + (lane >> 4) * 4;
+            *reinterpret_cast<f32x4*>(cs + lr * PITCH + lc) = acc[i][j];
+        }
+    __syncthreads();
+    const int groups = N >> 5;
+#pragma unroll 2
+    for (int c = threadIdx.x; c < BM * CH; c += 256) {
+        const int r = c / CH, k = (c % CH) * 4;
+        const int gr = m0 + r, gc = n0 + k;
+        const bool on = gr < M;
+        const f32x4 v = *reinterpret_cast<const f32x4*>(cs + r * PITCH + k);
+        if (on) {
+            st_out(reinterpret_cast<f32x4*>(e.out_f32 + (size_t)gr * e.ldo + gc), v);
+            st_out(reinterpret_cast<u32x2*>(e.out_bf + (size_t)gr * e.ldbf + gc), u32x2{pack2bf(v[0], v[1]), pack2bf(v[2], v[3])});
+        }
+        float t = ln_sum4(v);
+        t += __shfl_xor(t, 4, 64); t += __shfl_xor(t, 1, 64); t += __shfl_xor(t, 2, 64);
+        const float gmean = ln_group_mean(t);
+        float u = ln_sq4(v, gmean), w = ln_dev4(v, gmean);
+        u += __shfl_xor(u, 4, 64); u += __shfl_xor(u, 1, 64); u += __shfl_xor(u, 2, 64);
+        w += __shfl_xor(w, 4, 64); w += __shfl_xor(w, 1, 64); w += __shfl_xor(w, 2, 64);
+        const int sl = lane & 7;
+        if (on && sl < LN_SLOT) e.ln_part[((size_t)gr * groups + (gc >> 5)) * LN_SLOT + sl] = sl == 0 ? t : sl == 1 ? u : w;
     }
 }
 
@@ -624,6 +707,16 @@
     grouped_tile(t, tiles_m, tiles_n, gm, tm, tn);
     const int m0 = tm * BM, n0 = tn * BN;
     GemmTile<BM, BN, true, FP8> tile;
+    constexpr bool LNA = (FLAGS & EPI_LN_A) != 0;
+    LnPart lnp;
+    float4 c1v[LNA ? GemmTile<BM, BN>::FN : 1];
+    if constexpr (LNA) {
+#pragma unroll
+        for (int j = 0; j < GemmTile<BM, BN>::FN; ++j)
+            c1v[j] = *reinterpret_cast<const float4*>(e.ln_c1 + min(n0 + (int)((threadIdx.x >> 6) & 1) * (BN / 2) + j * 16 + (int)((threadIdx.x & 63) >> 4) * 4, N - 4));
+    }
+    if constexpr (LNA)
+        ln_load_part(lnp, e.ln_part, min(m0 + ((threadIdx.x >> 6) >> 1) * (BM / 2) + (int)(threadIdx.x & 63) % (BM / 2), M - 1), K);
     bool walked = false;
     if constexpr (FLAGS == EPI_OUT_F32 && NS == 2) {
         if (ksplit < -1) {
@@ -647,6 +740,22 @@
     if (walked) {
     } else if (NS == 2) tile.run_glds(A, lda, B, ldb, M, N, K, m0, n0, gemm_smem, kbeg);
     else tile.template run_ring<(NS < 3 ? 3 : NS)>(A, lda, B, ldb, M, N, K, m0, n0, gemm_smem, kbeg);
+    if constexpr (LNA) {
+        constexpr int FMt = GemmTile<BM, BN>::FM, FNt = GemmTile<BM, BN>::FN;
+        const int lane = threadIdx.x & 63, wave = threadIdx.x >> 6, wm = wave >> 1, wn = wave & 1;
+#pragma unroll
+        for (int v = 0; v < 18; ++v) asm volatile("" : "+v"(lnp.v[v].x), "+v"(lnp.v[v].y), "+v"(lnp.v[v].z), "+v"(lnp.v[v].w));
+        float mean, rstd;
+        ln_row_stats(lnp, K, e.ln_eps, mean, rstd);
+        const int srow = m0 + wm * (BM / 2) + lane;
+        if (tn == 0 && wn == 0 && lane < BM / 2 && srow < M) { e.ln_mean[srow] = mean; e.ln_rstd[srow] = rstd; }
+#pragma unroll
+        for (int i = 0; i < FMt; ++i) {
+            const float mi = __shfl(mean, i * 16 + (lane & 15), 64), ri = __shfl(rstd, i * 16 + (lane & 15), 64);
+#pragma unroll
+            for (int j = 0; j < FNt; ++j) tile.acc[i][j] = ln_apply(tile.acc[i][j], mi, ri, c1v[j]);
+        }
+    }
     constexpr bool HAS_OPERANDS = (FLAGS & (EPI_BIAS | EPI_RESID | EPI_GELU_GRAD)) != 0;
     constexpr bool STAGE_F32_FITS = (size_t)NS * GemmTile<BM, BN>::LDS_ELEMS * 2 >= (size_t)BM * (BN + 4) * 4;
     const bool pre_ok = HAS_OPERANDS && !(N & 3) && (!(FLAGS & EPI_RESID) || !(e.ldr & 3)) && (!(FLAGS & EPI_GELU_GRAD) || !(e.ldaux & 3));
@@ -724,6 +833,29 @@
 #pragma unroll
                     for (int r = 0; r < 4; ++r) tile.acc[i][j][r] = bf2f(f2bf(tile.acc[i][j][r]));
         }
+    } else if constexpr ((FLAGS & EPI_LN_STATS) != 0) {
+        static_assert(STAGE_F32_FITS, "an EPI_LN_STATS producer stages its fp32 tile");
+        constexpr int FMt = GemmTile<BM, BN>::FM, FNt = GemmTile<BM, BN>::FN;
+        const int lane = threadIdx.x & 63, wave = threadIdx.x >> 6, wm = wave >> 1, wn = wave & 1;
+        float4 pb[FNt], pr[FMt][FNt];
+#pragma unroll
+        for (int j = 0; j < FNt; ++j) {
+            const int colc = min(n0 + wn * (BN / 2) + j * 16 + (lane >> 4) * 4, N - 4);
+            pb[j] = *reinterpret_cast<const float4*>(e.bias + colc);
+#pragma unroll
+            for (int i = 0; i < FMt; ++i) {
+                const int rowc = min(m0 + wm * (BM / 2) + i * 16 + (lane & 15), M - 1);
+                const int rr = e.resid_mod ? rowc % e.resid_mod : rowc;
+                pr[i][j] = *reinterpret_cast<const float4*>(e.resid + (size_t)rr * e.ldr + colc);
+            }
+        }
+#pragma unroll
+        for (int i = 0; i < FMt; ++i)
+#pragma unroll
+            for (int j = 0; j < FNt; ++j)
+                tile.acc[i][j] = gemm_frag_value<FLAGS, true, false>(e, M, N, m0 + wm * (BM / 2) + i * 16 + (lane & 15),
+                                                                     n0 + wn * (BN / 2) + j * 16 + (lane >> 4) * 4, tile.acc[i][j], pb[j], pr[i][j], uint2{});
+        if constexpr (STAGE_F32_FITS) gemm_stage_store_f32_ln<BM, BN>(tile.acc, reinterpret_cast<float*>(gemm_smem), e, M, N, m0, n0);
     } else if (STAGE_F32_FITS && (FLAGS & EPI_OUT_F32) && !(FLAGS & (EPI_OUT_BF | EPI_COLS_F32)) && !(N & 3) && !(e.ldo & 3) && (!(FLAGS & EPI_RESID) || !(e.ldr & 3))) {
         constexpr int FMt = GemmTile<BM, BN>::FM, FNt = GemmTile<BM, BN>::FN;
         const int lane = threadIdx.x & 63, wave = threadIdx.x >> 6, wm = wave >> 1, wn = wave & 1;
diff --git a/splice_amd/csrc/gemm.hip b/splice_amd/csrc/gemm.hip
--- a/splice_amd/csrc/gemm.hip
+++ b/splice_amd/csrc/gemm.hip
@@ -9,11 +9,17 @@
                          hipStream_t s) {
     const long t128 = (long)cdiv(M, 128) * cdiv(N, 128);
     const long t12864 = (long)cdiv(M, 128) * cdiv(N, 64);
-    if constexpr (FLAGS == (EPI_BIAS | EPI_OUT_BF) || FLAGS == (EPI_BIAS | EPI_GELU | EPI_OUT_BF) || FLAGS == (EPI_BIAS | EPI_RESID | EPI_OUT_F32)) {
+    constexpr unsigned BASE = FLAGS & ~(EPI_LN_A | EPI_LN_STATS);
+    if constexpr (BASE == (EPI_BIAS | EPI_OUT_BF) || BASE == (EPI_BIAS | EPI_GELU | EPI_OUT_BF) || BASE == (EPI_BIAS | EPI_RESID | EPI_OUT_F32)) {
         constexpr int on8p = 7;
         const int bit = (FLAGS & EPI_OUT_F32) ? 4 : (FLAGS & EPI_GELU) ? 2 : 1;
         const bool want = g_force_tile == 5 ? gemm8p_operands_ok(N, K, e, FLAGS) : (!g_force_tile && (on8p & bit) && gemm8p_shape_ok(M, N, K, lda, ldb, e, FLAGS));
         if (want) {
+            if constexpr ((FLAGS & EPI_LN_A) != 0) {
+                SpliceProfScope ps(10);
+                const int rc = ln_fold_finalize_launch(e.ln_part, e.ln_mean, e.ln_rstd, M, K, e.ln_eps, s);
+                if (rc != SPLICE_OK) return rc;
+            }
             launch_gemm8p<FLAGS>(s, A, lda, B, ldb, M, N, K, e);
             return SPLICE_OK;
         }
@@ -40,12 +46,13 @@
         constexpr int shortns = 3;
         if (ring && tile == 3 && ks == 1 && K < 1536 && shortns == 3) ring = 2;
     }
+    if ((FLAGS & EPI_LN_STATS) && tile == 1) ring = 1;
     if constexpr ((FLAGS & EPI_ROWDOT) != 0) {
         if (ring == 2) launch_gemm_nt<64, 64, FLAGS, 3>(s, A, lda, B, ldb, M, N, K, e);
         else if (ring) launch_gemm_nt<64, 64, FLAGS, 4>(s, A, lda, B, ldb, M, N, K, e);
         else launch_gemm_nt<64, 64, FLAGS, 2>(s, A, lda, B, ldb, M, N, K, e);
     } else {
-        if constexpr (FLAGS == (EPI_BIAS | EPI_RESID | EPI_OUT_F32)) {
+        if constexpr (BASE == (EPI_BIAS | EPI_RESID | EPI_OUT_F32)) {
             constexpr int t96 = SPLICE_T96;
             const long wg64 = (long)cdiv(M, 64) * cdiv(N, 64), wg96 = (long)cdiv(M, 64) * (N / 96);
             if (t96 && !(t96 == 5 && K < 1536) && !(t96 == 6 && K >= 1536) && tile == 3 && N % 96 == 0 && wg64 > 256 && wg96 <= 256) {
@@ -57,7 +64,7 @@
         if (tile == 3 && ring == 2) { launch_gemm_nt<64, 64, FLAGS, 3>(s, A, lda, B, ldb, M, N, K, e); return SPLICE_OK; }
         if (tile == 2 && ring == 2) { launch_gemm_nt<128, 64, FLAGS, 3>(s, A, lda, B, ldb, M, N, K, e); return SPLICE_OK; }
         switch (tile * 2 + (ring ? 1 : 0)) {
-            case 2: launch_gemm_nt<128, 128, FLAGS, 2>(s, A, lda, B, ldb, M, N, K, e); break;
+            case 2: if constexpr (!(FLAGS & EPI_LN_STATS)) launch_gemm_nt<128, 128, FLAGS, 2>(s, A, lda, B, ldb, M, N, K, e); break;
             case 3: launch_gemm_nt<128, 128, FLAGS, 4>(s, A, lda, B, ldb, M, N, K, e); break;
             case 4: launch_gemm_nt<128, 64, FLAGS, 2>(s, A, lda, B, ldb, M, N, K, e); break;
             case 5: launch_gemm_nt<128, 64, FLAGS, 4>(s, A, lda, B, ldb, M, N, K, e); break;
@@ -73,7 +80,12 @@
     if (M < 1 || N < 1 || K < GEMM_BK || K % GEMM_BK || lda % 8 || ldb % 8) return SPLICE_ERR_ARG;
     if ((size_t)M * lda * sizeof(bf16_t) >= (1ull << 32) || (size_t)N * ldb * sizeof(bf16_t) >= (1ull << 32)) return SPLICE_ERR_ARG;
     if ((flags & EPI_OUT_T) && (e.ldt % 4)) return SPLICE_ERR_ARG;
-    if ((flags & EPI_ROWDOT) && (N % 64 || !e.rd_other || !e.rowdot || e.rd_rows < 1 || e.ld_rd % 4)) return SPLICE_ERR_ARG;
+    if ((flags & EPI_LN_STATS) && (N % 128 || N > LN_MAX_D || !e.ln_part || !e.out_bf || e.ldbf % 4 || e.ldo % 4 || e.ldr % 4 || !e.bias || !e.resid || !e.out_f32 ||
+                                   ((size_t)e.out_bf & 7) || ((size_t)e.out_f32 & 15) || ((size_t)e.resid & 15) || ((size_t)e.bias & 15) || ((size_t)e.ln_part & 3)))
+        return SPLICE_ERR_ARG;
+    if ((flags & EPI_LN_A) && (K % 128 || K > LN_MAX_D || N % 4 || !e.ln_part || !e.ln_c1 || !e.ln_mean || !e.ln_rstd || !e.bias || ((size_t)e.ln_part & 15) ||
+                               ((size_t)e.ln_c1 & 15)))
+        return SPLICE_ERR_ARG;
 #define CASE(F) case (F): return dispatch_tile<(F)>(A, lda, B, ldb, M, N, K, e, s)
     switch (flags) {
         CASE(EPI_BIAS | EPI_OUT_BF | EPI_OUT_T);
@@ -82,6 +94,10 @@
         CASE(EPI_BIAS | EPI_OUT_BF);
         CASE(EPI_BIAS | EPI_RESID | EPI_OUT_F32);
         CASE(EPI_BIAS | EPI_GELU | EPI_OUT_BF);
+        CASE(EPI_BIAS | EPI_RESID | EPI_OUT_F32 | EPI_LN_STATS);
+        CASE(EPI_BIAS | EPI_OUT_BF | EPI_LN_A);
+        CASE(EPI_BIAS | EPI_OUT_BF | EPI_OUT_T | EPI_COLS_F32 | EPI_LN_A);
+        CASE(EPI_BIAS | EPI_GELU | EPI_OUT_BF | EPI_LN_A);
         CASE(EPI_OUT_F32);
         CASE(EPI_OUT_F32 | EPI_ALPHA);
         CASE(EPI_OUT_BF);
diff --git a/splice_amd/csrc/gemm8p.h b/splice_amd/csrc/gemm8p.h
--- a/splice_amd/csrc/gemm8p.h
+++ b/splice_amd/csrc/gemm8p.h
@@ -162,8 +162,11 @@
 template <unsigned FLAGS>
 __global__ __launch_bounds__(512) void gemm8p_kernel(const bf16_t* __restrict__ A, int lda, const bf16_t* __restrict__ B, int ldb, int M, int N, int K, int gm,
                                                      GemmEpi e) {
-    static_assert(FLAGS == (EPI_BIAS | EPI_OUT_BF) || FLAGS == (EPI_BIAS | EPI_GELU | EPI_OUT_BF) || FLAGS == (EPI_BIAS | EPI_RESID | EPI_OUT_F32),
+    static_assert((FLAGS & ~(EPI_LN_A | EPI_LN_STATS)) == (EPI_BIAS | EPI_OUT_BF) || (FLAGS & ~(EPI_LN_A | EPI_LN_STATS)) == (EPI_BIAS | EPI_GELU | EPI_OUT_BF) ||
+                      (FLAGS & ~(EPI_LN_A | EPI_LN_STATS)) == (EPI_BIAS | EPI_RESID | EPI_OUT_F32),
                   "epilogues of the 8-phase tile");
+    static_assert(!(FLAGS & EPI_LN_A) || !(FLAGS & EPI_OUT_F32), "the folded LayerNorm's consumers write bf16");
+    static_assert(!(FLAGS & EPI_LN_STATS) || (FLAGS & EPI_OUT_F32), "the folded LayerNorm's producers write the fp32 row");
     extern __shared__ __attribute__((aligned(16))) bf16_t gemm8p_smem[];
     const int tiles_n = N / 256, tiles_m = (M + 255) / 256, ntiles = tiles_m * tiles_n;
     const int G = gridDim.x;
@@ -198,26 +201,54 @@
                                 for (int i = 0; i < 4; ++i) {
                                     const int row = m0 + mh * 128 + wr * 64 + i * 16 + (lane & 15);
                                     const f32x4 v0 = g.acc[mh * 4 + i][nh * 2 + 0], v1 = g.acc[mh * 4 + i][nh * 2 + 1];
+                                    const f32x4 x0 = {v0[0] + b0.x + r0[i].x, v0[1] + b0.y + r0[i].y, v0[2] + b0.z + r0[i].z, v0[3] + b0.w + r0[i].w};
+                                    const f32x4 x1 = {v1[0] + b1.x + r1[i].x, v1[1] + b1.y + r1[i].y, v1[2] + b1.z + r1[i].z, v1[3] + b1.w + r1[i].w};
                                     if (row < M) {
                                         float* q = e.out_f32 + (size_t)row * e.ldo + colf;
-                                        *reinterpret_cast<float4*>(q) = float4{v0[0] + b0.x + r0[i].x, v0[1] + b0.y + r0[i].y, v0[2] + b0.z + r0[i].z, v0[3] + b0.w + r0[i].w};
-                                        *reinterpret_cast<float4*>(q + 16) = float4{v1[0] + b1.x + r1[i].x, v1[1] + b1.y + r1[i].y, v1[2] + b1.z + r1[i].z, v1[3] + b1.w + r1[i].w};
+                                        *reinterpret_cast<float4*>(q) = float4{x0[0], x0[1], x0[2], x0[3]};
+                                        *reinterpret_cast<float4*>(q + 16) = float4{x1[0], x1[1], x1[2], x1[3]};
+                                    }
+                                    if constexpr ((FLAGS & EPI_LN_STATS) != 0) {
+                                        float t = ln_sum4(x0) + ln_sum4(x1);
+                                        t += __shfl_xor(t, 16, 64); t += __shfl_xor(t, 32, 64);
+                                        const float gmean = ln_group_mean(t);
+                                        float u = ln_sq4(x0, gmean) + ln_sq4(x1, gmean), w = ln_dev4(x0, gmean) + ln_dev4(x1, gmean);
+                                        u += __shfl_xor(u, 16, 64); u += __shfl_xor(u, 32, 64);
+                                        w += __shfl_xor(w, 16, 64); w += __shfl_xor(w, 32, 64);
+                                        if (grp < LN_SLOT && row < M) e.ln_part[((size_t)row * (N >> 5) + (colf >> 5)) * LN_SLOT + grp] = grp == 0 ? t : grp == 1 ? u : w;
+                                        const uint2 pa = uint2{pack2bf(x0[0], x0[1]), pack2bf(x0[2], x0[3])}, pb2 = uint2{pack2bf(x1[0], x1[1]), pack2bf(x1[2], x1[3])};
+                                        const auto rx = __builtin_amdgcn_permlane16_swap(pa.x, pb2.x, false, false);
+                                        const auto ry = __builtin_amdgcn_permlane16_swap(pa.y, pb2.y, false, false);
+                                        if (row < M) *reinterpret_cast<uint4*>(e.out_bf + (size_t)row * e.ldbf + n0 + nh * 128 + wc * 32 + c8) = uint4{rx[0], ry[0], rx[1], ry[1]};
                                     }
                                 }
                             }
                         }
                         return;
                     }
+                    float lnm[8], lnr[8];
+                    if constexpr ((FLAGS & EPI_LN_A) != 0) {
+#pragma unroll
+                        for (int q = 0; q < 8; ++q) {
+                            const int rowc = min(m0 + (q >> 2) * 128 + wr * 64 + (q & 3) * 16 + (lane & 15), M - 1);
+                            lnm[q] = e.ln_mean[rowc]; lnr[q] = e.ln_rstd[rowc];
+                        }
+                    }
 #pragma unroll
                     for (int nh = 0; nh < 2; ++nh) {
                         const int colf = n0 + nh * 128 + wc * 32 + grp * 4;
                         const float4 b0 = *reinterpret_cast<const float4*>(e.bias + colf), b1 = *reinterpret_cast<const float4*>(e.bias + colf + 16);
+                        float4 c10 = {}, c11 = {};
+                        if constexpr ((FLAGS & EPI_LN_A) != 0) { c10 = *reinterpret_cast<const float4*>(e.ln_c1 + colf); c11 = *reinterpret_cast<const float4*>(e.ln_c1 + colf + 16); }
                         const int col = n0 + nh * 128 + wc * 32 + c8;
 #pragma unroll
                         for (int mh = 0; mh < 2; ++mh)
 #pragma unroll
                             for (int i = 0; i < 4; ++i) {
                                 f32x4 v0 = g.acc[mh * 4 + i][nh * 2 + 0], v1 = g.acc[mh * 4 + i][nh * 2 + 1];
+                                if constexpr ((FLAGS & EPI_LN_A) != 0) {
+                                    v0 = ln_apply(v0, lnm[mh * 4 + i], lnr[mh * 4 + i], c10); v1 = ln_apply(v1, lnm[mh * 4 + i], lnr[mh * 4 + i], c11);
+                                }
                                 v0[0] += b0.x; v0[1] += b0.y; v0[2] += b0.z; v0[3] += b0.w;
                                 v1[0] += b1.x; v1[1] += b1.y; v1[2] += b1.z; v1[3] += b1.w;
                                 const int row = m0 + mh * 128 + wr * 64 + i * 16 + (lane & 15);
@@ -241,6 +272,8 @@
 
 static inline bool gemm8p_operands_ok(int N, int K, const GemmEpi& e, unsigned flags) {
     if (N % 256 || K % 128 || K < 128 || (reinterpret_cast<size_t>(e.bias) & 15)) return false;
+    if ((flags & EPI_LN_STATS) && (e.ldbf % 8 || (reinterpret_cast<size_t>(e.out_bf) & 15))) return false;
+    if ((flags & EPI_LN_A) && (reinterpret_cast<size_t>(e.ln_c1) & 15)) return false;
     if (flags & EPI_OUT_F32)
         return !e.resid_mod && e.ldr % 4 == 0 && e.ldo % 4 == 0 && !(reinterpret_cast<size_t>(e.resid) & 15) && !(reinterpret_cast<size_t>(e.out_f32) & 15);
     if (e.ldbf % 8 || (reinterpret_cast<size_t>(e.out_bf) & 15)) return false;
diff --git a/splice_amd/csrc/kernels.h b/splice_amd/csrc/kernels.h
--- a/splice_amd/csrc/kernels.h
+++ b/splice_amd/csrc/kernels.h
@@ -47,6 +47,8 @@
 
 int layernorm_fwd_launch(const float* x, const float* gamma, const float* beta, bf16_t* y, float* mean, float* rstd,
                          int rows, int D, float eps, hipStream_t s);
+int ln_fold_finalize_launch(const float* part, float* mean, float* rstd, int rows, int D, float eps, hipStream_t s);
+int ln_fold_pack_launch(const float* w, const float* gamma, const float* beta, const float* bias, bf16_t* wg, float* c1, float* bias_f, int N, int K, hipStream_t s);
 int layernorm_fwd_fp8_launch(const float* x, const float* gamma, const float* beta, uint8_t* y, float* yscale, float* mean, float* rstd,
                              int rows, int D, float eps, hipStream_t s);
 int quantize_rows_fp8_launch(const float* x, int ldx, uint8_t* q, int ldq, float* scale, int rows, int cols, hipStream_t s);
diff --git a/splice_amd/csrc/vit_engine.hip b/splice_amd/csrc/vit_engine.hip
--- a/splice_amd/csrc/vit_engine.hip
+++ b/splice_amd/csrc/vit_engine.hip
@@ -13,6 +13,8 @@
     int out = 0, in = 0;
     uint8_t* w8 = nullptr;
     float* w8_scale = nullptr;
+    bf16_t* wg = nullptr;
+    float *c1 = nullptr, *bfold = nullptr, *w32 = nullptr;
 };
 struct LayerW {
     float *ln1_g = nullptr, *ln1_b = nullptr, *ln2_g = nullptr, *ln2_b = nullptr;
@@ -33,6 +35,7 @@
     int fp8 = 0;
     int qfold = 1;
     float qscale = 1.0f;
+    int ln_fold = 0, ln_packed = 0;
 };
 static const float kLn2 = 0.6931471805599453f, kLog2e = 1.4426950408889634f;
 
@@ -50,6 +53,7 @@
     std::vector<float*> lse;
     float* qkv_last_f32 = nullptr;
     bf16_t* ln_out = nullptr;
+    float* ln_part = nullptr;
     int fp8 = 0;
     uint8_t* ln_out8 = nullptr;
     float* ln_scale = nullptr;
@@ -83,8 +87,13 @@
     return SPLICE_OK;
 }
 
-static int pack_linear(SpliceVit* v, Linear& L, const float* w, int out, int in, hipStream_t s) {
+static int pack_linear(SpliceVit* v, Linear& L, const float* w, int out, int in, hipStream_t s, bool keep_f32 = false) {
     L.out = out; L.in = in;
+    if (keep_f32 && v->ln_fold) {
+        if (!L.w32) RC(dev_alloc(v->allocs, &L.w32, (size_t)out * in));
+        HIPCHK(hipMemcpyAsync(L.w32, w, (size_t)out * in * sizeof(float), hipMemcpyDeviceToDevice, s));
+        v->ln_packed = 0;
+    }
     RC(dev_alloc(v->allocs, &L.w, (size_t)out * in));
     RC(dev_alloc(v->allocs, &L.wT, (size_t)out * in));
     RC(cast_f32_bf16_launch(w, L.w, (size_t)out * in, s));
@@ -95,12 +104,12 @@
     for (size_t i = (size_t)blockIdx.x * blockDim.x + threadIdx.x; i < n; i += (size_t)gridDim.x * blockDim.x) dst[i] = i < n_scaled ? src[i] * f : src[i];
 }
 static int pack_qkv(SpliceVit* v, Linear& L, const float* w, int D, hipStream_t s) {
-    if (!v->qfold) return pack_linear(v, L, w, 3 * D, D, s);
+    if (!v->qfold) return pack_linear(v, L, w, 3 * D, D, s, true);
     float* tmp = nullptr;
     const size_t n = (size_t)3 * D * D;
     HIPCHK(hipMalloc((void**)&tmp, n * sizeof(float)));
     hipLaunchKernelGGL(scale_f32_kernel, dim3(1024), dim3(256), 0, s, tmp, w, n, (size_t)D * D, v->qscale);
-    const int rc = pack_linear(v, L, tmp, 3 * D, D, s);
+    const int rc = pack_linear(v, L, tmp, 3 * D, D, s, true);
     (void)hipStreamSynchronize(s);
     (void)hipFree(tmp);
     return rc;
@@ -152,6 +161,7 @@
     v->patch = patch; v->dim = dim; v->depth = depth; v->heads = heads; v->hidden = 4 * dim;
     v->qfold = 1;
     v->qscale = v->qfold ? 0.125f * kLog2e : 1.0f;
+    v->ln_fold = dim <= LN_MAX_D && dim % 128 == 0;
     (void)hipGetDevice(&v->device);
     v->layers.resize(depth);
     *out = v;
@@ -192,16 +202,16 @@
         if (li < 0 || li >= v->depth) { splice_set_error("splice_vit_set_param: layer %d out of range", li); return SPLICE_ERR_ARG; }
         LayerW& L = v->layers[li];
         const std::string r = n.substr(dot + 1);
-        if (r == "norm1.weight") { if (!expect(D)) return SPLICE_ERR_ARG; RC(copy_vec(v, &L.ln1_g, data, D, s)); }
-        else if (r == "norm1.bias") { if (!expect(D)) return SPLICE_ERR_ARG; RC(copy_vec(v, &L.ln1_b, data, D, s)); }
-        else if (r == "norm2.weight") { if (!expect(D)) return SPLICE_ERR_ARG; RC(copy_vec(v, &L.ln2_g, data, D, s)); }
-        else if (r == "norm2.bias") { if (!expect(D)) return SPLICE_ERR_ARG; RC(copy_vec(v, &L.ln2_b, data, D, s)); }
+        if (r == "norm1.weight") { if (!expect(D)) return SPLICE_ERR_ARG; RC(copy_vec(v, &L.ln1_g, data, D, s)); v->ln_packed = 0; }
+        else if (r == "norm1.bias") { if (!expect(D)) return SPLICE_ERR_ARG; RC(copy_vec(v, &L.ln1_b, data, D, s)); v->ln_packed = 0; }
+        else if (r == "norm2.weight") { if (!expect(D)) return SPLICE_ERR_ARG; RC(copy_vec(v, &L.ln2_g, data, D, s)); v->ln_packed = 0; }
+        else if (r == "norm2.bias") { if (!expect(D)) return SPLICE_ERR_ARG; RC(copy_vec(v, &L.ln2_b, data, D, s)); v->ln_packed = 0; }
         else if (r == "attn.qkv.weight") { if (!expect(3LL * D * D)) return SPLICE_ERR_ARG; RC(pack_qkv(v, L.qkv, data, D, s)); }
-        else if (r == "attn.qkv.bias") { if (!expect(3 * D)) return SPLICE_ERR_ARG; RC(copy_vec(v, &L.qkv.b, data, 3 * D, s)); if (v->qfold) hipLaunchKernelGGL(scale_f32_kernel, dim3(8), dim3(256), 0, s, L.qkv.b, L.qkv.b, (size_t)3 * D, (size_t)D, v->qscale); }
+        else if (r == "attn.qkv.bias") { if (!expect(3 * D)) return SPLICE_ERR_ARG; RC(copy_vec(v, &L.qkv.b, data, 3 * D, s)); v->ln_packed = 0; if (v->qfold) hipLaunchKernelGGL(scale_f32_kernel, dim3(8), dim3(256), 0, s, L.qkv.b, L.qkv.b, (size_t)3 * D, (size_t)D, v->qscale); }
         else if (r == "attn.proj.weight") { if (!expect((long long)D * D)) return SPLICE_ERR_ARG; RC(pack_linear(v, L.proj, data, D, D, s)); }
         else if (r == "attn.proj.bias") { if (!expect(D)) return SPLICE_ERR_ARG; RC(copy_vec(v, &L.proj.b, data, D, s)); }
-        else if (r == "mlp.fc1.weight") { if (!expect((long long)Hd * D)) return SPLICE_ERR_ARG; RC(pack_linear(v, L.fc1, data, Hd, D, s)); }
-        else if (r == "mlp.fc1.bias") { if (!expect(Hd)) return SPLICE_ERR_ARG; RC(copy_vec(v, &L.fc1.b, data, Hd, s)); }
+        else if (r == "mlp.fc1.weight") { if (!expect((long long)Hd * D)) return SPLICE_ERR_ARG; RC(pack_linear(v, L.fc1, data, Hd, D, s, true)); }
+        else if (r == "mlp.fc1.bias") { if (!expect(Hd)) return SPLICE_ERR_ARG; RC(copy_vec(v, &L.fc1.b, data, Hd, s)); v->ln_packed = 0; }
         else if (r == "mlp.fc2.weight") { if (!expect((long long)Hd * D)) return SPLICE_ERR_ARG; RC(pack_linear(v, L.fc2, data, D, Hd, s)); }
         else if (r == "mlp.fc2.bias") { if (!expect(D)) return SPLICE_ERR_ARG; RC(copy_vec(v, &L.fc2.b, data, D, s)); }
         else { splice_set_error("splice_vit_set_param: unknown key %s", name); return SPLICE_ERR_ARG; }
@@ -238,6 +248,25 @@
     return ok ? 1 : 0;
 }
 
+static int vit_pack_ln_fold(SpliceVit* v, hipStream_t s) {
+    if (!v->ln_fold || v->ln_packed) return SPLICE_OK;
+    for (auto& L : v->layers) {
+        struct { Linear* lin; const float *g, *b; } jobs[2] = {{&L.qkv, L.ln1_g, L.ln1_b}, {&L.fc1, L.ln2_g, L.ln2_b}};
+        for (auto& j : jobs) {
+            Linear& lin = *j.lin;
+            if (!lin.w32) { splice_set_error("vit_pack_ln_fold: no fp32 weight"); return SPLICE_ERR_STATE; }
+            if (!lin.wg) {
+                RC(dev_alloc(v->allocs, &lin.wg, (size_t)lin.out * lin.in));
+                RC(dev_alloc(v->allocs, &lin.c1, (size_t)lin.out));
+                RC(dev_alloc(v->allocs, &lin.bfold, (size_t)lin.out));
+            }
+            RC(ln_fold_pack_launch(lin.w32, j.g, j.b, lin.b, lin.wg, lin.c1, lin.bfold, lin.out, lin.in, s));
+        }
+    }
+    v->ln_packed = 1;
+    return SPLICE_OK;
+}
+
 int splice_vit_ctx_create(void* h, int B, int H, int W, const float* pos_TD, int need_grad, splice_stream_t stream, void** out);
 }
 
@@ -264,6 +293,7 @@
     }
     const int p = v->patch, D = v->dim, Hd = v->hidden, pp3 = 3 * p * p;
     if (H < p || W < p) return SPLICE_ERR_ARG;
+    RC(vit_pack_ln_fold(v, s));
     SpliceVitCtx* c = new SpliceVitCtx();
     c->vit = v; c->B = B; c->H = H; c->W = W; c->need_grad = need_grad;
     c->T = 1 + (H / p) * (W / p);
@@ -288,6 +318,7 @@
     A(c->qkv_last_f32, rows * 3 * D);
     A(c->qkvT_last, rows * 3 * D);
     A(c->ln_out, rows * D);
+    if (v->ln_fold) A(c->ln_part, rows * (D / 32) * LN_SLOT);
     A(c->cls_attn, (size_t)B * D); A(c->cls_ln, (size_t)B * D); A(c->cls_h, (size_t)B * Hd); A(c->cls_probs, (size_t)B * v->heads * c->Tld);
     A(c->cls_slabs, (size_t)16 * B * Hd);
     if (need_grad) { A(c->cls_dh, (size_t)B * Hd); A(c->cls_dout, (size_t)B * D); A(c->cls_dln, (size_t)B * D); }
@@ -385,11 +416,19 @@
     bf16_t* patches = c->patches + r0 * pp3;
     bf16_t* ln_out = c->ln_out + r0 * D;
     bf16_t* hact = c->hact + r0 * Hd;
+    const bool fold = v->ln_fold && c->ln_part && !((c->fp8 & 1) && c->ln_out8 && v->layers[0].qkv.w8);
+    if (fold) RC(vit_pack_ln_fold(v, s));
+    float* ln_part = fold ? c->ln_part + r0 * (D / 32) * LN_SLOT : nullptr;
+    auto ln_producer = [&](GemmEpi& e) { e.out_bf = ln_out; e.ldbf = D; e.ln_part = ln_part; return (unsigned)EPI_LN_STATS; };
+    auto ln_consumer = [&](GemmEpi& e, const Linear& lin, float* mean, float* rstd) {
+        e.bias = lin.bfold; e.ln_part = ln_part; e.ln_c1 = lin.c1; e.ln_mean = mean; e.ln_rstd = rstd; e.ln_eps = 1e-6f;
+        return (unsigned)EPI_LN_A;
+    };
     RC(patchify_launch(img + (size_t)pass_begin * 3 * c->H * c->W, patches, Bp, c->H, c->W, v->patch, c->Tld, normalize, s));
     {
         GemmEpi e = {};
         e.bias = v->pe.b; e.resid = c->pos_eff; e.ldr = D; e.resid_mod = c->Tld; e.out_f32 = c->xs[0] + r0 * D; e.ldo = D;
-        RC(gemm_nt_launch(EPI_BIAS | EPI_RESID | EPI_OUT_F32, patches, pp3, v->pe.w, pp3, R, D, pp3, e, s));
+        RC(gemm_nt_launch(EPI_BIAS | EPI_RESID | EPI_OUT_F32 | (fold ? ln_producer(e) : 0u), patches, pp3, v->pe.w, pp3, R, D, pp3, e, s));
     }
     for (int l = 0; l < L; ++l) {
         const LayerW& W = v->layers[l];
@@ -397,7 +436,7 @@
         float* x_mid = c->xmid[l] + r0 * D;
         const bool fp8 = (c->fp8 & 1) && c->ln_out8 && W.qkv.w8;
         const bool fp8_attn = fp8 && (c->fp8 & 2) && c->qkv8;
-        {
+        if (!fold) {
             SpliceProfScope ps(10); SPLICE_DEV_REGION(1);
             if (fp8) RC(layernorm_fwd_fp8_launch(x_in, W.ln1_g, W.ln1_b, c->ln_out8 + r0 * D, c->ln_scale + r0, c->mean1[l] + r0, c->rstd1[l] + r0, R, D, 1e-6f, s));
             else RC(layernorm_fwd_launch(x_in, W.ln1_g, W.ln1_b, ln_out, c->mean1[l] + r0, c->rstd1[l] + r0, R, D, 1e-6f, s));
@@ -419,6 +458,9 @@
                     e.out_f8 = c->qkv8 + r0 * 3 * D; e.ld8 = 3 * D; e.out_f8_t = c->qkvT8 + r0; e.ldt8 = c->rows;
                 }
                 RC(gemm_nt_fp8_launch(fl | EPI_SCALE_RC, c->ln_out8 + r0 * D, D, W.qkv.w8, D, R, 3 * D, D, e, s));
+            } else if (fold) {
+                fl |= ln_consumer(e, W.qkv, c->mean1[l] + r0, c->rstd1[l] + r0);
+                RC(gemm_nt_launch(fl, ln_out, D, W.qkv.wg, D, R, 3 * D, D, e, s));
             } else {
                 RC(gemm_nt_launch(fl, ln_out, D, W.qkv.w, D, R, 3 * D, D, e, s));
             }
@@ -469,9 +511,9 @@
             GemmEpi e = {};
             e.bias = W.proj.b; e.resid = x_in; e.ldr = D; e.out_f32 = x_mid; e.ldo = D;
             SpliceProfScope ps(9); SPLICE_DEV_REGION(4);
-            RC(gemm_nt_launch(EPI_BIAS | EPI_RESID | EPI_OUT_F32, c->attn_out[l] + r0 * D, D, W.proj.w, D, R, D, D, e, s));
-        }
-        {
+            RC(gemm_nt_launch(EPI_BIAS | EPI_RESID | EPI_OUT_F32 | (fold ? ln_producer(e) : 0u), c->attn_out[l] + r0 * D, D, W.proj.w, D, R, D, D, e, s));
+        }
+        if (!fold) {
             SpliceProfScope ps(10); SPLICE_DEV_REGION(1);
             if (fp8) RC(layernorm_fwd_fp8_launch(x_mid, W.ln2_g, W.ln2_b, c->ln_out8 + r0 * D, c->ln_scale + r0, c->mean2[l] + r0, c->rstd2[l] + r0, R, D, 1e-6f, s));
             else RC(layernorm_fwd_launch(x_mid, W.ln2_g, W.ln2_b, ln_out, c->mean2[l] + r0, c->rstd2[l] + r0, R, D, 1e-6f, s));
@@ -486,6 +528,9 @@
                 e.out_bf = nullptr; e.out_f8 = c->hact8 + r0 * Hd; e.ld8 = Hd;
                 e.row_scale = c->ln_scale + r0; e.col_scale = W.fc1.w8_scale;
                 RC(gemm_nt_fp8_launch(EPI_SCALE_RC | EPI_BIAS | EPI_GELU | EPI_OUT_F8, c->ln_out8 + r0 * D, D, W.fc1.w8, D, R, Hd, D, e, s));
+            } else if (fold) {
+                const unsigned fl = EPI_BIAS | EPI_GELU | EPI_OUT_BF | ln_consumer(e, W.fc1, c->mean2[l] + r0, c->rstd2[l] + r0);
+                RC(gemm_nt_launch(fl, ln_out, D, W.fc1.wg, D, R, Hd, D, e, s));
             } else {
                 RC(gemm_nt_launch(EPI_BIAS | EPI_GELU | EPI_OUT_BF, ln_out, D, W.fc1.w, D, R, Hd, D, e, s));
             }
@@ -498,7 +543,7 @@
                 e.row_scale = nullptr; e.col_scale = W.fc2.w8_scale;
                 RC(gemm_nt_fp8_launch(EPI_SCALE_RC | EPI_BIAS | EPI_RESID | EPI_OUT_F32, c->hact8 + r0 * Hd, Hd, W.fc2.w8, Hd, R, D, Hd, e, s));
             } else {
-                RC(gemm_nt_launch(EPI_BIAS | EPI_RESID | EPI_OUT_F32, hact, Hd, W.fc2.w, Hd, R, D, Hd, e, s));
+                RC(gemm_nt_launch(EPI_BIAS | EPI_RESID | EPI_OUT_F32 | (fold && l + 1 < L ? ln_producer(e) : 0u), hact, Hd, W.fc2.w, Hd, R, D, Hd, e, s));
             }
         }
     }
diff --git a/splice_amd/csrc/vit_ops.hip b/splice_amd/csrc/vit_ops.hip
--- a/splice_amd/csrc/vit_ops.hip
+++ b/splice_amd/csrc/vit_ops.hip
@@ -47,6 +47,43 @@
                                    pack2bf((v[i].z - mean) * rstd * g.z + b.z, (v[i].w - mean) * rstd * g.w + b.w)});
         }
     }
+}
+
+__global__ __launch_bounds__(256) void ln_fold_finalize_kernel(const float* __restrict__ part, float* __restrict__ mean_o, float* __restrict__ rstd_o, int rows,
+                                                               int D, float eps) {
+    const int row = blockIdx.x * 256 + threadIdx.x;
+    LnPart p;
+    ln_load_part(p, part, min(row, rows - 1), D);
+    float mean, rstd;
+    ln_row_stats(p, D, eps, mean, rstd);
+    if (row < rows) { mean_o[row] = mean; rstd_o[row] = rstd; }
+}
+int ln_fold_finalize_launch(const float* part, float* mean, float* rstd, int rows, int D, float eps, hipStream_t s) {
+    if (!part || !mean || !rstd || rows < 1 || D % 128 || D > LN_MAX_D || ((size_t)part & 15)) return SPLICE_ERR_ARG;
+    SPLICE_LAUNCH(ln_fold_finalize_kernel, dim3(cdiv(rows, 256)), dim3(256), 0, s, part, mean, rstd, rows, D, eps);
+    return SPLICE_OK;
+}
+__global__ __launch_bounds__(256) void ln_fold_pack_kernel(const float* __restrict__ w, const float* __restrict__ gamma, const float* __restrict__ beta,
+                                                           const float* __restrict__ bias, bf16_t* __restrict__ wg, float* __restrict__ c1,
+                                                           float* __restrict__ bias_f, int N, int K) {
+    const int lane = threadIdx.x & 63, n = blockIdx.x * 4 + (threadIdx.x >> 6);
+    if (n >= N) return;
+    float s1 = 0.f, sb = 0.f;
+    for (int k = lane; k < K; k += 64) {
+        const float wv = w[(size_t)n * K + k];
+        const bf16_t h = f2bf(wv * gamma[k]);
+        wg[(size_t)n * K + k] = h;
+        s1 += bf2f(h);
+        sb += beta[k] * wv;
+    }
+    s1 = wave_sum(s1); sb = wave_sum(sb);
+    if (lane == 0) { c1[n] = s1; bias_f[n] = bias[n] + sb; }
+}
+int ln_fold_pack_launch(const float* w, const float* gamma, const float* beta, const float* bias, bf16_t* wg, float* c1, float* bias_f, int N, int K,
+                        hipStream_t s) {
+    if (!w || !gamma || !beta || !bias || !wg || !c1 || !bias_f || N < 1 || K < 1) return SPLICE_ERR_ARG;
+    SPLICE_LAUNCH(ln_fold_pack_kernel, dim3(cdiv(N, 4)), dim3(256), 0, s, w, gamma, beta, bias, wg, c1, bias_f, N, K);
+    return SPLICE_OK;
 }
 
 int layernorm_fwd_launch(const float* x, const float* gamma, const float* beta, bf16_t* y, float* mean, float* rstd,
```

After: 258.2. 0.984x the previous value.
